# Blosc/c-blosc

Measured on AMD Instinct MI355X. Metric: compress+decompress GB/s (uncompressed) at 1/2/4/8 GPUs vs HBM roofline; ratio, higher is better.
Workload: dtype u8; 1 GPU; config #2: byte-shuffle + lz4 clevel=5 typesize=8, 128 x 64 MiB bench19 chunks per GPU (8 GiB), step = compress pass + decompress pass, device-resident; chunks_per_gpu=128, chunks_total=128, chunk_bytes=67108864

## Files before the change

### c-blosc_amd/csrc/blosc_api.hip

```cpp
#include <errno.h>
#include <pthread.h>
#include <stdio.h>
#include <stdlib.h>
#include <string.h>

#include "../../include/blosc.h"
#include "../../include/blosc_gpu.h"
#include "../../include/blosc_gpu_packed.h"
#include "../../include/blosc_gpu_params.h"
#include "../../include/blosc_gpu_getitem.h"
#include "../../include/blosc_gpu_checksum.h"
#include "blosc_format.h"
#include "engine.h"

using namespace bamd;

static pthread_mutex_t g_mutex = PTHREAD_MUTEX_INITIALIZER;
static int g_compressor = BLOSC_BLOSCLZ;
static int g_threads = 1;
static int g_force_blocksize = 0;
static int g_initlib = 0;
static int g_splitmode = BLOSC_FORWARD_COMPAT_SPLIT;

static const char* const kNames[6] = {BLOSC_BLOSCLZ_COMPNAME, BLOSC_LZ4_COMPNAME, BLOSC_LZ4HC_COMPNAME,
// ... 199 lines not shown
  const bool nolock = getenv("BLOSC_NOLOCK") != NULL;
  if (!nolock) pthread_mutex_lock(&g_mutex);
  int r = decompress_one(src, dest, destsize);
  if (!nolock) pthread_mutex_unlock(&g_mutex);
  return r;
}

int blosc_getitem(const void* src, int start, int nitems, void* dest) {
  return engine_getitem(src, start, nitems, dest, engine_is_device_pointer(src), engine_is_device_pointer(dest), (hipStream_t)0);
}

int blosc_gpu_set_device(int device) { return engine_set_device(device); }

static int compress_batch(int clevel, int doshuffle, size_t typesize, const char* compressor, size_t blocksize,
                          int nchunks, const void* const* src, const size_t* nbytes, void* const* dest,
                          const size_t* destsize, int* cbytes_out, void* stream, bool device_ptrs) {
  if (nchunks <= 0) return 0;
  const int code = compressor ? blosc_compname_to_compcode(compressor) : g_compressor;
  if (code < 0 || !codec_built(code)) { for (int i = 0; i < nchunks; i++) cbytes_out[i] = -5; return 0; }
  Job* jobs = (Job*)malloc(sizeof(Job) * (size_t)nchunks);
  if (!jobs) return -1;
  for (int i = 0; i < nchunks; i++) jobs[i] = Job{src[i], dest[i], nbytes[i], destsize[i]};
  CompressParams p{clevel, doshuffle, typesize, code, (int32_t)(blocksize ? blocksize : (size_t)g_force_blocksize), g_splitmode};
  int r = engine_compress_batch(&p, false, nchunks, jobs, cbytes_out, device_ptrs, (hipStream_t)stream);
  free(jobs);
  return r;
}
int blosc_gpu_compress_batch(int clevel, int doshuffle, size_t typesize, const char* compressor, size_t blocksize,
                             int nchunks, const void* const* src, const size_t* nbytes, void* const* dest,
                             const size_t* destsize, int* cbytes_out, void* stream) {
  return compress_batch(clevel, doshuffle, typesize, compressor, blocksize, nchunks, src, nbytes, dest, destsize, cbytes_out, stream, true);
}
int blosc_gpu_compress_batch_host(int clevel, int doshuffle, size_t typesize, const char* compressor, size_t blocksize,
                                  int nchunks, const void* const* src, const size_t* nbytes, void* const* dest,
                                  const size_t* destsize, int* cbytes_out) {
  return compress_batch(clevel, doshuffle, typesize, compressor, blocksize, nchunks, src, nbytes, dest, destsize, cbytes_out, nullptr, false);
}

static int decompress_batch(int nchunks, const void* const* src, const size_t* srcsize, void* const* dest,
                            const size_t* destsize, int* nbytes_out, void* stream, bool device_ptrs) {
  if (nchunks <= 0) return 0;
  Job* jobs = (Job*)malloc(sizeof(Job) * (size_t)nchunks);
  if (!jobs) return -1;
  for (int i = 0; i < nchunks; i++) jobs[i] = Job{src[i], dest[i], srcsize ? srcsize[i] : 0, destsize[i]};
  int r = engine_decompress_batch(nchunks, jobs, nbytes_out, device_ptrs, (hipStream_t)stream);
  free(jobs);
  return r;
}
int blosc_gpu_decompress_batch(int nchunks, const void* const* src, const size_t* srcsize, void* const* dest,
                               const size_t* destsize, int* nbytes_out, void* stream) {
  return decompress_batch(nchunks, src, srcsize, dest, destsize, nbytes_out, stream, true);
}
int blosc_gpu_decompress_batch_host(int nchunks, const void* const* src, const size_t* srcsize, void* const* dest,
                                    const size_t* destsize, int* nbytes_out) {
  return decompress_batch(nchunks, src, srcsize, dest, destsize, nbytes_out, nullptr, false);
}

static bool packed_align(size_t* align) {
  if (*align == 0) *align = 1;
  return *align <= 4096 && (*align & (*align - 1)) == 0;
}
size_t blosc_gpu_packed_bound(int nchunks, const size_t* nbytes, size_t align) {
  if (nchunks <= 0 || !nbytes || !packed_align(&align)) return 0;
  size_t total = 0;
  for (int i = 0; i < nchunks; i++) total += (nbytes[i] + BLOSC_MAX_OVERHEAD + align - 1) / align * align;
  return total;
}

int blosc_gpu_compress_packed(int clevel, int doshuffle, size_t typesize, const char* compressor, size_t blocksize,
                              int nchunks, const void* const* src, const size_t* nbytes, void* dest, size_t destsize, size_t align,
                              size_t* offsets_out, int* cbytes_out, void* stream) {
  if (nchunks < 0 || !offsets_out || !packed_align(&align)) return -1;
  if (nchunks == 0) { offsets_out[0] = 0; return 0; }
  if (!src || !nbytes || !cbytes_out || (!dest && destsize)) return -1;
  const int code = compressor ? blosc_compname_to_compcode(compressor) : g_compressor;
  if (code < 0 || !codec_built(code)) {
    for (int i = 0; i < nchunks; i++) { cbytes_out[i] = -5; offsets_out[i] = 0; }
    offsets_out[nchunks] = 0;
    return 0;
  }
  Job* jobs = (Job*)malloc(sizeof(Job) * (size_t)nchunks);
  if (!jobs) return -1;
  for (int i = 0; i < nchunks; i++) jobs[i] = Job{src[i], nullptr, nbytes[i], nbytes[i] + BLOSC_MAX_OVERHEAD};
  CompressParams p{clevel, doshuffle, typesize, code, (int32_t)(blocksize ? blocksize : (size_t)g_force_blocksize), g_splitmode};
  const PackedBuffer pk{dest, destsize, align, offsets_out};
  int r = engine_compress_batch(&p, false, nchunks, jobs, cbytes_out, true, (hipStream_t)stream, &pk);
  free(jobs);
  return r;
}

static CompressParams* chunk_params(int nchunks, const blosc_gpu_cparams* params) {
  CompressParams* p = (CompressParams*)malloc(sizeof(CompressParams) * (size_t)nchunks);
  for (int i = 0; p && i < nchunks; i++) {
    const blosc_gpu_cparams& c = params[i];
    p[i] = CompressParams{c.clevel, c.doshuffle, c.typesize, c.compcode == -1 ? g_compressor : c.compcode,
                          (int32_t)(c.blocksize ? c.blocksize : (size_t)g_force_blocksize), c.splitmode ? c.splitmode : g_splitmode};
    if (p[i].codec < 0 || p[i].codec > 5) p[i].codec = BLOSC_SNAPPY;
    if (c.splitmode < 0 || c.splitmode > BLOSC_FORWARD_COMPAT_SPLIT) p[i].doshuffle = -1;
  }
  return p;
}
int blosc_gpu_compress_batch_params(int nchunks, const blosc_gpu_cparams* params, const void* const* src, const size_t* nbytes,
                                    void* const* dest, const size_t* destsize, int* cbytes_out, void* stream) {
  if (nchunks <= 0) return 0;
  if (!params || !src || !nbytes || !dest || !destsize || !cbytes_out) return -1;
  Job* jobs = (Job*)malloc(sizeof(Job) * (size_t)nchunks);
  CompressParams* p = chunk_params(nchunks, params);
  int r = -1;
  if (jobs && p) {
    for (int i = 0; i < nchunks; i++) jobs[i] = Job{src[i], dest[i], nbytes[i], destsize[i]};
    r = engine_compress_batch(p, true, nchunks, jobs, cbytes_out, true, (hipStream_t)stream);
  }
  free(jobs); free(p);
  return r;
}
int blosc_gpu_compress_packed_params(int nchunks, const blosc_gpu_cparams* params, const void* const* src, const size_t* nbytes,
                                     void* dest, size_t destsize, size_t align, size_t* offsets_out, int* cbytes_out, void* stream) {
  if (nchunks < 0 || !offsets_out || !packed_align(&align)) return -1;
  if (nchunks == 0) { offsets_out[0] = 0; return 0; }
  if (!params || !src || !nbytes || !cbytes_out || (!dest && destsize)) return -1;
  Job* jobs = (Job*)malloc(sizeof(Job) * (size_t)nchunks);
  CompressParams* p = chunk_params(nchunks, params);
  int r = -1;
  if (jobs && p) {
    for (int i = 0; i < nchunks; i++) jobs[i] = Job{src[i], nullptr, nbytes[i], nbytes[i] + BLOSC_MAX_OVERHEAD};
    const PackedBuffer pk{dest, destsize, align, offsets_out};
    r = engine_compress_batch(p, true, nchunks, jobs, cbytes_out, true, (hipStream_t)stream, &pk);
  }
  free(jobs); free(p);
  return r;
}

int blosc_gpu_decompress_packed(int nchunks, const void* container, size_t containersize, const size_t* offsets,
                                void* dest, size_t destsize, size_t* dest_offsets_out, int* nbytes_out, void* stream) {
  if (nchunks < 0 || !dest_offsets_out) return -1;
  if (nchunks == 0) { dest_offsets_out[0] = 0; return 0; }
  if (!container || !offsets || !nbytes_out) return -1;
  for (int i = 0; i < nchunks; i++) if (offsets[i + 1] < offsets[i]) return -1;
  if (offsets[nchunks] > containersize) return -1;
  Job* jobs = (Job*)malloc(sizeof(Job) * (size_t)nchunks);
  if (!jobs) return -1;
  for (int i = 0; i < nchunks; i++) {
    const size_t span = offsets[i + 1] - offsets[i];
    jobs[i] = Job{(const uint8_t*)container + offsets[i], nullptr, span < (size_t)BLOSC_MIN_HEADER_LENGTH ? 1 : span, 0};
  }
  const PackedBuffer pk{dest, dest ? destsize : 0, 0, dest_offsets_out};
  int r = engine_decompress_batch(nchunks, jobs, nbytes_out, true, (hipStream_t)stream, &pk);
  free(jobs);
  return r;
}

int blosc_gpu_cbuffer_sizes_batch(int nchunks, const void* const* src, size_t* nbytes, size_t* cbytes, size_t* blocksize, void* stream) {
  if (nchunks < 0 || (nchunks > 0 && !src)) return -1;
  if (nchunks == 0) return 0;
  Header* h = (Header*)malloc(sizeof(Header) * (size_t)nchunks);
  if (!h) return -1;
  const int r = engine_chunk_headers(nchunks, src, h, (hipStream_t)stream);
  for (int i = 0; r == 0 && i < nchunks; i++) {
    const bool known = h[i].version == BLOSC_VERSION_FORMAT;
    if (nbytes) nbytes[i] = known ? (size_t)h[i].nbytes : 0;
    if (cbytes) cbytes[i] = known ? (size_t)h[i].cbytes : 0;
    if (blocksize) blocksize[i] = known ? (size_t)h[i].blocksize : 0;
  }
  free(h);
  return r;
}

int blosc_gpu_device_count(void) { return engine_device_count(); }
int blosc_gpu_partition(size_t nchunks, int world, int rank, size_t* lo, size_t* hi) {
  if (world <= 0 || rank < 0 || rank >= world || !lo || !hi) return -1;
  const size_t w = (size_t)world, r = (size_t)rank;
  size_t l = (r * nchunks + w - 1) / w, h = ((r + 1) * nchunks + w - 1) / w;
  if (h > nchunks) h = nchunks;
  *lo = l; *hi = h;
  return 0;
}
struct MultiArg {
  int dev, rc; bool compress; size_t lo, hi;
  int clevel, doshuffle; size_t typesize; const char* compressor; size_t blocksize;
  const void* const* src; const size_t* insize; void* const* dest; const size_t* destsize; int* out;
};
static void* multi_worker(void* p) {
  MultiArg& a = *(MultiArg*)p;
  a.rc = 0;
  if (a.hi == a.lo) return nullptr;
  if (engine_thread_device(a.dev) != 0) { a.rc = -1; return nullptr; }
  const int n = (int)(a.hi - a.lo);
  const bool devp = engine_is_device_pointer(a.src[a.lo]);
  if (a.compress) a.rc = compress_batch(a.clevel, a.doshuffle, a.typesize, a.compressor, a.blocksize, n, a.src + a.lo, a.insize + a.lo, a.dest + a.lo,
                                        a.destsize + a.lo, a.out + a.lo, nullptr, devp);
  else a.rc = decompress_batch(n, a.src + a.lo, a.insize ? a.insize + a.lo : nullptr, a.dest + a.lo, a.destsize + a.lo, a.out + a.lo, nullptr, devp);
  (void)engine_thread_device(-1);
  return nullptr;
}
static int run_multi(MultiArg proto, int ndev, const int* devices, int nchunks) {
  if (nchunks <= 0) return 0;
  const int have = engine_device_count();
  if (ndev <= 0 || ndev > 64) return -1;
  MultiArg args[64];
  pthread_t th[64];
  for (int r = 0; r < ndev; r++) {
    args[r] = proto;
    args[r].dev = devices ? devices[r] : r;
    if (args[r].dev < 0 || args[r].dev >= have) { fprintf(stderr, "blosc_amd: multi-GPU call names device %d, this node shows %d\n", args[r].dev, have); return -1; }
    (void)blosc_gpu_partition((size_t)nchunks, ndev, r, &args[r].lo, &args[r].hi);
  }
  int started = 0, rc = 0;
  for (; started < ndev; started++) if (pthread_create(&th[started], nullptr, multi_worker, &args[started]) != 0) { rc = -1; break; }
  for (int r = 0; r < started; r++) { pthread_join(th[r], nullptr); if (args[r].rc < 0) rc = args[r].rc; }
  return rc;
}
int blosc_gpu_compress_batch_multi(int ndev, const int* devices, int clevel, int doshuffle, size_t typesize, const char* compressor, size_t blocksize,
                                   int nchunks, const void* const* src, const size_t* nbytes, void* const* dest, const size_t* destsize, int* cbytes_out) {
  MultiArg a{}; a.compress = true; a.clevel = clevel; a.doshuffle = doshuffle; a.typesize = typesize; a.compressor = compressor; a.blocksize = blocksize;
  a.src = src; a.insize = nbytes; a.dest = dest; a.destsize = destsize; a.out = cbytes_out;
  return run_multi(a, ndev, devices, nchunks);
}
int blosc_gpu_decompress_batch_multi(int ndev, const int* devices, int nchunks, const void* const* src, const size_t* srcsize, void* const* dest,
                                     const size_t* destsize, int* nbytes_out) {
  MultiArg a{}; a.compress = false; a.src = src; a.insize = srcsize; a.dest = dest; a.destsize = destsize; a.out = nbytes_out;
  return run_multi(a, ndev, devices, nchunks);
}

int blosc_gpu_getitem(const void* src, int start, int nitems, void* dest, void* stream) {
  return engine_getitem(src, start, nitems, dest, true, true, (hipStream_t)stream);
}

static ItemRange* item_ranges(int nranges, const int* chunk, const int* start, const int* nitems, void* const* dest) {
  ItemRange* r = (ItemRange*)malloc(sizeof(ItemRange) * (size_t)(nranges > 0 ? nranges : 1));
  for (int i = 0; r && i < nranges; i++) r[i] = ItemRange{chunk[i], start[i], nitems[i], dest ? dest[i] : nullptr};
  return r;
}
int blosc_gpu_getitem_batch(int nchunks, const void* const* src, int nranges, const int* chunk, const int* start, const int* nitems,
                            void* const* dest, int* result_out, void* stream) {
  if (nchunks < 0 || nranges < 0) return -1;
  if (nranges == 0) return 0;
  if ((nchunks > 0 && !src) || !chunk || !start || !nitems || !dest || !result_out) return -1;
  Job* jobs = (Job*)malloc(sizeof(Job) * (size_t)(nchunks > 0 ? nchunks : 1));
  ItemRange* ranges = item_ranges(nranges, chunk, start, nitems, dest);
  int r = -1;
  if (jobs && ranges) {
    for (int i = 0; i < nchunks; i++) jobs[i] = Job{src[i], nullptr, 0, 0};
    r = engine_getitem_batch(nchunks, jobs, nranges, ranges, result_out, (hipStream_t)stream);
  }
  free(jobs); free(ranges);
  return r;
}
int blosc_gpu_getitem_packed(int nchunks, const void* container, size_t containersize, const size_t* offsets,
                             int nranges, const int* chunk, const int* start, const int* nitems,
                             void* dest, size_t destsize, size_t* dest_offsets_out, int* result_out, void* stream) {
  if (nchunks < 0 || nranges < 0 || !dest_offsets_out) return -1;
  if (nranges == 0) { dest_offsets_out[0] = 0; return 0; }
  if ((nchunks > 0 && (!container || !offsets)) || !chunk || !start || !nitems || !result_out) return -1;
  for (int i = 0; i < nchunks; i++) if (offsets[i + 1] < offsets[i]) return -1;
  if (nchunks > 0 && offsets[nchunks] > containersize) return -1;
  Job* jobs = (Job*)malloc(sizeof(Job) * (size_t)(nchunks > 0 ? nchunks : 1));
  ItemRange* ranges = item_ranges(nranges, chunk, start, nitems, nullptr);
  int r = -1;
  if (jobs && ranges) {
    for (int i = 0; i < nchunks; i++) {
      const size_t span = offsets[i + 1] - offsets[i];
      jobs[i] = Job{(const uint8_t*)container + offsets[i], nullptr, span < (size_t)BLOSC_MIN_HEADER_LENGTH ? 1 : span, 0};
    }
    const PackedBuffer pk{dest, dest ? destsize : 0, 0, dest_offsets_out};
    r = engine_getitem_batch(nchunks, jobs, nranges, ranges, result_out, (hipStream_t)stream, &pk);
  }
  free(jobs); free(ranges);
  return r;
}

static const size_t kChecksumMaxRun = (size_t)INT32_MAX + 16;
static int checksum_runs(int kind, int nruns, Job* jobs, unsigned int* digest_out, void* stream) {
  int r = -1;
  if (jobs) {
    bool ok = true;
    for (int i = 0; i < nruns && ok; i++) ok = jobs[i].srcsize <= kChecksumMaxRun && (jobs[i].srcsize == 0 || jobs[i].src);
    if (ok) r = engine_checksum_batch(kind, nruns, jobs, digest_out, (hipStream_t)stream);
  }
  free(jobs);
  return r;
}
int blosc_gpu_checksum_batch(int kind, int nruns, const void* const* src, const size_t* nbytes, unsigned int* digest_out, void* stream) {
  if (kind != BLOSC_GPU_CHECKSUM_ADLER32 && kind != BLOSC_GPU_CHECKSUM_CRC32) return -1;
  if (nruns <= 0) return 0;
  if (!src || !nbytes || !digest_out) return -1;
  Job* jobs = (Job*)malloc(sizeof(Job) * (size_t)nruns);
  for (int i = 0; jobs && i < nruns; i++) jobs[i] = Job{src[i], nullptr, nbytes[i], 0};
  return checksum_runs(kind, nruns, jobs, digest_out, stream);
}
int blosc_gpu_checksum_packed(int kind, int nruns, const void* container, size_t containersize, const size_t* offsets,
                              const size_t* length, unsigned int* digest_out, void* stream) {
  if (kind != BLOSC_GPU_CHECKSUM_ADLER32 && kind != BLOSC_GPU_CHECKSUM_CRC32) return -1;
  if (nruns <= 0) return 0;
  if (!offsets || !digest_out) return -1;
  for (int i = 0; i < nruns; i++)
    if (offsets[i + 1] < offsets[i] || (length && length[i] > offsets[i + 1] - offsets[i])) return -1;
  if (offsets[nruns] > containersize || (offsets[nruns] > offsets[0] && !container)) return -1;
  Job* jobs = (Job*)malloc(sizeof(Job) * (size_t)nruns);
  for (int i = 0; jobs && i < nruns; i++)
    jobs[i] = Job{(const uint8_t*)container + offsets[i], nullptr, length ? length[i] : offsets[i + 1] - offsets[i], 0};
  return checksum_runs(kind, nruns, jobs, digest_out, stream);
}

__attribute__((visibility("default"))) void blosc_internal_shuffle(const size_t typesize, const size_t blocksize,
                                                                   const uint8_t* src, const uint8_t* dest) {
  if (engine_filter(0, typesize, blocksize, src, (void*)dest) != 0) fprintf(stderr, "blosc_amd: shuffle failed (no GPU?)\n");
}
__attribute__((visibility("default"))) void blosc_internal_unshuffle(const size_t typesize, const size_t blocksize,
                                                                     const uint8_t* src, const uint8_t* dest) {
  if (engine_filter(1, typesize, blocksize, src, (void*)dest) != 0) fprintf(stderr, "blosc_amd: unshuffle failed (no GPU?)\n");
}
__attribute__((visibility("default"))) void blosc_internal_shuffle_generic(const size_t typesize, const size_t blocksize,
                                                                           const uint8_t* const src, uint8_t* const dest) {
  blosc_internal_shuffle(typesize, blocksize, src, dest);
}
__attribute__((visibility("default"))) void blosc_internal_unshuffle_generic(const size_t typesize, const size_t blocksize,
                                                                             const uint8_t* const src, uint8_t* const dest) {
  blosc_internal_unshuffle(typesize, blocksize, src, dest);
}
#define BAMD_SHUFFLE_ALIAS(isa)                                                                                                                  \
  __attribute__((visibility("default"))) void blosc_internal_shuffle_##isa(const size_t typesize, const size_t blocksize, const uint8_t* const src, \
                                                                           uint8_t* const dest) { blosc_internal_shuffle(typesize, blocksize, src, dest); } \
  __attribute__((visibility("default"))) void blosc_internal_unshuffle_##isa(const size_t typesize, const size_t blocksize, const uint8_t* const src, \
                                                                             uint8_t* const dest) { blosc_internal_unshuffle(typesize, blocksize, src, dest); }
BAMD_SHUFFLE_ALIAS(sse2)
BAMD_SHUFFLE_ALIAS(avx2)
#undef BAMD_SHUFFLE_ALIAS
__attribute__((visibility("default"))) int blosc_internal_bitshuffle(const size_t typesize, const size_t blocksize,
                                                                     const uint8_t* src, const uint8_t* dest,
                                                                     const uint8_t* tmp) {
  (void)tmp;
  if (engine_filter(2, typesize, blocksize, src, (void*)dest) != 0) return -1;
  const size_t n = blocksize / typesize;
  return (int)((n % 8) ? n : n * typesize);
}
__attribute__((visibility("default"))) int blosc_internal_bitunshuffle(const size_t typesize, const size_t blocksize,
                                                                       const uint8_t* src, const uint8_t* dest,
                                                                       const uint8_t* tmp) {
  (void)tmp;
  if (engine_filter(3, typesize, blocksize, src, (void*)dest) != 0) return -1;
  const size_t n = blocksize / typesize;
  return (int)((n % 8) ? n : n * typesize);
}

__attribute__((visibility("default"))) int blosc_amd_policy_blocksize(int clevel, int typesize, int nbytes, int forced,
                                                                      int codec, int splitmode) {
  return compute_blocksize(clevel, typesize, nbytes, forced, codec, splitmode);
}
__attribute__((visibility("default"))) int blosc_amd_policy_split(int codec, int typesize, int blocksize, int splitmode) {
  return split_block(codec, typesize, blocksize, splitmode);
}
__attribute__((visibility("default"))) void blosc_amd_getitem_pass_bytes(size_t bytes) { engine_getitem_pass_bytes(bytes); }

__attribute__((visibility("default"))) void blosc_amd_checksum_tile_bytes(size_t bytes) { engine_checksum_tile_bytes(bytes); }

void blosc_gpu_profile(int enable) { engine_prof_enable(enable); }
void blosc_gpu_profile_reset(void) { engine_prof_reset(); }
int blosc_gpu_profile_get(const char* kernel, double* total_ms, int* launches) { return engine_prof_get(kernel, total_ms, launches); }

}
```

### c-blosc_amd/csrc/enc_lz.h

```cpp
constexpr int ENC_WAVES = 1;
#ifndef BAMD_ENC_HASH_BITS
#define BAMD_ENC_HASH_BITS 11
#endif
constexpr int ENC_HASH_BITS = BAMD_ENC_HASH_BITS;
constexpr int ENC_TAB = 1 << ENC_HASH_BITS;
typedef uint32_t enc_entry_t;
#ifndef BAMD_ENC_SPLIT_TAB
#define BAMD_ENC_SPLIT_TAB 1
#endif
constexpr int ENC_TAB_BYTES = BAMD_ENC_SPLIT_TAB ? ENC_TAB * 3 : ENC_TAB * 4;
#ifndef BAMD_ENC_MINWAVES
#define BAMD_ENC_MINWAVES (BAMD_ENC_SPLIT_TAB ? 6 : 5)
#endif
#ifndef BAMD_ENC_SEQ_SKIPCAP
#define BAMD_ENC_SEQ_SKIPCAP 32u
#endif
#ifndef BAMD_ENC_LZ_MINWAVES
#define BAMD_ENC_LZ_MINWAVES 6
#endif
constexpr int ENC_LDS_WAVES = (160 * 1024) / ENC_TAB_BYTES;
constexpr int ENC_WAVES_PER_CU = ENC_LDS_WAVES < 4 * BAMD_ENC_MINWAVES ? ENC_LDS_WAVES : 4 * BAMD_ENC_MINWAVES;
constexpr int ENC_LZ_LDS_WAVES = (160 * 1024) / (ENC_TAB_BYTES + 512);
constexpr int ENC_LZ_WAVES_PER_CU = ENC_LZ_LDS_WAVES < 4 * BAMD_ENC_LZ_MINWAVES ? ENC_LZ_LDS_WAVES : 4 * BAMD_ENC_LZ_MINWAVES;

struct EncTable {
  __attribute__((address_space(3))) uint32_t* w;
  __attribute__((address_space(3))) uint16_t* pos;
  __attribute__((address_space(3))) uint8_t* tag;
  __device__ __forceinline__ void init(void* base) {
    w = (__attribute__((address_space(3))) uint32_t*)base;
    pos = (__attribute__((address_space(3))) uint16_t*)base;
    tag = (__attribute__((address_space(3))) uint8_t*)base + 2 * ENC_TAB;
  }
  __device__ __forceinline__ void clear(int lane) {
    for (int k = lane; k < ENC_TAB_BYTES / 4; k += 64) w[k] = 0u;
  }
  __device__ __forceinline__ void put(uint32_t h, uint32_t entry) {
    if (BAMD_ENC_SPLIT_TAB) { pos[h] = (uint16_t)entry; tag[h] = (uint8_t)(entry >> 24); }
    else w[h] = entry;
  }
  __device__ __forceinline__ uint32_t get(uint32_t h) const {
    if (BAMD_ENC_SPLIT_TAB) return (uint32_t)pos[h] | ((uint32_t)tag[h] << 24);
    return w[h];
  }
  __device__ __forceinline__ static bool tag_equal(uint32_t a, uint32_t b) {
    return BAMD_ENC_SPLIT_TAB ? ((a ^ b) >> 24) == 0u : ((a ^ b) >> 16) == 0u;
  }
};

__device__ __forceinline__ uint32_t enc_mix(uint32_t seq) { return seq * 2654435761u; }
__device__ __forceinline__ uint32_t enc_slot(uint32_t mix) { return mix >> (32 - ENC_HASH_BITS); }
__device__ __forceinline__ uint32_t enc_entry(uint32_t mix, uint32_t p) { return ((mix << ENC_HASH_BITS) & 0xffff0000u) | (p & 0xffffu); }

__device__ __forceinline__ uint64_t ld8u(const gu8* p) { return g_ld8(p); }

__device__ __forceinline__ uint32_t common16(const uint4& x, const uint4& y) {
  const uint64_t lo = ((uint64_t)(x.y ^ y.y) << 32) | (x.x ^ y.x);
  const uint64_t hi = ((uint64_t)(x.w ^ y.w) << 32) | (x.z ^ y.z);
  if (lo) return (uint32_t)__builtin_ctzll(lo) >> 3;
  return hi ? 8u + ((uint32_t)__builtin_ctzll(hi) >> 3) : 16u;
}

__device__ __forceinline__ uint32_t wave_common_fwd_rest(const gu8* src, uint32_t n, uint32_t a, uint32_t b,
                                                         uint32_t maxlen, uint32_t done, int lane) {
  if (done == 256u && done < maxlen && a + done + 1024u <= n) {
    const uint4 x0 = g_ld16(src + a + done + 16 * lane), y0 = g_ld16(src + b + done + 16 * lane);
    const uint32_t q1 = done + 16u * (uint32_t)lane;
    uint32_t e1 = common16(x0, y0);
    const uint32_t r1 = q1 < maxlen ? maxlen - q1 : 0u;
    if (e1 > r1) e1 = r1;
    const uint64_t s1 = __ballot(e1 < 16u);
    if (s1) { const int f = __builtin_ctzll(s1); return done + 16u * (uint32_t)f + (uint32_t)__builtin_amdgcn_readlane((int)e1, f); }
    done += 1024u;
  }
  while (done < maxlen && a + done + 2048u <= n) {
    const gu8* pa = src + a + done + 16 * lane;
    const gu8* pb = src + b + done + 16 * lane;
    const uint4 x0 = g_ld16(pa), x1 = g_ld16(pa + 1024);
    const uint4 y0 = g_ld16(pb), y1 = g_ld16(pb + 1024);
    const uint32_t q = done + 16u * (uint32_t)lane;
    uint32_t e0 = common16(x0, y0), e1 = common16(x1, y1);
    const uint32_t r0 = q < maxlen ? maxlen - q : 0u;
    const uint32_t r1 = q + 1024u < maxlen ? maxlen - q - 1024u : 0u;
    if (e0 > r0) e0 = r0;
    if (e1 > r1) e1 = r1;
    const uint64_t s0 = __ballot(e0 < 16u);
    if (s0) { const int f = __builtin_ctzll(s0); return done + 16u * (uint32_t)f + (uint32_t)__builtin_amdgcn_readlane((int)e0, f); }
    const uint64_t s1 = __ballot(e1 < 16u);
    if (s1) { const int f = __builtin_ctzll(s1); return done + 1024u + 16u * (uint32_t)f + (uint32_t)__builtin_amdgcn_readlane((int)e1, f); }
    done += 2048u;
  }
  while (done < maxlen) {
    const uint32_t q = done + 8u * (uint32_t)lane;
    uint32_t vb = 0;
    if (q < maxlen) vb = (maxlen - q < 8u) ? maxlen - q : 8u;
    uint32_t eq = 0;
    if (vb) {
      if (a + q + 8u <= n) {
        uint64_t x = ld8u(src + a + q) ^ ld8u(src + b + q);
        eq = x ? (uint32_t)(__builtin_ctzll(x) >> 3) : 8u;
        if (eq > vb) eq = vb;
      } else {
        while (eq < vb && src[a + q + eq] == src[b + q + eq]) eq++;
      }
    }
    const uint64_t stop = __ballot(eq < 8u);
    if (stop) {
      const int f = __builtin_ctzll(stop);
      return done + 8u * (uint32_t)f + (uint32_t)__builtin_amdgcn_readlane((int)eq, f);
    }
    done += 512u;
  }
  return maxlen;
}
__device__ __forceinline__ uint32_t wave_common_first256(uint32_t x, uint32_t maxlen, int lane) {
  const uint32_t q = 4u * (uint32_t)lane;
  uint32_t e0 = x ? (uint32_t)(__builtin_ctz(x) >> 3) : 4u;
  const uint32_t r0 = q < maxlen ? maxlen - q : 0u;
  if (e0 > r0) e0 = r0;
  const uint64_t s0 = __ballot(e0 < 4u);
  if (s0) { const int f = __builtin_ctzll(s0); return 4u * (uint32_t)f + (uint32_t)__builtin_amdgcn_readlane((int)e0, f); }
  return 0xffffffffu;
}
__device__ __forceinline__ uint32_t wave_common_fwd(const gu8* src, uint32_t n, uint32_t a, uint32_t b,
                                                    uint32_t maxlen, int lane) {
  uint32_t done = 0;
  if (maxlen && a + 256u <= n) {
    const uint32_t r = wave_common_first256(g_ld4(src + a + 4 * lane) ^ g_ld4(src + b + 4 * lane), maxlen, lane);
    if (r != 0xffffffffu) return r;
    done = 256u;
  }
  return wave_common_fwd_rest(src, n, a, b, maxlen, done, lane);
}

#ifdef BAMD_ENC_NOSTORE
#define ENC_ST1(ptr, val) do { (void)(ptr); (void)(val); } while (0)
#else
#define ENC_ST1(ptr, val) do { *(ptr) = (val); } while (0)
#endif
__device__ __forceinline__ uint32_t emit_ext255(gu8* p, uint32_t v, int lane) {
  const uint32_t n255 = v / 255u, rem = v - n255 * 255u;
  for (uint32_t k = (uint32_t)lane; k < n255; k += 64u) ENC_ST1(p + k, (uint8_t)255u);
  if (lane == 0) ENC_ST1(p + n255, (uint8_t)rem);
  return n255 + 1u;
}

enum { EF_LZ4 = 0, EF_BLOSCLZ = 1, EF_ZSTD = 2, EF_ZLIB = 3, EF_ZLIB2 = 4 };
#ifndef BAMD_ZSTD_MINLEN
#define BAMD_ZSTD_MINLEN 4
#endif

struct ZsSink {
  gu8* lit;
  uint32_t nlit, litcap;
  BAMD_GAS uint64_t* seq;
  uint32_t nseq, seqcap;
};
__device__ __forceinline__ uint32_t zs_emit_seq(ZsSink& z, const gu8* lit, uint32_t ll, uint32_t off, uint32_t mlen, int lit_lane0, uint32_t ownbyte, int lane);

struct DflSink {
  gu8* out; uint32_t cap;
  uint32_t pos;
  uint32_t acc, nb;
  volatile BAMD_LAS uint32_t* zb;
};
__device__ __forceinline__ uint32_t wave_incl_scan_u32(uint32_t v, int lane) {
#pragma unroll
  for (int d = 1; d < 64; d <<= 1) { const uint32_t t = (uint32_t)__shfl_up((int)v, d, 64); if (lane >= d) v += t; }
  return v;
}
__device__ __forceinline__ bool dfl_put_symbols(DflSink& z, uint32_t bits, uint32_t nbits, int lane) {
  const uint32_t incl = wave_incl_scan_u32(nbits, lane);
  const uint32_t total = (uint32_t)__builtin_amdgcn_readlane((int)incl, 63);
  z.zb[lane] = lane == 0 ? z.acc : 0u;
  if (lane == 0) z.zb[64] = 0u;
  BAMD_LDS_SYNC();
  if (nbits) {
    const uint32_t start = z.nb + incl - nbits, w = start >> 5, sh = start & 31u;
    __hip_atomic_fetch_or((BAMD_LAS uint32_t*)z.zb + w, bits << sh, __ATOMIC_RELAXED, __HIP_MEMORY_SCOPE_WAVEFRONT);
    if (sh + nbits > 32u) __hip_atomic_fetch_or((BAMD_LAS uint32_t*)z.zb + w + 1u, bits >> (32u - sh), __ATOMIC_RELAXED, __HIP_MEMORY_SCOPE_WAVEFRONT);
  }
  const uint32_t fill = z.nb + total, ndw = fill >> 5;
  if (z.pos + 4u * ndw + 16u > z.cap) return false;
  BAMD_LDS_SYNC();
  const uint32_t mine = z.zb[lane], rest = z.zb[ndw];
  if ((uint32_t)lane < ndw) g_st4(z.out + z.pos + 4u * (uint32_t)lane, mine);
  z.acc = uni(rest); z.nb = fill & 31u; z.pos += 4u * ndw;
  return true;
}
__device__ __forceinline__ uint32_t dfl_emit_seq(DflSink& z, const gu8* lit, uint32_t ll, uint32_t dist, uint32_t mlen, int lit_lane0, uint32_t ownbyte, int lane) {
  const bool in_regs = lit_lane0 >= 0 && ll <= 64u && (uint32_t)lit_lane0 + ll <= 64u;
  const uint32_t np = mlen ? dfl::npieces(mlen) : 0u;
  uint32_t ldone = 0, pdone = 0;
  do {
    const uint32_t lcnt = ll - ldone < 64u ? ll - ldone : 64u;
    uint32_t pcnt = 0;
    if (ldone + lcnt == ll) { pcnt = np - pdone < 64u - lcnt ? np - pdone : 64u - lcnt; }
    const uint32_t vreg = in_regs ? (uint32_t)__builtin_amdgcn_ds_bpermute((int)(((uint32_t)lit_lane0 + (uint32_t)lane) & 63u) << 2, (int)ownbyte) & 0xffu : 0u;
    dfl::Sym s = {0u, 0u};
    if ((uint32_t)lane < lcnt) s = dfl::literal(in_regs ? vreg : (uint32_t)lit[ldone + (uint32_t)lane]);
    else if ((uint32_t)lane < lcnt + pcnt) s = dfl::match(dfl::piece_len(mlen, pdone + (uint32_t)lane - lcnt, np), dist);
    if (!dfl_put_symbols(z, s.bits, s.nbits, lane)) return 0xffffffffu;
    ldone += lcnt; pdone += pcnt;
  } while (ldone < ll || pdone < np);
  return 0u;
}

__device__ __forceinline__ void emit_literals(gu8* dst, const gu8* lit, uint32_t ll, int lit_lane0, uint32_t ownbyte, int lane) {
  if (lit_lane0 >= 0 && ll <= 64u && (uint32_t)lit_lane0 + ll <= 64u) {
    const uint32_t v = (uint32_t)__builtin_amdgcn_ds_bpermute((int)(((uint32_t)lit_lane0 + (uint32_t)lane) & 63u) << 2, (int)ownbyte);
    if ((uint32_t)lane < ll) ENC_ST1(dst + lane, (uint8_t)v);
  } else {
    wave_copy_disjoint(dst, lit, ll, lane);
  }
}

__device__ __forceinline__ uint32_t lz4_emit_seq(gu8* dst, uint32_t op, uint32_t cap, const gu8* lit,
                                                 uint32_t ll, uint32_t off, uint32_t mlen, int lit_lane0, uint32_t ownbyte, int lane) {
  if (op + 1u + ll + (2u + 1u + 5u) + ll / 255u > cap) return 0xffffffffu;
  const uint32_t mcode = mlen - 4u;
  if (ll < 15u && mcode < 15u + 255u && (ll == 0u || (lit_lane0 >= 0 && (uint32_t)lit_lane0 + ll <= 64u))) {
    if (op + 1u + ll + 2u + (1u + 5u) + (mcode + 240u) / 255u > cap) return 0xffffffffu;
    const uint32_t v = (uint32_t)__builtin_amdgcn_ds_bpermute((int)(((uint32_t)lit_lane0 + (uint32_t)lane - 1u) & 63u) << 2, (int)ownbyte);
    uint32_t b = v;
    b = lane == 0 ? ((ll << 4) | (mcode < 15u ? mcode : 15u)) : b;
    b = (uint32_t)lane == ll + 1u ? off : b;
    b = (uint32_t)lane == ll + 2u ? off >> 8 : b;
    b = (uint32_t)lane == ll + 3u ? mcode - 15u : b;
    const uint32_t total = ll + 3u + (mcode >= 15u ? 1u : 0u);
    if ((uint32_t)lane < total) ENC_ST1(dst + op + lane, (uint8_t)b);
    return op + total;
  }
  const uint32_t tok = ((ll < 15u ? ll : 15u) << 4) | (mcode < 15u ? mcode : 15u);
  if (lane == 0) ENC_ST1(dst + op, (uint8_t)tok);
  op += 1u;
  if (ll >= 15u) op += emit_ext255(dst + op, ll - 15u, lane);
  emit_literals(dst + op, lit, ll, lit_lane0, ownbyte, lane);
  op += ll;
  if (lane < 2) ENC_ST1(dst + op + lane, (uint8_t)(off >> (8 * lane)));
  op += 2u;
  if (op + (1u + 5u) + (mcode + 240u) / 255u > cap) return 0xffffffffu;
  if (mcode >= 15u) op += emit_ext255(dst + op, mcode - 15u, lane);
  return op;
}
__device__ __forceinline__ uint32_t lz4_emit_tail(gu8* dst, uint32_t op, uint32_t cap, const gu8* lit,
                                                  uint32_t run, int lane) {
  if (op + run + 1u + (run + 255u - 15u) / 255u > cap) return 0xffffffffu;
  if (lane == 0) dst[op] = (uint8_t)((run < 15u ? run : 15u) << 4);
  op += 1u;
  if (run >= 15u) op += emit_ext255(dst + op, run - 15u, lane);
  wave_copy_disjoint(dst + op, lit, run, lane);
  return op + run;
}

__device__ __forceinline__ uint32_t blz_emit_literals(gu8* dst, uint32_t op, uint32_t cap, const gu8* lit,
                                                      uint32_t ll, int lane) {
  if (ll == 0u) return op;
  const uint32_t nch = (ll + 31u) >> 5;
  if (op + ll + nch > cap) return 0xffffffffu;
  for (uint32_t c = (uint32_t)lane; c < nch; c += 64u) {
    const uint32_t cnt = (ll - 32u * c < 32u) ? ll - 32u * c : 32u;
    dst[op + 33u * c] = (uint8_t)(cnt - 1u);
  }
  for (uint32_t k = (uint32_t)lane; k < ll; k += 64u) dst[op + k + (k >> 5) + 1u] = lit[k];
  return op + ll + nch;
}
__device__ __forceinline__ uint32_t blz_emit_match(gu8* dst, uint32_t op, uint32_t cap, uint32_t dist,
                                                   uint32_t mlen, int lane) {
  const uint32_t L = mlen - 2u;
  uint32_t bd = dist - 1u;
  const bool far = bd >= 8191u;
  if (far) bd -= 8191u;
  const uint32_t hi = far ? 31u : (bd >> 8);
  const uint32_t next = (L >= 7u) ? (L - 7u) / 255u + 1u : 0u;
  const uint32_t total = 1u + next + (far ? 3u : 1u);
  if (op + total + 2u > cap) return 0xffffffffu;
  if (lane == 0) dst[op] = (uint8_t)(((L < 7u ? L : 7u) << 5) | hi);
  op += 1u;
  if (L >= 7u) op += emit_ext255(dst + op, L - 7u, lane);
  if (far) {
    if (lane == 0) { dst[op] = 255u; dst[op + 1] = (uint8_t)(bd >> 8); dst[op + 2] = (uint8_t)bd; }
    op += 3u;
  } else {
    if (lane == 0) dst[op] = (uint8_t)bd;
    op += 1u;
  }
  return op;
}

#ifndef BAMD_ENC_RANK_CAP
#define BAMD_ENC_RANK_CAP 20
#endif
constexpr uint32_t RANK_CAP = BAMD_ENC_RANK_CAP;

struct Bytes20 { uint64_t a, b; uint32_t c; };

__device__ __forceinline__ Bytes20 load20(const gu8* src, uint32_t pos, uint32_t n) {
  Bytes20 r;
  if (pos + 20u <= n) { r.a = g_ld8(src + pos); r.b = g_ld8(src + pos + 8u); r.c = RANK_CAP > 16u ? g_ld4(src + pos + 16u) : 0u; }
  else {
    r.a = 0; r.b = 0; r.c = 0;
    for (uint32_t k = 0; k < 20u && pos + k < n; k++) {
      const uint64_t v = src[pos + k];
      if (k < 8u) r.a |= v << (8u * k); else if (k < 16u) r.b |= v << (8u * (k - 8u)); else r.c |= (uint32_t)v << (8u * (k - 16u));
    }
  }
  return r;
}
__device__ __forceinline__ uint32_t common20(const Bytes20& x, const Bytes20& y) {
  uint64_t d = x.a ^ y.a;
  if (d) return (uint32_t)__builtin_ctzll(d) >> 3;
  d = x.b ^ y.b;
  if (d) return 8u + ((uint32_t)__builtin_ctzll(d) >> 3);
  const uint32_t e = x.c ^ y.c;
  return e ? 16u + ((uint32_t)__builtin_ctz(e) >> 3) : 20u;
}
__device__ __forceinline__ uint32_t runlen20(const Bytes20& x, uint32_t v) {
  const uint64_t rep = 0x0101010101010101ull * (uint64_t)v;
  Bytes20 y; y.a = rep; y.b = rep; y.c = (uint32_t)rep;
  return common20(x, y);
}
template <int N> __device__ __forceinline__ uint32_t dpp_row_shr0(uint32_t v) {
  return (uint32_t)__builtin_amdgcn_update_dpp(0, (int)v, 0x110 + N, 0xf, 0xf, true);
}
__device__ __forceinline__ uint32_t wave_max_u32(uint32_t v) {
  uint32_t t;
// ... 452 lines not shown
```

### c-blosc_amd/csrc/enc_lz4p.h

```cpp
#ifndef BAMD_ENC_PAR
#define BAMD_ENC_PAR 1
#endif
constexpr int ENC_SCR_BYTES = 512;
static_assert(ENC_LZ_LDS_WAVES == (160 * 1024) / (ENC_TAB_BYTES + ENC_SCR_BYTES), "enc_lz.h sizes the persistent grid with this scratch in mind");
#ifndef BAMD_ENC_BACK2
#define BAMD_ENC_BACK2 1
#endif
#ifndef BAMD_ENC_SKIPCAP
#define BAMD_ENC_SKIPCAP 32u
#endif
#ifndef BAMD_ENC_NEIGHBOUR
#define BAMD_ENC_NEIGHBOUR 4u
#endif
#ifndef BAMD_ENC_KEEPJ
#define BAMD_ENC_KEEPJ 0
#endif
#ifndef BAMD_ENC_EXT2
#define BAMD_ENC_EXT2 1
#endif
#ifndef BAMD_ENC_LAUNDER
#define BAMD_ENC_LAUNDER 1
#endif
#ifndef BAMD_ENC_PREFULL
#define BAMD_ENC_PREFULL 1
#endif

template <int N> __device__ __forceinline__ uint32_t dpp_row_shl0(uint32_t v) {
  return (uint32_t)__builtin_amdgcn_update_dpp(0, (int)v, 0x100 + N, 0xf, 0xf, true);
}
__device__ __forceinline__ uint32_t umax32(uint32_t a, uint32_t b) { return a > b ? a : b; }
__device__ __forceinline__ uint32_t umin32(uint32_t a, uint32_t b) { return a < b ? a : b; }

__device__ __forceinline__ uint32_t wave_common_fwd_lite(const gu8* src, uint32_t n, uint32_t a, uint32_t b, uint32_t maxlen, int lane) {
  uint32_t done = 0;
  if (maxlen && a + 256u <= n) {
    const uint32_t x = g_ld4(src + a + 4 * lane) ^ g_ld4(src + b + 4 * lane);
    const uint32_t q = 4u * (uint32_t)lane;
    uint32_t e0 = x ? (uint32_t)(__builtin_ctz(x) >> 3) : 4u;
    const uint32_t r0 = q < maxlen ? maxlen - q : 0u;
    if (e0 > r0) e0 = r0;
    const uint64_t s0 = __ballot(e0 < 4u);
    if (s0) { const int f = __builtin_ctzll(s0); return 4u * (uint32_t)f + (uint32_t)__builtin_amdgcn_readlane((int)e0, f); }
    done = 256u;
  }
  while (done < maxlen && a + done + 1024u <= n) {
    const uint4 x0 = g_ld16(src + a + done + 16 * lane), y0 = g_ld16(src + b + done + 16 * lane);
    const uint32_t q1 = done + 16u * (uint32_t)lane;
    uint32_t e1 = common16(x0, y0);
    const uint32_t r1 = q1 < maxlen ? maxlen - q1 : 0u;
    if (e1 > r1) e1 = r1;
    const uint64_t s1 = __ballot(e1 < 16u);
    if (s1) { const int f = __builtin_ctzll(s1); return done + 16u * (uint32_t)f + (uint32_t)__builtin_amdgcn_readlane((int)e1, f); }
    done += 1024u;
  }
  while (done < maxlen) {
    const uint32_t q = done + 8u * (uint32_t)lane;
    uint32_t vb = 0;
    if (q < maxlen) vb = (maxlen - q < 8u) ? maxlen - q : 8u;
    uint32_t eq = 0;
    if (vb) {
      if (a + q + 8u <= n) {
        const uint64_t x = ld8u(src + a + q) ^ ld8u(src + b + q);
        eq = x ? (uint32_t)(__builtin_ctzll(x) >> 3) : 8u;
        if (eq > vb) eq = vb;
      } else {
        while (eq < vb && src[a + q + eq] == src[b + q + eq]) eq++;
      }
    }
    const uint64_t stop = __ballot(eq < 8u);
    if (stop) { const int f = __builtin_ctzll(stop); return done + 8u * (uint32_t)f + (uint32_t)__builtin_amdgcn_readlane((int)eq, f); }
    done += 512u;
  }
  return maxlen;
}

template <int SS>
__device__ uint32_t lz4_encode_wave_par(const gu8* __restrict__ src, uint32_t n, gu8* __restrict__ dst, uint32_t cap,
                                        int clevel, enc_entry_t* tab_generic, int lane_in EPROF_ARG) {
  static_assert(SS == 0 || SS == 1, "one or two positions per lane");
  const int lane = lane_in;
  constexpr uint32_t SPAN = 64u << SS;
  EncTable tab;
  tab.init((void*)tab_generic);
  volatile BAMD_LAS uint32_t* scr = (volatile BAMD_LAS uint32_t*)((BAMD_LAS uint8_t*)(void*)tab_generic + ENC_TAB_BYTES);
  if (n < 13u) return 0u;
  const uint32_t last_start = n - 12u;
  const uint32_t mlimit = n - 5u;
  const int accel = 10 - clevel;
  const uint32_t minlen = clevel >= 9 ? 4u : (clevel >= 6 ? 5u : 7u);
  tab.clear(lane);
  EncWindow win;
  win.init(src, n, lane);
  uint32_t ip = 0, anchor = 0, op = 0, nfail = 0;
  bool ins_pending = false;
  while (ip <= last_start) {
    int lane = lane_in;
#if !defined(BAMD_WAVE_EMU) && BAMD_ENC_LAUNDER
    asm volatile("; lane of this step" : "+v"(lane));
#endif
    const uint32_t lq = (uint32_t)lane << SS;
    const uint32_t p = ip + lq;
    const bool live = p <= last_start;
    const bool live1 = SS && p + 1u <= last_start;
    win.seek(ip, lane);
    const uint32_t lo = ip >= 4u ? ip - 4u : 0u;
    const uint32_t rb = lo & ~3u;
    const uint32_t D = (rb - win.wbase) >> 2;
    const int gsel = (int)((D + (uint32_t)lane) << 2);
    const uint32_t ra = (uint32_t)__builtin_amdgcn_ds_bpermute(gsel, (int)win.w0);
    const uint32_t rc = (uint32_t)__builtin_amdgcn_ds_bpermute(gsel, (int)win.w1);
    const uint32_t r = (D + (uint32_t)lane < 64u) ? ra : rc;
    const uint32_t bo0 = ip - rb;
    const uint32_t bo = bo0 + lq;
    const int ksel = (int)((bo >> 2) << 2);
    const uint32_t x0 = (uint32_t)__builtin_amdgcn_ds_bpermute(ksel, (int)r);
    const uint32_t x1 = (uint32_t)__builtin_amdgcn_ds_bpermute(ksel + 4, (int)r);
    const uint32_t x2 = (uint32_t)__builtin_amdgcn_ds_bpermute(ksel + 8, (int)r);
    const uint32_t x3 = (uint32_t)__builtin_amdgcn_ds_bpermute(ksel + 12, (int)r);
    const uint32_t x4 = (uint32_t)__builtin_amdgcn_ds_bpermute(ksel + 16, (int)r);
    const uint32_t x5 = (uint32_t)__builtin_amdgcn_ds_bpermute(ksel + 20, (int)r);
    const uint32_t sh = bo & 3u;
    const uint32_t o0 = __builtin_amdgcn_alignbyte(x1, x0, sh), o1 = __builtin_amdgcn_alignbyte(x2, x1, sh);
    const uint32_t o2 = __builtin_amdgcn_alignbyte(x3, x2, sh), o3 = __builtin_amdgcn_alignbyte(x4, x3, sh);
    const uint32_t o4 = __builtin_amdgcn_alignbyte(x5, x4, sh);
    const uint32_t ownpre = __builtin_amdgcn_alignbyte(x0, (uint32_t)__builtin_amdgcn_ds_bpermute(ksel - 4, (int)r), sh);
    Bytes20 own;
    own.a = ((uint64_t)o1 << 32) | o0; own.b = ((uint64_t)o3 << 32) | o2; own.c = RANK_CAP > 16u ? o4 : 0u;
    const uint64_t r01 = ((uint64_t)(uint32_t)__builtin_amdgcn_readlane((int)r, 1) << 32) | (uint32_t)__builtin_amdgcn_readlane((int)r, 0);
    const uint32_t before2 = bo0 >= 2u ? (uint32_t)(r01 >> (8u * (bo0 - 2u))) & 0xffffu : 0u;
    uint32_t prev;
    if (SS) prev = ownpre >> 24;
    else prev = (uint32_t)__builtin_amdgcn_update_dpp(0, (int)(o0 & 0xffu), 0x138, 0xf, 0xf, false);
    if (lane == 0) prev = ip ? (bo0 >= 2u ? before2 >> 8 : (uint32_t)(r01 >> (8u * (bo0 - 1u))) & 0xffu) : 0x100u;
    if (ins_pending) {
      const uint32_t m2 = enc_mix(before2 | (o0 << 16));
      if (lane == 0) tab.put(enc_slot(m2), enc_entry(m2, ip - 2u));
      ins_pending = false;
    }
    uint32_t cand = 0, limit = 0;
    bool tab_ok = false;
    const uint32_t mix = enc_mix(o0);
#define PAR_PUT() do { const uint32_t mix_ = enc_mix((uint32_t)own.a); tab.put(enc_slot(mix_), enc_entry(mix_, p)); } while (0)
#define PAR_PUT1() do { const uint32_t mix1_ = enc_mix((uint32_t)(own.a >> 8)); tab.put(enc_slot(mix1_), enc_entry(mix1_, p + 1u)); } while (0)
    if (live) {
      limit = mlimit - p; if (limit > RANK_CAP) limit = RANK_CAP;
      const uint32_t h = enc_slot(mix), mine = enc_entry(mix, p);
      const uint32_t e = tab.get(h);
      const uint32_t d = (p - e) & 0xffffu;
      if (d != 0u && d <= p && EncTable::tag_equal(e, mine)) { cand = p - d; tab_ok = true; }
    } else {
      prev = 0x100u;
    }
    PROF_LAP(8); PROF_ADD(0, 1);
    uint32_t len = 0, nb = 0;
    if (tab_ok) {
      const uint32_t cpre = cand >= 4u ? ld4u(src + cand - 4u) : 0u;
      const Bytes20 cb = load20(src, cand, n);
      if (cand >= 4u) { const uint32_t x = cpre ^ ownpre; nb = x ? (uint32_t)__builtin_clz(x) >> 3 : 4u; }
      len = common20(own, cb);
      if (len > limit) len = limit;
      if (len < 4u || len + (SS && nb ? 1u : 0u) < minlen) len = 0;
    }
    if (live && prev < 0x100u) {
      uint32_t rl = runlen20(own, prev);
      if (rl > limit) rl = limit;
      const uint32_t xr = (ownpre ^ (ownpre << 8)) | 0xffu;
      const uint32_t nbr = p >= 5u ? (uint32_t)__builtin_clz(xr) >> 3 : 0u;
      if (rl >= 4u && rl + (SS && nbr ? 1u : 0u) >= minlen && rl > len) { len = rl; cand = p - 1u; nb = nbr; }
    }
    win.settle(lane);
    PROF_LAP(9);
    const uint32_t step_end = ip + SPAN;
    const uint32_t cn = (p - cand) | (nb << 28);
    uint32_t S = len ? (((len + (SS && nb ? 1u : 0u) + SPAN - lq) << 11) | ((63u - (uint32_t)lane) << 5) | len) : 0u;
    S = umax32(S, dpp_row_shl0<1>(S)); S = umax32(S, dpp_row_shl0<2>(S)); S = umax32(S, dpp_row_shl0<4>(S)); S = umax32(S, dpp_row_shl0<8>(S));
    {
      const uint32_t t3 = (uint32_t)__builtin_amdgcn_readlane((int)S, 48);
      const uint32_t t2 = umax32((uint32_t)__builtin_amdgcn_readlane((int)S, 32), t3);
      const uint32_t t1 = umax32((uint32_t)__builtin_amdgcn_readlane((int)S, 16), t2);
      const uint32_t add = lane < 16 ? t1 : (lane < 32 ? t2 : (lane < 48 ? t3 : 0u));
      S = umax32(S, add);
    }
    uint32_t J0;
    {
      const uint32_t wS = 63u - ((S >> 5) & 63u), LS = S & 31u;
      const uint32_t nx = ((wS << SS) + LS + (SS ? 1u : 0u)) >> SS;
      J0 = (S == 0u || LS >= RANK_CAP || nx > 63u) ? 63u : nx;
    }
#if BAMD_ENC_KEEPJ
    const uint32_t J1 = (uint32_t)__builtin_amdgcn_ds_bpermute((int)(J0 << 2), (int)J0);
    const uint32_t J2 = (uint32_t)__builtin_amdgcn_ds_bpermute((int)(J1 << 2), (int)J1);
    const uint32_t J3 = (uint32_t)__builtin_amdgcn_ds_bpermute((int)(J2 << 2), (int)J2);
#endif
    uint32_t lane_lo = 0;
    bool any = false, tail_open = false;
    for (;;) {
#if !defined(BAMD_WAVE_EMU) && BAMD_ENC_LAUNDER
      asm volatile("; lane of this chain" : "+v"(lane));
#endif
#if !BAMD_ENC_KEEPJ
      const uint32_t J1 = (uint32_t)__builtin_amdgcn_ds_bpermute((int)(J0 << 2), (int)J0);
      const uint32_t J2 = (uint32_t)__builtin_amdgcn_ds_bpermute((int)(J1 << 2), (int)J1);
      const uint32_t J3 = (uint32_t)__builtin_amdgcn_ds_bpermute((int)(J2 << 2), (int)J2);
#endif
      uint32_t c = umin32((lane_lo + (SS ? 1u : 0u)) >> SS, 63u);
      { const uint32_t t = (uint32_t)__builtin_amdgcn_ds_bpermute((int)(c << 2), (int)J0); c = (lane & 1) ? t : c; }
      { const uint32_t t = (uint32_t)__builtin_amdgcn_ds_bpermute((int)(c << 2), (int)J1); c = (lane & 2) ? t : c; }
      { const uint32_t t = (uint32_t)__builtin_amdgcn_ds_bpermute((int)(c << 2), (int)J2); c = (lane & 4) ? t : c; }
      { const uint32_t t = (uint32_t)__builtin_amdgcn_ds_bpermute((int)(c << 2), (int)J3); c = (lane & 8) ? t : c; }
      const uint32_t Sr = (uint32_t)__builtin_amdgcn_ds_bpermute((int)(c << 2), (int)S);
      const bool valid = lane < 16 && c < 63u && Sr != 0u;
      const uint32_t nseq = (uint32_t)__builtin_popcountll(__ballot(valid));
      if (nseq == 0u) { tail_open = any; break; }
      any = true;
      const uint32_t last = nseq - 1u;
      const uint32_t w = 63u - ((Sr >> 5) & 63u), L = Sr & 31u;
      const uint32_t wq = w << SS;
      const uint32_t cnr = (uint32_t)__builtin_amdgcn_ds_bpermute((int)(w << 2), (int)cn);
      const uint32_t dist_r = cnr & 0xffffu, nb_r = cnr >> 28;
      const uint32_t cand_r = ip + wq - dist_r;
      uint32_t cq = c;
      if (SS) { const uint32_t e_prev = dpp_row_shr0<1>(wq + L); cq = lane == 0 ? lane_lo : e_prev; }
      const uint32_t room = wq - cq;
      const uint32_t w_last = (uint32_t)__builtin_amdgcn_readlane((int)wq, (int)last), L_last = (uint32_t)__builtin_amdgcn_readlane((int)L, (int)last);
      const uint32_t pm_last = ip + w_last;
      uint32_t mext = 0;
      if (L_last >= RANK_CAP && pm_last + RANK_CAP < mlimit) {
        const uint32_t c_last = (uint32_t)__builtin_amdgcn_readlane((int)cand_r, (int)last);
        mext = BAMD_ENC_EXT2 ? wave_common_fwd(src, n, pm_last + RANK_CAP, c_last + RANK_CAP, mlimit - (pm_last + RANK_CAP), lane)
                              : wave_common_fwd_lite(src, n, pm_last + RANK_CAP, c_last + RANK_CAP, mlimit - (pm_last + RANK_CAP), lane);
      }
      uint32_t back = valid ? umin32(nb_r, umin32(room, cand_r)) : 0u;
      if (BAMD_ENC_BACK2) {
        const bool more = valid && back == 4u && room > 4u && cand_r >= 12u;
        if (__ballot(more)) {
          const uint32_t pm = ip + wq;
          const uint64_t a = g_ld8(src + (more ? pm - 12u : 0u)), b = g_ld8(src + (more ? cand_r - 12u : 0u));
          const uint64_t x = a ^ b;
          const uint32_t eq = x ? (uint32_t)__builtin_clzll(x) >> 3 : 8u;
          if (more) back += umin32(eq, room - 4u);
        }
      }
      uint32_t pre = lane_lo == 0u ? ip - anchor : 0u;
      uint32_t pre_ext = 0;
      if (BAMD_ENC_PREFULL && pre) {
        const uint32_t b0 = (uint32_t)__builtin_amdgcn_readlane((int)back, 0), room0 = (uint32_t)__builtin_amdgcn_readlane((int)room, 0);
        const uint32_t cand0 = (uint32_t)__builtin_amdgcn_readlane((int)cand_r, 0);
        if (b0 == room0 && cand0 > b0) {
          uint32_t maxb = umin32(pre, cand0 - b0);
          if (maxb > 64u) maxb = 64u;
          const uint32_t pm0 = ip + (uint32_t)__builtin_amdgcn_readlane((int)wq, 0) - b0, cm0 = cand0 - b0;
          const bool bl = (uint32_t)lane < maxb;
          const uint32_t bx = src[bl ? pm0 - 1u - (uint32_t)lane : pm0], by = src[bl ? cm0 - 1u - (uint32_t)lane : cm0];
          const uint64_t bm = __ballot(!bl || bx != by);
          pre_ext = bm ? (uint32_t)__builtin_ctzll(bm) : 64u;
          pre -= pre_ext;
        }
      }
      PROF_LAP(10); PROF_ADD(2, L_last >= RANK_CAP); PROF_ADD(6, nseq);
      const uint32_t mlen = L + back + ((uint32_t)lane == last ? mext : 0u) + (lane == 0 ? pre_ext : 0u);
      const uint32_t mcode = mlen - 4u;
      const uint32_t inl = room - back;
      const uint32_t ll = inl + (lane == 0 ? pre : 0u);
      const bool r0pre = pre != 0u && lane == 0;
      const uint32_t hdr = r0pre ? 0u : (ll >= 15u ? 2u : 1u);
      const uint32_t nme = mcode >= 15u ? 1u : 0u;
      const uint32_t size = valid ? hdr + inl + 2u + nme : 0u;
      uint32_t incl = size;
      incl += dpp_row_shr0<1>(incl); incl += dpp_row_shr0<2>(incl); incl += dpp_row_shr0<4>(incl); incl += dpp_row_shr0<8>(incl);
      const uint32_t excl = incl - size;
      const uint32_t mcode_last = (uint32_t)__builtin_amdgcn_readlane((int)mcode, (int)last);
      const uint32_t extra_last = mcode_last >= 15u + 255u ? (mcode_last - 15u) / 255u : 0u;
      const uint32_t total = (uint32_t)__builtin_amdgcn_readlane((int)incl, (int)last) + extra_last;
      uint32_t ll0 = 0, prebytes = 0;
      if (pre) { ll0 = (uint32_t)__builtin_amdgcn_readlane((int)ll, 0); prebytes = 1u + (ll0 >= 15u ? 1u + (ll0 - 15u) / 255u : 0u) + pre; }
      if (op + prebytes + total + 8u > cap) return 0u;
      if (pre) {
        const uint32_t mc0 = (uint32_t)__builtin_amdgcn_readlane((int)mcode, 0);
        if (lane == 0) ENC_ST1(dst + op, (uint8_t)(((ll0 < 15u ? ll0 : 15u) << 4) | (mc0 < 15u ? mc0 : 15u)));
        op += 1u;
        if (ll0 >= 15u) op += emit_ext255(dst + op, ll0 - 15u, lane);
        wave_copy_disjoint(dst + op, src + anchor, pre, lane);
        op += pre;
        PROF_ADD(3, 1);
      }
      scr[lane] = 0u;
      if (SS) scr[lane + 64] = 0u;
      BAMD_LDS_SYNC();
      if (valid) scr[cq] = 0x80000000u | (excl + hdr) | (inl << 10) | (w << 17) | (L << 23);
      BAMD_LDS_SYNC();
      const uint32_t myw = scr[lq];
      const uint32_t myw1 = SS ? scr[lq + 1u] : 0u;
      const uint64_t fm = __ballot((myw >> 31) != 0u);
      uint32_t s;
      bool has;
      if (SS) {
        const uint64_t fm1 = __ballot((myw1 >> 31) != 0u);
        const uint64_t be = fm & ((2ull << lane) - 1ull), bo_ = fm1 & ((1ull << lane) - 1ull);
        const uint32_t se = 2u * (63u - (uint32_t)__builtin_clzll(be | 1ull)), so = 2u * (63u - (uint32_t)__builtin_clzll(bo_ | 1ull)) + 1u;
        s = (bo_ != 0ull && (be == 0ull || so > se)) ? so : se;
        has = (be | bo_) != 0ull;
      } else {
        const uint64_t below = fm & ((2ull << lane) - 1ull);
        s = 63u - (uint32_t)__builtin_clzll(below | 1ull);
        has = below != 0ull;
      }
      const uint32_t inf = scr[s];
      BAMD_LDS_SYNC();
      {
        const uint32_t tpos = op + excl;
        if (valid && hdr) ENC_ST1(dst + tpos, (uint8_t)(((ll < 15u ? ll : 15u) << 4) | (mcode < 15u ? mcode : 15u)));
        if (valid && hdr == 2u) ENC_ST1(dst + tpos + 1u, (uint8_t)(ll - 15u));
        const uint32_t opos = tpos + hdr + inl;
#ifndef BAMD_ENC_NOSTORE
        if (valid) g_st2(dst + opos, dist_r);
#endif
        if (valid && nme) ENC_ST1(dst + opos + 2u, (uint8_t)(mcode - 15u < 255u ? mcode - 15u : 255u));
        if (extra_last) {
          const uint32_t opos_last = (uint32_t)__builtin_amdgcn_readlane((int)opos, (int)last);
          emit_ext255(dst + opos_last + 2u, mcode_last - 15u, lane);
        }
      }
      {
        const uint32_t k = lq - s;
        const uint32_t i_out = inf & 1023u, i_inl = (inf >> 10) & 127u, i_w = ((inf >> 17) & 63u) << SS, i_L = (inf >> 23) & 31u;
        if (has && k < i_inl) ENC_ST1(dst + op + i_out + k, (uint8_t)own.a);
        const bool open_end = i_L < RANK_CAP;
        const uint32_t e = i_w + i_L;
        if (live && has && (lq <= i_w || (open_end && (lq + 2u == e || lq >= e)))) PAR_PUT();
      }
      if (SS) {
        const bool own1 = (myw1 >> 31) != 0u;
        const uint32_t inf1 = own1 ? myw1 : inf;
        const bool has1 = has || own1;
        const uint32_t q1 = lq + 1u, k1 = own1 ? 0u : q1 - s;
        const uint32_t j_out = inf1 & 1023u, j_inl = (inf1 >> 10) & 127u, j_w = ((inf1 >> 17) & 63u) << SS, j_L = (inf1 >> 23) & 31u;
        if (has1 && k1 < j_inl) ENC_ST1(dst + op + j_out + k1, (uint8_t)(own.a >> 8));
        const bool open1 = j_L < RANK_CAP;
        const uint32_t e1 = j_w + j_L;
        if (live1 && has1 && (q1 <= j_w || (open1 && (q1 + 2u == e1 || q1 >= e1)))) PAR_PUT1();
      }
      op += total;
      const uint32_t e_last = w_last + L_last + mext;
      anchor = ip + e_last;
      PROF_LAP(11);
      if (L_last < RANK_CAP || e_last >= SPAN) break;
      lane_lo = e_last;
      if (live && lq + 2u == lane_lo) PAR_PUT();
      if (live1 && lq + 3u == lane_lo) PAR_PUT1();
    }
    if (!any) {
      PROF_ADD(1, 1);
      if (live) PAR_PUT();
      if (live1) PAR_PUT1();
      nfail += 1u << SS;
      uint32_t adv = (nfail * (uint32_t)accel) / 16u;
      if (adv > BAMD_ENC_SKIPCAP - (1u << SS)) adv = BAMD_ENC_SKIPCAP - (1u << SS);
      if (BAMD_ENC_NEIGHBOUR && ((nfail >> SS) & (BAMD_ENC_NEIGHBOUR - 1u)) == 0u) adv = 0u;
      ip += SPAN + 64u * adv;
      continue;
    }
    nfail = 0;
    if (anchor >= step_end) {
      ip = anchor;
      ins_pending = true;
    } else {
      if (tail_open && live && lq >= lane_lo) PAR_PUT();
      if (tail_open && live1 && lq + 1u >= lane_lo) PAR_PUT1();
      ip = step_end;
    }
  }
#undef PAR_PUT
#undef PAR_PUT1
  op = lz4_emit_tail(dst, op, cap, src + anchor, n - anchor, lane);
  if (op == 0xffffffffu) return 0u;
  PROF_LAP(12);
  return op < n ? op : 0u;
}

#ifndef BAMD_ENC_STRIDE2_MAXCLEVEL
#define BAMD_ENC_STRIDE2_MAXCLEVEL 5
#endif
__device__ __forceinline__ uint32_t lz4_encode_wave_auto(const gu8* __restrict__ src, uint32_t n, gu8* __restrict__ dst, uint32_t cap,
                                                         int clevel, enc_entry_t* tab_generic, int lane EPROF_ARG) {
  if (clevel <= BAMD_ENC_STRIDE2_MAXCLEVEL) return lz4_encode_wave_par<1>(src, n, dst, cap, clevel, tab_generic, lane EPROF_PASS);
  return lz4_encode_wave_par<0>(src, n, dst, cap, clevel, tab_generic, lane EPROF_PASS);
}
```

### c-blosc_amd/csrc/engine.h

```cpp
#pragma once
#include <hip/hip_runtime.h>
#include <stddef.h>
#include <stdint.h>

namespace bamd {

struct CompressParams {
  int clevel;
  int doshuffle;
  size_t typesize;
  int codec;
  int32_t forced_blocksize;
  int splitmode;
};

struct Job {
  const void* src;
  void* dst;
  size_t srcsize;
  size_t dstsize;
};

struct PackedBuffer {
  void* base;
  size_t size;
  size_t align;
  size_t* offsets;
};

int engine_compress_batch(const CompressParams* params, bool per_chunk, int n, const Job* jobs, int* results, bool device_ptrs,
                          hipStream_t stream, const PackedBuffer* packed = nullptr);
int engine_decompress_batch(int n, const Job* jobs, int* results, bool device_ptrs, hipStream_t stream,
                            const PackedBuffer* packed = nullptr);
struct Header;
int engine_chunk_headers(int n, const void* const* src, Header* out, hipStream_t stream);
int engine_getitem(const void* src, int start, int nitems, void* dest, bool src_on_device, bool dst_on_device,
                   hipStream_t stream);
struct ItemRange { int chunk, start, nitems; void* dst; };
int engine_getitem_batch(int nchunks, const Job* chunks, int nranges, const ItemRange* ranges, int* results, hipStream_t stream,
                         const PackedBuffer* packed = nullptr);
void engine_getitem_pass_bytes(size_t bytes);

int engine_checksum_batch(int kind, int n, const Job* runs, uint32_t* digests, hipStream_t stream);
void engine_checksum_tile_bytes(size_t bytes);

int engine_filter(int kind, size_t typesize, size_t blocksize, const void* src, void* dst);

int engine_set_device(int dev);
int engine_thread_device(int dev);
int engine_device_count();
void engine_release();
bool engine_is_device_pointer(const void* p);

void engine_prof_enable(int on);
void engine_prof_reset();
int engine_prof_get(const char* kernel, double* total_ms, int* launches);

}
```

### c-blosc_amd/csrc/engine.hip

```cpp
#include "engine.h"

#include <pthread.h>
#include <stdio.h>
#include <stdlib.h>
#include <string.h>

#include <map>
#include <atomic>
#include <mutex>
#include <string>
#include <vector>
#include <algorithm>

#include <chrono>
#include "blosc_format.h"
#include "dev_types.h"
#include "queue_order.h"

#include "k_filters.hip"
#include "k_decode.hip"
#include "k_encode.hip"
#include "k_zstd.hip"
#include "k_zstd2.hip"
#include "k_zlib.hip"
#include "k_checksum.hip"

namespace bamd {

static std::atomic<bool> g_warned{false};
#define HIP_TRY(expr)                                                                             \
  do {                                                                                            \
    hipError_t _e = (expr);                                                                       \
    if (_e != hipSuccess) {                                                                       \
      fprintf(stderr, "blosc_amd: HIP error '%s' at %s:%d (%s)\n", hipGetErrorString(_e), __FILE__, __LINE__, #expr); \
      return -1;                                                                                  \
    }                                                                                             \
  } while (0)

static inline size_t align_up(size_t v, size_t a) { return (v + a - 1) / a * a; }
struct Carver {
  size_t off = 0; size_t take(size_t bytes, size_t align = 256) { off = align_up(off, align); size_t r = off; off += bytes; return r; }
};

constexpr long SWITCH_SET = -0x7fffffffL;
static long switch_every_call(const char* name, long dflt) {
  const char* e = getenv(name);
  return dflt == SWITCH_SET ? (e != nullptr) : (e ? atol(e) : dflt);
}
#define SWITCH_ONCE(name, dflt) ([] { static const long v = switch_every_call(name, dflt); return v; }())
#ifdef BAMD_ENV_EVERY_CALL
#define SWITCH_PLACEMENT switch_every_call
#else
#define SWITCH_PLACEMENT SWITCH_ONCE
#endif
#ifndef BAMD_LZ4HC_DEFAULT
#define BAMD_LZ4HC_DEFAULT 1
#endif
#ifndef BAMD_ZSTD_TABLES_DEFAULT
#define BAMD_ZSTD_TABLES_DEFAULT 1
#endif
static bool is_on(long v) { return (int)v != 0; }
static bool debug_cost_enabled()  { return is_on(SWITCH_ONCE("BLOSC_AMD_DEBUG_COST", SWITCH_SET)); }
static bool hosttime_on()         { return is_on(SWITCH_ONCE("BLOSC_AMD_HOSTTIME", 0)); }
static bool table_cache_enabled() { return is_on(SWITCH_ONCE("BLOSC_AMD_TABLE_CACHE", 1)); }
static bool fuse_enabled()        { return is_on(SWITCH_ONCE("BLOSC_AMD_FUSE", 1)); }
static bool span_enabled()        { return is_on(SWITCH_ONCE("BLOSC_AMD_SPANS", 1)); }
static bool periodic_enabled()    { return is_on(SWITCH_ONCE("BLOSC_AMD_PERIODIC", 1)); }
static int zstd2_mode()           { return (int)SWITCH_ONCE("BLOSC_AMD_ZSTD2", 2); }
static int contexts_wanted()      { return (int)SWITCH_ONCE("BLOSC_AMD_CONTEXTS", 8); }
static size_t arena_skew_bytes()  { const long k = SWITCH_PLACEMENT("BLOSC_AMD_ARENA_SKEW_KIB", 0); return (size_t)(k < 0 ? 0 : (k > 65536 ? 65536 : k)) << 10; }
static bool debug_enabled()        { return is_on(switch_every_call("BLOSC_AMD_DEBUG", SWITCH_SET)); }
static bool single_queue_forced()  { return is_on(switch_every_call("BLOSC_AMD_SINGLE_QUEUE", 0)); }
static bool lz4hc_search_enabled() { return is_on(switch_every_call("BLOSC_AMD_LZ4HC", BAMD_LZ4HC_DEFAULT)); }
static bool zstd_tables_enabled()  { return is_on(switch_every_call("BLOSC_AMD_ZSTD_TABLES", BAMD_ZSTD_TABLES_DEFAULT)); }
static bool zstd_search_enabled(int clevel) { return is_on(switch_every_call("BLOSC_AMD_ZSTD_SEARCH", clevel >= 6)); }
static bool zlib_search_enabled()  { return is_on(switch_every_call("BLOSC_AMD_ZLIB_SEARCH", 1)); }
static bool zstd_huffman_enabled() { return is_on(switch_every_call("BLOSC_AMD_ZSTD_HUFFMAN", 0)); }
static bool zlib_dynamic_enabled() { return is_on(switch_every_call("BLOSC_AMD_ZLIB_DYNAMIC", 1)); }

struct DeviceArena {
  uint8_t* base = nullptr;
  uint8_t* raw = nullptr;
  size_t cap = 0;
  int ensure(size_t bytes) {
    if (bytes <= cap) return 0;
    if (raw) { (void)hipFree(raw); raw = base = nullptr; cap = 0; }
    size_t want = align_up(bytes + bytes / 8, 1 << 20);
    const size_t skew = arena_skew_bytes();
    HIP_TRY(hipMalloc((void**)&raw, want + skew));
    base = raw + skew;
    cap = want;
    if (debug_enabled()) fprintf(stderr, "[blosc_amd] device arena %p, %zu MiB\n", (void*)base, want >> 20);
    return 0;
  }
  void release() { if (raw) (void)hipFree(raw); raw = base = nullptr; cap = 0; }
};
struct PinnedArena {
  uint8_t* base = nullptr;
  size_t cap = 0;
  int ensure(size_t bytes) {
    if (bytes <= cap) return 0;
    if (base) { (void)hipHostFree(base); base = nullptr; cap = 0; }
    size_t want = align_up(bytes + bytes / 4, 1 << 16);
    HIP_TRY(hipHostMalloc((void**)&base, want, hipHostMallocDefault));
    cap = want;
    return 0;
  }
  void release() { if (base) (void)hipHostFree(base); base = nullptr; cap = 0; }
};

struct ProfEntry { double ms = 0; int launches = 0; };

constexpr size_t kCostWords = 264;
static int check_done(const uint32_t* fb, size_t expect, size_t expect_zstd, const char* what, size_t expect_zlib = 0) {
  if (fb[256] == expect && fb[257] == expect_zstd && fb[259] == expect_zlib) return 0;
  fprintf(stderr, "blosc_amd: %s: the device took %u of %zu queued tasks (Zstd: %u of %zu, Zlib: %u of %zu) - results discarded\n",
          what, fb[256], expect, fb[257], expect_zstd, fb[259], expect_zlib);
  return -1;
}

struct EngineState {
  std::mutex mu;
  bool device_ok = false;
  int device = -1;
  std::atomic<int> device_hint{-1};
  DeviceArena dev;
  DeviceArena io;
  PinnedArena pin;
  std::map<std::string, ProfEntry> prof_acc;
  struct Pending { std::string name; hipEvent_t a, b; };
  std::vector<Pending> prof_pending;
  std::vector<hipEvent_t> ev_pool;
  uint32_t enc_cost[256] = {0}, dec_cost[256] = {0};
  bool enc_cost_valid = false, dec_cost_valid = false;
  bool single_queue = false;
  int cus = 0;
  struct TableKey { std::vector<BlockDesc> blocks; std::vector<uint32_t> modes; std::vector<int> order; int nq = 0; };
  struct EncGroup { int mode; size_t q_at, sh_at; int32_t ntasks; };
  struct TableCache {
    TableKey key; bool valid = false;
    DeviceArena tabs; size_t o_queues = 0, o_zqueues = 0; std::vector<EncGroup> groups;
    bool hit = false;
    std::vector<int32_t> queues, zqueues; size_t p_blocks = 0, p_queues = 0, p_zqueues = 0;
    bool same(const TableKey& k) const {
      return valid && key.nq == k.nq && key.blocks.size() == k.blocks.size() && key.modes == k.modes && key.order == k.order &&
             (k.blocks.empty() || memcmp(key.blocks.data(), k.blocks.data(), k.blocks.size() * sizeof(BlockDesc)) == 0);
    }
    template <class Build>
    int begin(const char* what, const TableKey& k, size_t queue_words, size_t zqueue_words, Carver& pin, Build&& build) {
      hit = table_cache_enabled() && same(k);
      if (debug_cost_enabled()) fprintf(stderr, "[blosc_amd] %s: block table and queues %s\n", what, hit ? "still on the device" : "built and uploaded");
      if (hit) return 0;
      valid = false;
      queues.clear(); zqueues.clear();
      build(*this);
      const size_t nblk = k.blocks.size();
      Carver tcv;
      tcv.take(sizeof(BlockDesc) * (nblk ? nblk : 1));
      o_queues = tcv.take(sizeof(int32_t) * (queue_words ? queue_words : queues.size()));
      if (zqueue_words) o_zqueues = tcv.take(sizeof(int32_t) * zqueue_words);
      if (tabs.ensure(tcv.off)) return -1;
      p_blocks = pin.take(sizeof(BlockDesc) * (nblk ? nblk : 1));
      p_queues = pin.take(sizeof(int32_t) * queues.size());
      p_zqueues = pin.take(sizeof(int32_t) * (zqueues.size() + 1));
      return 0;
    }
    int upload(const TableKey& k, uint8_t* P, hipStream_t stream) {
      if (hit) return 0;
      const struct { size_t dev, pin; const void* from; size_t bytes; } up[3] = {
        {0, p_blocks, k.blocks.data(), sizeof(BlockDesc) * k.blocks.size()},
        {o_queues, p_queues, queues.data(), sizeof(int32_t) * queues.size()},
        {o_zqueues, p_zqueues, zqueues.data(), sizeof(int32_t) * zqueues.size()}};
      for (const auto& u : up) {
        if (!u.bytes) continue;
        memcpy(P + u.pin, u.from, u.bytes);
        HIP_TRY(hipMemcpyAsync(tabs.base + u.dev, P + u.pin, u.bytes, hipMemcpyHostToDevice, stream));
      }
      return 0;
    }
    void commit(TableKey& k) { if (!hit) { std::swap(key, k); valid = true; } }
    BlockDesc* d_blocks() const { return (BlockDesc*)tabs.base; }
    const int32_t* d_qoff() const { return (const int32_t*)(tabs.base + o_queues); }
    const int32_t* d_zqoff() const { return (const int32_t*)(tabs.base + o_zqueues); }
    void drop() { valid = false; tabs.release(); }
  } enc_tabs, dec_tabs;
  hipStream_t own = nullptr;
};

constexpr int kMaxCtx = 8;
static EngineState g_ctx[kMaxCtx];
static std::atomic<int> g_device{-1};
static thread_local int tl_device = -1;
static bool g_forked = false;
static int wanted_device() {
  if (tl_device >= 0) return tl_device;
  int d = g_device.load();
  if (d >= 0 || g_forked) return d;
  int cur = -1;
  if (hipGetDevice(&cur) != hipSuccess || cur < 0) { (void)hipGetLastError(); return -1; }
  int none = -1;
  (void)g_device.compare_exchange_strong(none, cur);
  return g_device.load();
}
static std::atomic<bool> g_prof{false};
static std::atomic<unsigned> g_ctx_turn{0};
static int ctx_count() {
#ifdef BAMD_WAVE_EMU
  return 1;
#else
  return std::min(std::max(contexts_wanted(), 1), kMaxCtx);
#endif
}
static std::mutex g_pick_mu;
struct CtxGuard {
  EngineState* st = nullptr;
  CtxGuard() {
    const int n = ctx_count();
    const int want = wanted_device();
    int wait_on = -1;
    {
      std::lock_guard<std::mutex> pick(g_pick_mu);
      for (int pass = 0; pass < 3 && !st; pass++)
        for (int i = 0; i < n && !st; i++) {
          if (!g_ctx[i].mu.try_lock()) continue;
          const bool ok = pass == 2 || (pass == 0 ? (g_ctx[i].device_ok && g_ctx[i].device == want) : !g_ctx[i].device_ok);
          if (ok) st = &g_ctx[i]; else g_ctx[i].mu.unlock();
        }
      if (!st) {
        const unsigned turn = g_ctx_turn.fetch_add(1u);
        for (int k = 0; k < n && wait_on < 0; k++) { const int i = (int)((turn + (unsigned)k) % (unsigned)n); if (g_ctx[i].device_hint.load(std::memory_order_relaxed) == want) wait_on = i; }
        if (wait_on < 0) wait_on = (int)(turn % (unsigned)n);
      }
    }
    if (!st) { st = &g_ctx[wait_on]; st->mu.lock(); }
  }
  ~CtxGuard() { st->mu.unlock(); }
  CtxGuard(const CtxGuard&) = delete;
  CtxGuard& operator=(const CtxGuard&) = delete;
};

__global__ void k_probe_xcc(uint32_t* hist) {
  if (threadIdx.x == 0) atomicAdd(&hist[__builtin_amdgcn_s_getreg((3 << 11) | 20) & 15u], 1u);
}
static void probe_topology(EngineState& st) {
  st.single_queue = single_queue_forced();
  if (st.single_queue) return;
  uint32_t* d = nullptr; uint32_t h[16] = {0};
  bool ok = hipMalloc((void**)&d, sizeof h) == hipSuccess && hipMemset(d, 0, sizeof h) == hipSuccess;
  if (ok) {
    hipLaunchKernelGGL(k_probe_xcc, dim3(64), dim3(64), 0, 0, d);
    ok = hipMemcpy(h, d, sizeof h, hipMemcpyDeviceToHost) == hipSuccess;
  }
  if (d) (void)hipFree(d);
  for (int x = 0; ok && x < 16; x++) ok = h[x] == (x < 8 ? 8u : 0u);
  if (!ok) {
    st.single_queue = true;
    if (debug_enabled()) fprintf(stderr, "blosc_amd: workgroups are not dealt round-robin to 8 XCDs here; using one task queue and unfused filters\n");
  }
}

static void atfork_prepare() { g_pick_mu.lock(); for (int i = 0; i < kMaxCtx; i++) g_ctx[i].mu.lock(); }
static void atfork_parent() { for (int i = kMaxCtx - 1; i >= 0; i--) g_ctx[i].mu.unlock(); g_pick_mu.unlock(); }
static void atfork_child() { for (int i = kMaxCtx - 1; i >= 0; i--) g_ctx[i].mu.unlock(); g_pick_mu.unlock(); g_forked = true; }

static int ensure_device(EngineState& st) {
  if (g_forked) {
    fprintf(stderr, "blosc_amd: this process was forked after the library had initialised its HIP device; a device context does not survive fork() - call exec() or use the library only in the parent\n");
    return -1;
  }
  static std::once_flag atfork_once;
  std::call_once(atfork_once, [] { (void)pthread_atfork(atfork_prepare, atfork_parent, atfork_child); });
  const int want_dev = wanted_device();
  if (st.device_ok && want_dev == st.device) { HIP_TRY(hipSetDevice(st.device)); return 0; }
  if (st.device_ok) {
    (void)hipSetDevice(st.device);
    st.dev.release(); st.io.release(); st.enc_tabs.drop(); st.dec_tabs.drop();
    if (st.own) { (void)hipStreamDestroy(st.own); st.own = nullptr; }
    for (auto& p : st.prof_pending) { (void)hipEventDestroy(p.a); (void)hipEventDestroy(p.b); }
    st.prof_pending.clear();
    for (hipEvent_t e : st.ev_pool) (void)hipEventDestroy(e);
    st.ev_pool.clear();
    st.device_ok = false;
  }
  st.device = want_dev;
  int cnt = 0;
  hipError_t e = hipGetDeviceCount(&cnt);
  if (e != hipSuccess || cnt <= 0) {
    if (!g_warned.exchange(true))
      fprintf(stderr, "blosc_amd: no usable HIP device (%s); this library has no CPU path\n",
              e == hipSuccess ? "device count 0" : hipGetErrorString(e));
    return -1;
  }
  if (st.device >= 0) HIP_TRY(hipSetDevice(st.device));
  else { HIP_TRY(hipGetDevice(&st.device)); int none = -1; (void)g_device.compare_exchange_strong(none, st.device); }
  probe_topology(st);
  hipDeviceProp_t pr;
  const bool have_props = hipGetDeviceProperties(&pr, st.device) == hipSuccess;
  st.cus = (have_props && pr.multiProcessorCount > 0) ? pr.multiProcessorCount : 256;
  if (!st.single_queue && !(have_props && (strncmp(pr.gcnArchName, "gfx950", 6) == 0 || strncmp(pr.gcnArchName, "gfx942", 6) == 0))) {
    st.single_queue = true;
    if (debug_enabled()) fprintf(stderr, "blosc_amd: %s is not on the allow-list of the relaxed in-kernel hand-off; using one task queue and unfused filters\n", have_props ? pr.gcnArchName : "(unknown device)");
  }
  st.enc_cost_valid = st.dec_cost_valid = false;
  st.device_ok = true;
  st.device_hint.store(st.device, std::memory_order_relaxed);
  return 0;
}

static hipEvent_t prof_event(EngineState& st) {
  if (!st.ev_pool.empty()) { hipEvent_t e = st.ev_pool.back(); st.ev_pool.pop_back(); return e; }
  hipEvent_t e; (void)hipEventCreate(&e); return e;
}
struct HostTime { double t[2][6] = {}; long calls[2] = {}; };
static HostTime g_ht;
static double now_ms() { return std::chrono::duration<double, std::milli>(std::chrono::steady_clock::now().time_since_epoch()).count(); }
static std::mutex g_ht_mu;
struct HostPhases {
  const int dir; double last = 0.0;
  explicit HostPhases(int dir_) : dir(dir_) { if (hosttime_on()) { last = now_ms(); std::lock_guard<std::mutex> l(g_ht_mu); g_ht.calls[dir]++; } }
  void mark(int i) {
    if (!hosttime_on()) return;
    const double t = now_ms();
    std::lock_guard<std::mutex> l(g_ht_mu);
    g_ht.t[dir][i] += t - last; last = t;
  }
};
struct ProfScope {
  EngineState& st; hipStream_t s; const char* name; hipEvent_t a{}, b{}; bool on;
  ProfScope(EngineState& st_, hipStream_t s_, const char* n) : st(st_), s(s_), name(n), on(g_prof.load(std::memory_order_relaxed)) {
    if (on) { a = prof_event(st); b = prof_event(st); (void)hipEventRecord(a, s); }
  }
  ~ProfScope() { if (on) { (void)hipEventRecord(b, s); st.prof_pending.push_back({name, a, b}); } }
};
static void prof_collect(EngineState& st) {
  for (auto& p : st.prof_pending) {
    float ms = 0;
    if (hipEventElapsedTime(&ms, p.a, p.b) == hipSuccess) { auto& e = st.prof_acc[p.name]; e.ms += ms; e.launches++; }
    st.ev_pool.push_back(p.a); st.ev_pool.push_back(p.b);
  }
  st.prof_pending.clear();
}

__global__ void k_gather_headers(const uint8_t* const* __restrict__ srcs, uint8_t* __restrict__ out, int n) {
  int i = blockIdx.x * blockDim.x + threadIdx.x;
  if (i >= n * 16) return;
  out[i] = srcs[i >> 4][i & 15];
}

static unsigned persistent_grid(const EngineState& st, size_t nitems, int waves_per_cu) {
  const int cus = st.cus > 0 ? st.cus : 256;
  size_t g = (size_t)cus * (size_t)waves_per_cu;
  if (nitems < g) g = nitems;
  return (unsigned)(g < 8 ? 8 : g);
}

static dim3 grid1(size_t n, int per) { return dim3((unsigned)((n + per - 1) / per)); }

static bool fused_typesize(int T) { return T >= 2 && T <= 32; }
static bool fused_fast_typesize(int T) { return T == 8 || T == 4 || T == 2 || T == 16; }
static bool bitunshuffle_fused_host(int T) { return T == 1 || T == 2 || T == 4 || T == 8; }

static void order_signature(const std::vector<BlockDesc>& blocks, const uint32_t* cost, bool valid, std::vector<int>& sig) {
  bool seen[257] = {false};
  for (const BlockDesc& b : blocks) seen[b.nstreams < 0 ? 0 : (b.nstreams > 256 ? 256 : b.nstreams)] = true;
  sig.clear();
  std::vector<int> order; int nheavy = 0;
  for (int T = 2; T <= 256; T++) {
    if (!seen[T]) continue;
    plane_order(cost, valid && sched_enabled(), T, order, &nheavy);
    std::sort(order.begin(), order.begin() + (nheavy < T ? nheavy : T));
    sig.push_back(T); sig.push_back(nheavy); sig.insert(sig.end(), order.begin(), order.begin() + (nheavy < T ? nheavy : 0));
  }
}

static int call_stream(EngineState& st, bool host_buffers, hipStream_t* stream) {
  if (!host_buffers || *stream != (hipStream_t)0 || ctx_count() == 1) return 0;
  if (!st.own) HIP_TRY(hipStreamCreateWithFlags(&st.own, hipStreamNonBlocking));
  *stream = st.own;
  return 0;
}

static int filter_tile_count(int32_t elems, int per_tile) { const int t = (elems + per_tile - 1) / per_tile; return t < 1 ? 1 : t; }

constexpr size_t kTicketGap = 32;
constexpr size_t kEncTicketWords = 16;
constexpr size_t kDecTicketWords = 8;
static size_t ticket_offset(size_t nchunks) { return sizeof(int32_t) * nchunks + kTicketGap; }

struct HostStaging {
  const bool host;
  size_t in_bytes = 0, out_bytes = 0, in_at = 0, out_at = 0;
  uint8_t *in_base = nullptr, *out_base = nullptr;
  void add(size_t in, size_t out) { if (host) { in_bytes = align_up(in_bytes, 256) + in; out_bytes = align_up(out_bytes, 256) + out; } }
  int reserve(DeviceArena& io) {
    if (!host) return 0;
    const size_t out_off = align_up(in_bytes + 256, 256);
    if (io.ensure(out_off + out_bytes + 512)) return -1;
    in_base = io.base; out_base = io.base + out_off; return 0;
  }
  int stage(ChunkDesc& c, const void* src, size_t in, size_t out, hipStream_t stream) {
    if (!host) return 0;
    in_at = align_up(in_at, 256); out_at = align_up(out_at, 256);
    HIP_TRY(hipMemcpyAsync(in_base + in_at, src, in, hipMemcpyHostToDevice, stream));
    c.src = in_base + in_at; c.dst = out_base + out_at;
    in_at += in; out_at += out; return 0;
  }
  int collect(int n, const Job* jobs, const std::vector<ChunkDesc>& chunks, const std::vector<uint8_t>& live, const int* results, hipStream_t stream) {
    if (!host) return 0;
    for (int i = 0; i < n; i++)
      if (live[(size_t)i] && results[i] > 0) HIP_TRY(hipMemcpyAsync(jobs[i].dst, chunks[(size_t)i].dst, (size_t)results[i], hipMemcpyDeviceToHost, stream));
    HIP_TRY(hipStreamSynchronize(stream));
    return 0;
  }
};

#ifdef BAMD_PROFILE_DECODE
struct StreamProfile {
  uint32_t* d = nullptr; const char* path; size_t bytes; hipStream_t stream;
  StreamProfile(const char* switch_name, size_t nstr, hipStream_t s) : path(getenv(switch_name)), bytes(nstr * 64), stream(s) {
    if (path && hipMalloc((void**)&d, bytes) == hipSuccess) (void)hipMemsetAsync(d, 0, bytes, stream);
  }
  ~StreamProfile() {
    if (!d) return;
    std::vector<uint32_t> h(bytes / 4);
    (void)hipStreamSynchronize(stream); (void)hipMemcpy(h.data(), d, bytes, hipMemcpyDeviceToHost); (void)hipFree(d);
    FILE* f = fopen(path, "wb");
    if (f) { fwrite(h.data(), 4, h.size(), f); fclose(f); }
  }
};
#define BAMD_STREAM_PROFILE(var, switch_name, nstr) StreamProfile var(switch_name, nstr, stream)
#define BAMD_PROF_ARG(var) , var.d
#else
#define BAMD_STREAM_PROFILE(var, switch_name, nstr)
#define BAMD_PROF_ARG(var)
#endif

struct EncVariant {
  int mode = ENC_LZ; const char* name = "k_encode_streams";
  int waves_per_cu = 0;
  bool zstd = false, zdyn = false;
  int detect = 0;
};
static EncVariant encoder_variant(int codec, int clevel) {
  EncVariant v;
  const bool zstd = codec == kZstd, zlibc = codec == kZlib;
  const bool hc = codec == kLZ4HC && lz4hc_search_enabled();
  const bool ztab = zstd && zstd_tables_enabled();
  const bool zsearch = (zstd && zstd_search_enabled(clevel)) || (zlibc && zlib_search_enabled());
  const bool zhuf = zstd && (ztab || zsearch) && zstd_huffman_enabled();
  const int enc_wpc_lz = (zstd || zlibc) ? ENC_WAVES_PER_CU : ENC_LZ_WAVES_PER_CU;
  v.waves_per_cu = zsearch ? (160 * 1024) / (HC_TAB_BYTES + ZS_LDS_BYTES) : (hc ? HC_WAVES_PER_CU : enc_wpc_lz);
  v.zstd = zstd;
  v.zdyn = zlibc && zlib_dynamic_enabled();
  v.detect = (!zstd && !zlibc && periodic_enabled()) ? 1 : 0;
  v.name = zstd ? "k_zstd_encode" : (zlibc ? "k_zlib_encode" : (hc ? "k_lz4hc_encode" : "k_encode_streams"));
  if (zstd && zsearch) v.mode = zhuf ? ENC_ZSTD_HCH : ENC_ZSTD_HC;
  else if (zstd && ztab) v.mode = zhuf ? ENC_ZSTD_TH : ENC_ZSTD_T;
  else if (zstd) v.mode = ENC_ZSTD;
  else if (zlibc && v.zdyn) v.mode = zsearch ? ENC_ZLIB_DYN_HC : ENC_ZLIB_DYN;
  else if (zlibc && zsearch) v.mode = ENC_ZLIB_HC;
  else if (zlibc) v.mode = ENC_ZLIB;
  else if (hc) v.mode = ENC_HC;
  else v.mode = ENC_LZ;
  return v;
}
constexpr int kEncModes = 11;

struct EncodeBatch {
  std::vector<ChunkDesc> chunks; std::vector<uint8_t> live;
  std::vector<uint8_t> variant;
  EncVariant variants[kEncModes]; bool present[kEncModes] = {false}; int ngroups = 0;
  EngineState::TableKey key;
  size_t nstr = 0, filt_bytes = 0, stage_bytes = 0;
  int tiles_shuf = 0, tiles_bit = 0; bool any_shuf = false, any_bit = false;
  explicit EncodeBatch(int n) : chunks((size_t)n), live((size_t)n, 0), variant((size_t)n, (uint8_t)kEncModes) {}
};

static bool add_encode_chunk(const CompressParams& p, const Job& job, int i, int n, bool may_fuse, EncodeBatch& B, int* result) {
  ChunkDesc& c = B.chunks[(size_t)i];
  std::vector<BlockDesc>& blocks = B.key.blocks;
  memset(&c, 0, sizeof c);
  c.mode = CH_SKIP;
  size_t nbytes = job.srcsize, destsize = job.dstsize, typesize = p.typesize;
  const int codec = p.codec;
  *result = 0;
  if (nbytes > (size_t)kMaxBufferSize || destsize < (size_t)kMaxOverhead) return false;
  if (destsize - kMaxOverhead > nbytes) destsize = nbytes + kMaxOverhead;
  if (p.clevel < 0 || p.clevel > 9 || (p.doshuffle != 0 && p.doshuffle != 1 && p.doshuffle != 2) || typesize == 0) { *result = -10; return false; }
  if (typesize > (size_t)kMaxTypeSize) typesize = 1;
  if (codec != kBloscLZ && codec != kLZ4 && codec != kLZ4HC && codec != kZlib && codec != kZstd) { *result = -5; return false; }
  const int32_t T = (int32_t)typesize, nb = (int32_t)nbytes;
  const int32_t bs = compute_blocksize(p.clevel, T, nb, p.forced_blocksize, codec, p.splitmode);
  const int32_t leftover = nb % bs, nblocks = nb / bs + (leftover > 0 ? 1 : 0);
  const bool memcpyed = (p.clevel == 0) || (nb < kMinBufferSize);
  const int split = split_block(codec, T, bs, p.splitmode);
  int flags = ((!split) << 4) | (codec_to_format(codec) << 5);
  if (memcpyed) flags |= kFlagMemcpyed;
  if (p.doshuffle == 1) flags |= kFlagShuffle;
  if (p.doshuffle == 2) flags |= kFlagBitShuffle;
  if (memcpyed && (size_t)nb + kMaxOverhead > destsize) return false;

  c.src = (const uint8_t*)job.src; c.dst = (uint8_t*)job.dst;
  c.nbytes = nb; c.cbytes = (int32_t)destsize; c.blocksize = bs; c.typesize = T;
  c.nblocks = nblocks; c.leftover = leftover; c.nsplits = split ? T : 1;
  c.fmt = codec_to_format(codec); c.clevel = (codec == kLZ4HC) ? 9 : p.clevel; c.hdr_flags = flags;
  c.mode = 0;
  c.first_block = (int32_t)blocks.size(); c.first_stream = (int32_t)B.nstr;
  if (memcpyed) c.mode |= CH_MEMCPYED;
  else if (p.doshuffle == 1 && T > 1) { c.mode |= CH_SHUFFLE; if (fused_typesize(T) && fuse_enabled() && may_fuse) c.mode |= CH_FUSED_SHUF; }
  else if (p.doshuffle == 2) { c.mode |= CH_BITSHUFFLE; if (bitunshuffle_fused_host(T) && fuse_enabled() && may_fuse) c.mode |= CH_FUSED_SHUF; }
  const bool filtered = (c.mode & (CH_SHUFFLE | CH_BITSHUFFLE)) != 0;
  if (filtered && !(c.mode & CH_FUSED_SHUF)) {
    if (c.mode & CH_SHUFFLE) { B.any_shuf = true; B.tiles_shuf = std::max(B.tiles_shuf, filter_tile_count(bs / T, shuffle_tile_elems(T))); }
    else { B.any_bit = true; B.tiles_bit = std::max(B.tiles_bit, filter_tile_count(bs / T, bitshuffle_tile_elems(T))); }
  }
  if (blocks.capacity() < blocks.size() + (size_t)nblocks) blocks.reserve(std::max(blocks.size() + (size_t)nblocks, (size_t)(n - i) * (size_t)nblocks + blocks.size()));
  for (int32_t j = 0; j < nblocks; j++) {
    BlockDesc b;
    b.chunk = i; b.blk = j; b.first_stream = (int32_t)B.nstr;
    const bool last = (j == nblocks - 1) && leftover > 0;
    b.nstreams = memcpyed ? 0 : ((split && !last) ? T : 1);
    b.bsize = last ? leftover : bs; b.flags = 0;
    B.nstr += (size_t)b.nstreams;
    blocks.push_back(b);
  }
  if (!memcpyed) {
    if (filtered) B.filt_bytes = align_up(B.filt_bytes, 256) + (size_t)nb;
    B.stage_bytes = align_up(B.stage_bytes, 256) + (size_t)nb;
  }
  return true;
}

int engine_compress_batch(const CompressParams* params, bool per_chunk, int n, const Job* jobs, int* results, bool device_ptrs,
                          hipStream_t stream, const PackedBuffer* packed) {
  if (n <= 0) return 0;
  if (packed && !device_ptrs) return -1;
  CtxGuard ctx; EngineState& st = *ctx.st;
  if (ensure_device(st) || call_stream(st, !device_ptrs, &stream)) return -1;
  HostPhases ht(0);
  EncodeBatch B(n);
  HostStaging io{!device_ptrs};
  std::vector<ChunkDesc>& chunks = B.chunks;
  int8_t variant_of[6][10]; memset(variant_of, -1, sizeof variant_of);
  for (int i = 0; i < n; i++) {
    const CompressParams& p = params[per_chunk ? i : 0];
    B.live[(size_t)i] = add_encode_chunk(p, jobs[i], i, n, !st.single_queue, B, &results[i]);
    if (!B.live[(size_t)i]) continue;
    io.add((size_t)chunks[(size_t)i].nbytes, (size_t)chunks[(size_t)i].cbytes);
    if (chunks[(size_t)i].mode & CH_MEMCPYED) continue;
    int8_t& m = variant_of[p.codec][p.clevel];
    if (m < 0) { const EncVariant v = encoder_variant(p.codec, p.clevel); m = (int8_t)v.mode; B.variants[v.mode] = v; }
    B.variant[(size_t)i] = (uint8_t)m;
    if (!B.present[m]) { B.present[m] = true; B.ngroups++; }
  }
  const size_t nblk = B.key.blocks.size(), nstr = B.nstr;
  const bool feedback = B.ngroups <= 1;
  const bool cost_valid = feedback && st.enc_cost_valid;
  const size_t ngrp = (size_t)(B.ngroups > 0 ? B.ngroups : 1);
  ht.mark(0);
  EngineState::TableCache& tc = st.enc_tabs;
  B.key.nq = st.single_queue ? 1 : 8;
  B.key.modes.resize((size_t)n);
  for (int i = 0; i < n; i++) B.key.modes[(size_t)i] = (chunks[(size_t)i].mode & CH_FUSED_SHUF) | (B.variant[(size_t)i] < kEncModes ? (uint32_t)(B.variant[(size_t)i] + 1) << 8 : 0u);
  order_signature(B.key.blocks, st.enc_cost, cost_valid, B.key.order);
  Carver pc;
  if (tc.begin("compress", B.key, 0, 0, pc, [&](EngineState::TableCache& t) {
        t.groups.clear();
        std::vector<int32_t> q;
        for (int m = 0; m < kEncModes; m++) {
          if (!B.present[m]) continue;
          size_t sh_at = 0;
          build_encode_queues(B.key.blocks, chunks, st.enc_cost, cost_valid, q, B.key.nq, &sh_at, B.ngroups > 1 ? B.variant.data() : nullptr, m);
          t.groups.push_back({m, t.queues.size(), t.queues.size() + sh_at, q[8]});
          t.queues.insert(t.queues.end(), q.begin(), q.end());
        }
      })) return -1;
  Carver cv;
  const size_t o_chunks = cv.take(sizeof(ChunkDesc) * (size_t)n);
  const size_t o_streams = cv.take(sizeof(StreamDesc) * (nstr ? nstr : 1));
  const size_t o_blkoff = cv.take(sizeof(int32_t) * (nblk ? nblk : 1));
  const size_t o_results = cv.take(ticket_offset((size_t)n) + sizeof(uint32_t) * kEncTicketWords * ngrp);
  const size_t o_ready = cv.take(sizeof(uint32_t) * (nblk ? nblk : 1));
  const size_t o_cost = cv.take(sizeof(uint32_t) * kCostWords * ngrp);
  const size_t clear_bytes = cv.off - o_results;
  const size_t o_filt = cv.take(B.filt_bytes + 256);
  const size_t o_stage = cv.take(B.stage_bytes + 256);
  size_t o_ctabs[kEncModes] = {0}, o_seqbufs[kEncModes] = {0};
  bool any_zstd = false;
  for (const EngineState::EncGroup& g : tc.groups) {
    const EncVariant& v = B.variants[g.mode];
    const size_t zwaves = (v.zstd || v.zdyn) ? (size_t)(st.cus > 0 ? st.cus : 256) * (size_t)v.waves_per_cu : 0;
    if (v.zstd) { o_ctabs[g.mode] = cv.take(sizeof(zenc::CTabs) + 64); any_zstd = true; }
    if (zwaves) o_seqbufs[g.mode] = cv.take(zwaves * (v.zdyn ? (size_t)ZD_SCRATCH_U64 : (size_t)ZS_SEQCAP) * sizeof(uint64_t) + 64);
  }
  const size_t o_offsets = packed ? cv.take(sizeof(uint64_t) * ((size_t)n + 1)) : 0;
  if (st.dev.ensure(cv.off)) return -1;
  uint8_t* D = st.dev.base;
  if (any_zstd) {
    static zenc::CTabs host_tabs; static bool built = false;
    if (!built) { zenc::build_predefined(host_tabs); built = true; }
    for (const EngineState::EncGroup& g : tc.groups)
      if (B.variants[g.mode].zstd) HIP_TRY(hipMemcpyAsync(D + o_ctabs[g.mode], &host_tabs, sizeof host_tabs, hipMemcpyHostToDevice, stream));
  }
  if (io.reserve(st.io)) return -1;
  {
    size_t fo = 0, so = 0;
    for (int i = 0; i < n; i++) {
      if (!B.live[(size_t)i]) continue;
      ChunkDesc& c = chunks[(size_t)i];
      if (io.stage(c, jobs[i].src, (size_t)c.nbytes, (size_t)c.cbytes, stream)) return -1;
      if (c.mode & CH_MEMCPYED) continue;
      const bool filtered = (c.mode & (CH_SHUFFLE | CH_BITSHUFFLE)) != 0;
      if (filtered) { fo = align_up(fo, 256); c.filt = D + o_filt + fo; fo += (size_t)c.nbytes; }
      so = align_up(so, 256); c.stage = D + o_stage + so; so += (size_t)c.nbytes;
    }
  }
  ht.mark(1);
  const size_t p_chunks = pc.take(sizeof(ChunkDesc) * (size_t)n);
  const size_t p_results = pc.take(sizeof(int32_t) * (size_t)n);
  const size_t p_cost = pc.take(sizeof(uint32_t) * kCostWords * ngrp);
  const size_t p_offsets = packed ? pc.take(sizeof(uint64_t) * ((size_t)n + 1)) : 0;
  if (st.pin.ensure(pc.off)) return -1;
  uint8_t* P = st.pin.base;
  memcpy(P + p_chunks, chunks.data(), sizeof(ChunkDesc) * (size_t)n);
  if (tc.upload(B.key, P, stream)) return -1;
  HIP_TRY(hipMemsetAsync(D + o_results, 0, clear_bytes, stream));
  HIP_TRY(hipMemcpyAsync(D + o_chunks, P + p_chunks, sizeof(ChunkDesc) * (size_t)n, hipMemcpyHostToDevice, stream));

  ChunkDesc* d_chunks = (ChunkDesc*)(D + o_chunks); BlockDesc* d_blocks = tc.d_blocks(); StreamDesc* d_streams = (StreamDesc*)(D + o_streams);
  int32_t* d_blkoff = (int32_t*)(D + o_blkoff); int32_t* d_results = (int32_t*)(D + o_results);
  uint32_t* d_tickets = (uint32_t*)(D + o_results + ticket_offset((size_t)n));
  ht.mark(2);
  if (nstr) hipLaunchKernelGGL(k_encode_plan, grid1(nblk, 256), dim3(256), 0, stream, d_chunks, d_blocks, d_streams, (int)nblk);
  if (B.any_shuf && nblk) {
    ProfScope ps(st, stream, "k_shuffle");
    hipLaunchKernelGGL(k_shuffle, dim3((unsigned)nblk, (unsigned)B.tiles_shuf), dim3(FT_THREADS), 0, stream, d_chunks, d_blocks);
  }
  if (B.any_bit && nblk) {
    ProfScope ps(st, stream, "k_bitshuffle");
    hipLaunchKernelGGL(k_bitfilter_fast<0>, dim3((unsigned)nblk, (unsigned)B.tiles_bit), dim3(FT_THREADS), 0, stream, d_chunks, d_blocks);
    hipLaunchKernelGGL(k_bitshuffle, dim3((unsigned)nblk, (unsigned)B.tiles_bit), dim3(FT_THREADS), 0, stream, d_chunks, d_blocks, 1);
  }
  for (size_t k = 0; nstr && k < tc.groups.size(); k++) {
    const EngineState::EncGroup& g = tc.groups[k];
    const EncVariant& v = B.variants[g.mode];
    if (g.ntasks <= 0) continue;
    ProfScope ps(st, stream, v.name);
    const int32_t* d_qoff = tc.d_qoff() + g.q_at; const int32_t* d_qlist = d_qoff + 9; const int32_t* d_shoff = tc.d_qoff() + g.sh_at;
    uint32_t* d_ticket = d_tickets + kEncTicketWords * k;
    uint32_t* d_cost = (uint32_t*)(D + o_cost) + kCostWords * k;
    uint32_t* d_ready = (uint32_t*)(D + o_ready);
    uint64_t* d_seqbufs = (v.zstd || v.zdyn) ? (uint64_t*)(D + o_seqbufs[g.mode]) : nullptr;
    const zenc::CTabs* d_ctabs = v.zstd ? (const zenc::CTabs*)(D + o_ctabs[g.mode]) : nullptr;
    const int detect = v.detect;
    const dim3 grid(persistent_grid(st, (size_t)g.ntasks, v.waves_per_cu)), block(64 * ENC_WAVES);
    BAMD_STREAM_PROFILE(prof, "BLOSC_AMD_ENC_PROFILE", nstr);
#define BAMD_ENC_LAUNCH(MODE) case MODE: hipLaunchKernelGGL(k_encode_streams_t<MODE>, grid, block, 0, stream, d_streams, d_ticket, d_qlist, d_qoff, d_shoff, d_chunks, d_blocks, d_ready, d_cost, st.single_queue ? 1 : 0, d_seqbufs, d_ctabs, detect BAMD_PROF_ARG(prof)); break
    switch (g.mode) {
      BAMD_ENC_LAUNCH(ENC_ZSTD_HCH); BAMD_ENC_LAUNCH(ENC_ZSTD_HC); BAMD_ENC_LAUNCH(ENC_ZSTD_TH); BAMD_ENC_LAUNCH(ENC_ZSTD_T); BAMD_ENC_LAUNCH(ENC_ZSTD);
      BAMD_ENC_LAUNCH(ENC_ZLIB_DYN_HC); BAMD_ENC_LAUNCH(ENC_ZLIB_DYN); BAMD_ENC_LAUNCH(ENC_ZLIB_HC); BAMD_ENC_LAUNCH(ENC_ZLIB);
      BAMD_ENC_LAUNCH(ENC_HC); BAMD_ENC_LAUNCH(ENC_LZ);
    }
#undef BAMD_ENC_LAUNCH
  }
  if (!packed) {
    ProfScope ps(st, stream, "k_chunk_scan");
    hipLaunchKernelGGL(k_chunk_scan, dim3((unsigned)n), dim3(SCAN_THREADS), 0, stream, d_chunks, d_blocks, d_streams, d_blkoff, d_results);
  } else {
    uint64_t* d_offsets = (uint64_t*)(D + o_offsets);
    {
      ProfScope ps(st, stream, "k_chunk_scan");
      hipLaunchKernelGGL(k_chunk_scan_packed, dim3((unsigned)n), dim3(SCAN_THREADS), 0, stream, d_chunks, d_blocks, d_streams, d_blkoff, d_results);
    }
    ProfScope ps(st, stream, "k_packed_layout");
    hipLaunchKernelGGL(k_packed_layout, dim3(1), dim3(SCAN_THREADS), 0, stream, d_chunks, d_results, n, (uint8_t*)packed->base, (uint64_t)packed->size,
                       (uint64_t)packed->align, d_offsets);
    hipLaunchKernelGGL(k_packed_headers, dim3((unsigned)n), dim3(SCAN_THREADS), 0, stream, d_chunks, d_blkoff, d_results, d_offsets, (uint64_t)packed->size);
  }
  if (nblk) {
    ProfScope ps(st, stream, "k_chunk_compact");
    hipLaunchKernelGGL(k_chunk_compact, dim3((unsigned)nblk), dim3(COMPACT_THREADS), 0, stream, d_chunks, d_blocks, d_streams, d_blkoff);
  }
  HIP_TRY(hipGetLastError());
  HIP_TRY(hipMemcpyAsync(P + p_results, d_results, sizeof(int32_t) * (size_t)n, hipMemcpyDeviceToHost, stream));
  HIP_TRY(hipMemcpyAsync(P + p_cost, D + o_cost, sizeof(uint32_t) * kCostWords * ngrp, hipMemcpyDeviceToHost, stream));
  if (packed) HIP_TRY(hipMemcpyAsync(P + p_offsets, D + o_offsets, sizeof(uint64_t) * ((size_t)n + 1), hipMemcpyDeviceToHost, stream));
  ht.mark(3);
  HIP_TRY(hipStreamSynchronize(stream));
  ht.mark(4);
  prof_collect(st);
  for (size_t k = 0; nstr && k < tc.groups.size(); k++)
    if (check_done((const uint32_t*)(P + p_cost) + kCostWords * k, (size_t)tc.groups[k].ntasks, 0, "compress")) return -1;
  if (packed) for (int i = 0; i <= n; i++) packed->offsets[i] = (size_t)((const uint64_t*)(P + p_offsets))[i];
  tc.commit(B.key);
  if (feedback && nstr >= 4096) { memcpy(st.enc_cost, P + p_cost, sizeof st.enc_cost); st.enc_cost_valid = true; }
  const int32_t* r = (const int32_t*)(P + p_results);
  for (int i = 0; i < n; i++) if (B.live[(size_t)i]) results[i] = r[i];
  return io.collect(n, jobs, chunks, B.live, results, stream);
}

static int classify_for_decompress(const Header& h, size_t srcsize, size_t destsize, int* res, int* fmt) {
  if (h.nbytes == 0) { *res = 0; return 0; }
  if (h.blocksize <= 0 || (size_t)h.blocksize > destsize || h.blocksize > kMaxBlockSize || h.typesize <= 0) { *res = -1; return 0; }
  if (h.version != kVersionFormat) { *res = -1; return 0; }
  if (h.flags & kFlagReserved) { *res = -1; return 0; }
  const bool neg = h.nbytes < 0;
  if (!neg && (size_t)h.nbytes > destsize) { *res = -1; return 0; }
  if (srcsize && (h.cbytes < 0 || (size_t)h.cbytes > srcsize)) { *res = -1; return 0; }
  if (h.flags & kFlagMemcpyed) {
    if ((int32_t)((uint32_t)h.nbytes + (uint32_t)kMaxOverhead) != h.cbytes) { *res = -1; return 0; }
    *fmt = 0;
    if (neg) { *res = 0; return 0; }
    return 1;
  }
  const int f = (h.flags & 0xe0) >> 5;
  if (f != FMT_BLOSCLZ && f != FMT_LZ4 && f != FMT_ZLIB && f != FMT_ZSTD) { *res = -5; return 0; }
  if (h.versionlz != 1) { *res = -9; return 0; }
  *fmt = f;
  int32_t nblocks = h.nbytes / h.blocksize + ((h.nbytes % h.blocksize) > 0 ? 1 : 0);
  if (nblocks > (h.cbytes - 16) / 4) { *res = -1; return 0; }
  if (neg) { *res = 0; return 0; }
  return 1;
}

static int fetch_headers(EngineState& st, int n, const Job* jobs, bool device_ptrs, hipStream_t stream,
                         std::vector<Header>& hdrs) {
  hdrs.resize((size_t)n);
  if (!device_ptrs) {
    for (int i = 0; i < n; i++) hdrs[(size_t)i] = parse_header((const uint8_t*)jobs[i].src);
    return 0;
  }
  if (st.dev.ensure(16)) return -1;
  Carver cv;
  const size_t o_ptrs = cv.take(sizeof(void*) * (size_t)n);
  const size_t o_hdr = cv.take(16 * (size_t)n);
  if (st.pin.ensure(cv.off)) return -1;
  const void** pp = (const void**)(st.pin.base + o_ptrs);
  bool any_short = false;
  for (int i = 0; i < n; i++) { const bool sh = jobs[i].srcsize && jobs[i].srcsize < (size_t)kMaxOverhead; any_short |= sh; pp[i] = sh ? (const void*)st.dev.base : jobs[i].src; }
  if (any_short) HIP_TRY(hipMemsetAsync(st.dev.base, 0, 16, stream));
  hipLaunchKernelGGL(k_gather_headers, grid1((size_t)n * 16, 256), dim3(256), 0, stream,
                     (const uint8_t* const*)(st.pin.base + o_ptrs), st.pin.base + o_hdr, n);
  HIP_TRY(hipGetLastError());
  HIP_TRY(hipStreamSynchronize(stream));
  for (int i = 0; i < n; i++) hdrs[(size_t)i] = parse_header(st.pin.base + o_hdr + 16 * (size_t)i);
  for (int i = 0; i < n; i++) if (jobs[i].srcsize && jobs[i].srcsize < (size_t)kMaxOverhead) { hdrs[(size_t)i] = Header{}; hdrs[(size_t)i].nbytes = -1; hdrs[(size_t)i].version = -1; }
  return 0;
}

static void add_decode_chunk(const Header& h, int fmt, int chunk_index, int32_t j0, int32_t j1,
                             ChunkDesc& c, std::vector<BlockDesc>& blocks, size_t& nstreams) {
  memset(&c, 0, sizeof c);
  const int32_t T = h.typesize, bs = h.blocksize;
  c.nbytes = h.nbytes; c.cbytes = h.cbytes; c.blocksize = bs; c.typesize = T;
  c.nblocks = h.nbytes / bs + ((h.nbytes % bs) ? 1 : 0);
  c.leftover = h.nbytes % bs;
  c.fmt = fmt;
  const bool dont_split = (h.flags & kFlagDontSplit) != 0;
  const bool split = !dont_split && T <= kMaxSplits && bs / T >= kMinBufferSize;
  c.nsplits = split ? T : 1;
  c.mode = 0;
  if (h.flags & kFlagMemcpyed) c.mode |= CH_MEMCPYED;
  else if ((h.flags & kFlagShuffle) && T > 1) c.mode |= CH_SHUFFLE;
  else if (h.flags & kFlagBitShuffle) c.mode |= CH_BITSHUFFLE;
  c.first_block = (int32_t)blocks.size();
  c.first_stream = (int32_t)nstreams;
  if (c.mode & CH_MEMCPYED) return;
  for (int32_t j = j0; j < j1; j++) {
    BlockDesc b;
    b.chunk = chunk_index; b.blk = j; b.first_stream = (int32_t)nstreams;
    const bool last = (j == c.nblocks - 1) && c.leftover > 0;
    b.nstreams = (split && !last) ? T : 1;
    b.bsize = last ? c.leftover : bs; b.flags = fmt == FMT_ZSTD ? BLK_Z : (fmt == FMT_ZLIB ? (BLK_Z | BLK_ZLIB) : 0);
    nstreams += (size_t)b.nstreams;
    blocks.push_back(b);
  }
}

struct DecodeLaunch {
  ChunkDesc* d_chunks; BlockDesc* d_blocks; StreamDesc* d_streams; int32_t* d_status; uint32_t* d_ticket; uint32_t* d_blkdone;
  size_t clear_bytes;
  uint32_t* d_spans; uint8_t* d_pat;
  uint32_t* d_cost;
  uint32_t* d_zticket; bool any_zstd;
  bool any_zlib;
  const int32_t* d_zqlist; const int32_t* d_zqoff; size_t nstr_zlib;
  ZMeta* d_zmeta; ptrdiff_t zseq_delta;
  ZgLds* d_zgscr;
  ZcTab* d_zctab;
  const int32_t* d_qlist; const int32_t* d_qoff;
  size_t nblk, nstr; int nchunks;
  bool any_shuf, any_bit, any_copy; int tiles_shuf, tiles_bit;
  size_t nstr_queued;
};

struct DecodeShape {
  int nchunks; size_t nblk, nstr;
  size_t filt_bytes;
  size_t zlit_bytes;
  bool any_zstd, two_phase;
  size_t out_bytes = 0;
  size_t extra_bytes = 0;
};
struct DecodeAreas { uint8_t *filt, *zlit, *out, *extra; };
static int decode_workspace(EngineState& st, const DecodeShape& s, DecodeLaunch& L, DecodeAreas& A) {
  const size_t n = (size_t)s.nchunks, nblk1 = s.nblk ? s.nblk : 1, nstr1 = s.nstr ? s.nstr : 1;
  const int zstd2 = (s.any_zstd && s.two_phase) ? zstd2_mode() : 0;
  const bool use_zctab = zstd2 == 2 && BAMD_ZSTD_SEQ_KERNEL && !BAMD_ZSTD_LDS_FSE;
  Carver cv;
  const size_t o_chunks = cv.take(sizeof(ChunkDesc) * n);
  const size_t o_streams = cv.take(sizeof(StreamDesc) * nstr1);
  const size_t o_blkdone = ticket_offset(n) + sizeof(uint32_t) * kDecTicketWords;
  const size_t o_status = cv.take(o_blkdone + sizeof(uint32_t) * nblk1);
  const size_t o_cost = cv.take(sizeof(uint32_t) * kCostWords);
  L.clear_bytes = cv.off - o_status;
  const size_t o_spans = cv.take(8 * nstr1);
  const size_t o_pat = cv.take(span_enabled() ? (size_t)2048 * nstr1 : 256);
  const size_t o_filt = cv.take(s.filt_bytes + 256);
  const size_t o_zlit = cv.take(s.zlit_bytes + 256);
  const size_t o_zseq = cv.take(s.zlit_bytes + 512);
  const size_t o_zmeta = cv.take(s.any_zstd && s.two_phase ? sizeof(ZMeta) * nstr1 : 64);
  const size_t o_zticket = cv.take(64);
  const size_t o_zgscr = cv.take(zstd2 == 2 ? sizeof(ZgLds) * nstr1 : 64);
  const size_t o_zctab = cv.take(use_zctab ? sizeof(ZcTab) * nstr1 : 64);
  const size_t o_out = cv.take(s.out_bytes ? s.out_bytes + 256 : 0);
  const size_t o_extra = cv.take(s.extra_bytes);
  if (st.dev.ensure(cv.off)) return -1;
  uint8_t* D = st.dev.base;
  A = DecodeAreas{D + o_filt, D + o_zlit, D + o_out, D + o_extra};
  L.d_chunks = (ChunkDesc*)(D + o_chunks); L.d_streams = (StreamDesc*)(D + o_streams);
  L.d_status = (int32_t*)(D + o_status);
  L.d_ticket = (uint32_t*)(D + o_status + ticket_offset(n));
  L.d_blkdone = (uint32_t*)(D + o_status + o_blkdone);
  L.d_cost = (uint32_t*)(D + o_cost);
  L.d_spans = span_enabled() ? (uint32_t*)(D + o_spans) : nullptr; L.d_pat = D + o_pat;
  L.d_zticket = (uint32_t*)(D + o_zticket);
  L.d_zmeta = (s.any_zstd && s.two_phase) ? (ZMeta*)(D + o_zmeta) : nullptr; L.zseq_delta = (ptrdiff_t)o_zseq - (ptrdiff_t)o_zlit + 8;
  L.d_zgscr = zstd2 == 2 ? (ZgLds*)(D + o_zgscr) : nullptr;
  L.d_zctab = use_zctab ? (ZcTab*)(D + o_zctab) : nullptr;
  L.nblk = s.nblk; L.nstr = s.nstr; L.nchunks = s.nchunks;
  return 0;
}
static int clear_decode_counters(const DecodeLaunch& L, hipStream_t stream) {
  HIP_TRY(hipMemsetAsync(L.d_status, 0, L.clear_bytes, stream));
  if (L.any_zstd || L.any_zlib) HIP_TRY(hipMemsetAsync(L.d_zticket, 0, 64, stream));
  return 0;
}

static int read_back_decode(const DecodeLaunch& L, void* status, void* cost, hipStream_t stream) {
  HIP_TRY(hipMemcpyAsync(status, L.d_status, sizeof(int32_t) * (size_t)L.nchunks, hipMemcpyDeviceToHost, stream));
  HIP_TRY(hipMemcpyAsync(cost, L.d_cost, sizeof(uint32_t) * kCostWords, hipMemcpyDeviceToHost, stream));
  return 0;
}
static int decode_feedback(EngineState& st, const DecodeLaunch& L, const void* cost, const char* what) {
  if (check_done((const uint32_t*)cost, L.nstr_queued, L.any_zstd ? L.nstr : 0, what, L.nstr_zlib)) return -1;
  if (L.nstr >= 4096) { memcpy(st.dec_cost, cost, sizeof st.dec_cost); st.dec_cost_valid = true; }
  return 0;
}

static int launch_decode(EngineState& st, const DecodeLaunch& L, hipStream_t stream) {
  if (L.nblk) {
    {
      ProfScope ps(st, stream, "k_decode_plan");
      hipLaunchKernelGGL(k_decode_plan, grid1(L.nblk, 256), dim3(256), 0, stream, L.d_chunks, L.d_blocks, L.d_streams, L.d_status, (int)L.nblk);
    }
    if (L.nstr_queued) {
      ProfScope ps(st, stream, "k_decode_streams");
      const dim3 dgrid(persistent_grid(st, L.nstr_queued ? L.nstr_queued : 1, DEC_WAVES_PER_CU));
      BAMD_STREAM_PROFILE(prof, "BLOSC_AMD_DEC_PROFILE", L.nstr);
      hipLaunchKernelGGL(k_decode_streams, dgrid, dim3(64 * DEC_WAVES), 0, stream, L.d_streams, L.d_status, L.d_ticket, L.d_qlist, L.d_qoff, L.d_chunks, L.d_blocks, L.d_blkdone, L.d_spans, L.d_pat, L.d_cost, st.single_queue ? 1 : 0 BAMD_PROF_ARG(prof));
    }
    const int zstd2 = zstd2_mode();
    const uint32_t* d_taken = nullptr;
    if (L.any_zstd && L.d_zmeta && zstd2) {
      {
        ProfScope ps(st, stream, "k_zstd_entropy");
        if (zstd2 == 2 && L.d_zgscr) hipLaunchKernelGGL(k_zstd_entropy_t<true>, grid1(L.nstr, ZG_FRAMES), dim3(64), 0, stream, L.d_streams, (int)L.nstr, L.d_chunks, L.d_blocks, L.d_zmeta, L.zseq_delta, L.d_zgscr, L.d_zctab);
        else hipLaunchKernelGGL(k_zstd_entropy_t<false>, grid1(L.nstr, ZG_FRAMES), dim3(64), 0, stream, L.d_streams, (int)L.nstr, L.d_chunks, L.d_blocks, L.d_zmeta, L.zseq_delta, (ZgLds*)nullptr, (ZcTab*)nullptr);
      }
      if (zstd2 == 2 && L.d_zgscr && BAMD_ZSTD_SEQ_KERNEL && !BAMD_ZSTD_LDS_FSE) {
        ProfScope ps(st, stream, "k_zstd_seq");
        hipLaunchKernelGGL(k_zstd_seq, grid1(L.nstr, ZSEQ_FRAMES), dim3(64), 0, stream, L.d_streams, (int)L.nstr, L.d_chunks, L.d_blocks, L.d_zmeta, L.zseq_delta, L.d_zgscr, L.d_zctab);
      }
      {
        ProfScope ps(st, stream, "k_zstd_exec");
        hipLaunchKernelGGL(k_zstd_exec, dim3(persistent_grid(st, L.nstr, ZEXEC_WAVES_PER_CU)), dim3(64), 0, stream, L.d_streams, (int)L.nstr, L.d_status, L.d_zticket + 1,
                           L.d_chunks, L.d_blocks, L.d_zmeta, L.zseq_delta);
      }
      d_taken = (const uint32_t*)L.d_zmeta;
    }
    if (L.any_zstd) {
      ProfScope ps(st, stream, "k_zstd_streams");
      BAMD_STREAM_PROFILE(zprof, "BLOSC_AMD_ZSTD_PROFILE", L.nstr);
      hipLaunchKernelGGL(k_zstd_streams, dim3(persistent_grid(st, L.nstr, ZSTD_WAVES_PER_CU)), dim3(64), 0, stream, L.d_streams, (int)L.nstr, L.d_status,
                         L.d_zticket, L.d_chunks, L.d_blocks, L.d_cost + 257, d_taken BAMD_PROF_ARG(zprof));
    }
    if (L.any_zlib) {
      ProfScope ps(st, stream, "k_zlib_streams");
      hipLaunchKernelGGL(k_zlib_streams, dim3(persistent_grid(st, L.nstr_zlib ? L.nstr_zlib : 1, ZLIB_WAVES_PER_CU)), dim3(64), 0, stream, L.d_streams, L.d_status,
                         L.d_zticket + 8, L.d_zqlist, L.d_zqoff, L.d_cost + 259, L.d_chunks, L.d_blocks, L.d_blkdone, st.single_queue ? 1 : 0);
    }
    if (L.any_shuf) {
      ProfScope ps(st, stream, "k_unshuffle");
      hipLaunchKernelGGL(k_unshuffle, dim3((unsigned)L.nblk, (unsigned)L.tiles_shuf), dim3(FT_THREADS), 0, stream, L.d_chunks, L.d_blocks);
    }
    if (L.any_bit) {
      ProfScope ps(st, stream, "k_bitunshuffle");
      hipLaunchKernelGGL(k_bitfilter_fast<1>, dim3((unsigned)L.nblk, (unsigned)L.tiles_bit), dim3(FT_THREADS), 0, stream, L.d_chunks, L.d_blocks);
      hipLaunchKernelGGL(k_bitunshuffle, dim3((unsigned)L.nblk, (unsigned)L.tiles_bit), dim3(FT_THREADS), 0, stream, L.d_chunks, L.d_blocks, 1);
    }
  }
  if (L.any_copy) {
    ProfScope ps(st, stream, "k_copy_chunks");
    hipLaunchKernelGGL(k_copy_chunks, dim3(64, (unsigned)L.nchunks), dim3(COMPACT_THREADS), 0, stream, L.d_chunks, kMaxOverhead);
  }
  HIP_TRY(hipGetLastError());
  return 0;
}

static void filter_tiles(ChunkDesc& c, DecodeLaunch& L, bool may_fuse) {
  const int32_t T = c.typesize, N = c.blocksize / T;
  const bool zfmt = c.fmt == FMT_ZSTD || c.fmt == FMT_ZLIB;
  if ((c.mode & CH_SHUFFLE) && fuse_enabled() && may_fuse && (zfmt ? (fused_fast_typesize(T) && (c.fmt == FMT_ZLIB || c.nsplits == 1)) : fused_typesize(T))) { c.mode |= CH_FUSED_UNSHUF; return; }
  if (c.mode & CH_SHUFFLE) {
    L.any_shuf = true;
    L.tiles_shuf = std::max(L.tiles_shuf, filter_tile_count(N, shuffle_tile_elems(T)));
  } else if ((c.mode & CH_BITSHUFFLE) && bitunshuffle_fused_host(T) && fuse_enabled() && may_fuse && !zfmt) {
    c.mode |= CH_FUSED_BITUNSH;
  } else if (c.mode & CH_BITSHUFFLE) {
    L.any_bit = true;
    L.tiles_bit = std::max(L.tiles_bit, filter_tile_count(N, bitshuffle_tile_elems(T)));
  }
}

static bool place_packed_chunks(int n, const std::vector<Header>& hdrs, const PackedBuffer& pk, std::vector<Job>& jobs, int* results) {
  constexpr size_t kAnySize = (size_t)INT32_MAX;
  size_t off = 0;
  for (int i = 0; i < n; i++) {
    const Header& h = hdrs[(size_t)i];
    int res = -1, fmt = 0;
    const bool valid = classify_for_decompress(h, jobs[(size_t)i].srcsize, kAnySize, &res, &fmt) == 1;
    const size_t width = valid ? (size_t)h.nbytes : 0;
    pk.offsets[i] = off;
    jobs[(size_t)i].dst = pk.base ? (uint8_t*)pk.base + off : nullptr;
    jobs[(size_t)i].dstsize = valid ? (off + width <= pk.size ? width : 0) : kAnySize;
    if (!pk.base) results[i] = valid ? h.nbytes : res;
    off += width;
  }
  pk.offsets[n] = off;
  return pk.base != nullptr;
}

int engine_chunk_headers(int n, const void* const* src, Header* out, hipStream_t stream) {
  if (n <= 0) return 0;
  CtxGuard ctx; EngineState& st = *ctx.st;
  if (ensure_device(st)) return -1;
  std::vector<Job> jobs((size_t)n);
  for (int i = 0; i < n; i++) jobs[(size_t)i] = Job{src[i], nullptr, 0, 0};
  std::vector<Header> hdrs;
  if (fetch_headers(st, n, jobs.data(), true, stream, hdrs)) return -1;
  std::copy(hdrs.begin(), hdrs.end(), out);
  return 0;
}

int engine_decompress_batch(int n, const Job* jobs, int* results, bool device_ptrs, hipStream_t stream, const PackedBuffer* packed) {
  if (n <= 0) return 0;
  if (packed && !device_ptrs) return -1;
  CtxGuard ctx; EngineState& st = *ctx.st;
  if (ensure_device(st) || call_stream(st, !device_ptrs, &stream)) return -1;
  HostPhases ht(1);
  std::vector<Header> hdrs;
  if (fetch_headers(st, n, jobs, device_ptrs, stream, hdrs)) return -1;
  ht.mark(0);
  std::vector<Job> placed;
  if (packed) {
    placed.assign(jobs, jobs + n);
    if (!place_packed_chunks(n, hdrs, *packed, placed, results)) return 0;
    jobs = placed.data();
  }
  std::vector<ChunkDesc> chunks((size_t)n);
  std::vector<uint8_t> live((size_t)n, 0);
  EngineState::TableKey key;
  std::vector<BlockDesc>& blocks = key.blocks;
  HostStaging io{!device_ptrs};
  size_t nstr = 0, nstr_z = 0, nstr_zlib = 0, filt_bytes = 0, zlit_bytes = 0;
  DecodeLaunch L{};
  for (int i = 0; i < n; i++) {
    ChunkDesc& c = chunks[(size_t)i];
    const Header& h = hdrs[(size_t)i];
    memset(&c, 0, sizeof c);
    c.mode = CH_SKIP;
    int res = -1, fmt = 0;
    if (!classify_for_decompress(h, jobs[i].srcsize, jobs[i].dstsize, &res, &fmt)) { results[i] = res; continue; }
    add_decode_chunk(h, fmt, i, 0, h.nbytes / h.blocksize + ((h.nbytes % h.blocksize) ? 1 : 0), c, blocks, nstr);
    c.src = (const uint8_t*)jobs[i].src; c.dst = (uint8_t*)jobs[i].dst;
    live[(size_t)i] = 1;
    results[i] = c.nbytes;
    if (c.mode & CH_MEMCPYED) L.any_copy = true;
    filter_tiles(c, L, !st.single_queue);
    if (c.mode & (CH_SHUFFLE | CH_BITSHUFFLE)) filt_bytes = align_up(filt_bytes, 256) + (size_t)c.nblocks * filt_block_stride(c);
    if (c.fmt == FMT_ZSTD && !(c.mode & CH_MEMCPYED)) { L.any_zstd = true; zlit_bytes = align_up(zlit_bytes, 256) + (size_t)c.nbytes; }
    if (c.fmt == FMT_ZLIB && !(c.mode & CH_MEMCPYED)) L.any_zlib = true;
    if (c.fmt == FMT_ZSTD || c.fmt == FMT_ZLIB) nstr_z += nstr - (size_t)c.first_stream;
    if (c.fmt == FMT_ZLIB) nstr_zlib += nstr - (size_t)c.first_stream;
    io.add((size_t)c.cbytes, (size_t)c.nbytes);
  }
  const size_t nblk = blocks.size();
  DecodeAreas A;
  if (decode_workspace(st, DecodeShape{n, nblk, nstr, filt_bytes, zlit_bytes, L.any_zstd,  true}, L, A)) return -1;
  if (io.reserve(st.io)) return -1;
  {
    size_t fo = 0, zo = 0;
    for (int i = 0; i < n; i++) {
      if (!live[(size_t)i]) continue;
      ChunkDesc& c = chunks[(size_t)i];
      if (io.stage(c, jobs[i].src, (size_t)c.cbytes, (size_t)c.nbytes, stream)) return -1;
      if (c.mode & (CH_SHUFFLE | CH_BITSHUFFLE)) { fo = align_up(fo, 256); c.filt = A.filt + fo; fo += (size_t)c.nblocks * filt_block_stride(c); }
      if (c.fmt == FMT_ZSTD && !(c.mode & CH_MEMCPYED)) { zo = align_up(zo, 256); c.stage = A.zlit + zo; zo += (size_t)c.nbytes; }
    }
  }
  EngineState::TableCache& tc = st.dec_tabs;
  key.nq = st.single_queue ? 1 : 8;
  order_signature(blocks, st.dec_cost, st.dec_cost_valid, key.order);
  Carver pc;
  const size_t queue_words = 9 + (nstr ? nstr : 1);
  if (tc.begin("decompress", key, queue_words, queue_words, pc, [&](EngineState::TableCache& t) {
        build_xcd_queues(blocks, nstr, st.dec_cost, st.dec_cost_valid, t.queues, key.nq);
        if (L.any_zlib) build_xcd_queues(blocks, nstr, nullptr, false, t.zqueues, key.nq, BLK_ZLIB);
      })) return -1;
  const size_t p_chunks = pc.take(sizeof(ChunkDesc) * (size_t)n);
  const size_t p_status = pc.take(sizeof(int32_t) * (size_t)n);
  const size_t p_cost = pc.take(sizeof(uint32_t) * kCostWords);
  if (st.pin.ensure(pc.off)) return -1;
  uint8_t* P = st.pin.base;
  memcpy(P + p_chunks, chunks.data(), sizeof(ChunkDesc) * (size_t)n);
  HIP_TRY(hipMemcpyAsync(L.d_chunks, P + p_chunks, sizeof(ChunkDesc) * (size_t)n, hipMemcpyHostToDevice, stream));
  if (tc.upload(key, P, stream) || clear_decode_counters(L, stream)) return -1;
  L.d_blocks = tc.d_blocks();
  L.d_qoff = tc.d_qoff(); L.d_qlist = L.d_qoff + 9;
  L.d_zqoff = tc.d_zqoff(); L.d_zqlist = L.d_zqoff + 9; L.nstr_zlib = nstr_zlib;
  L.nstr_queued = nstr - nstr_z;
  ht.mark(2);
  if (launch_decode(st, L, stream) || read_back_decode(L, P + p_status, P + p_cost, stream)) return -1;
  ht.mark(3);
  HIP_TRY(hipStreamSynchronize(stream));
  ht.mark(4);
  prof_collect(st);
  if (nblk && decode_feedback(st, L, P + p_cost, "decompress")) return -1;
  tc.commit(key);
  if (debug_cost_enabled()) {
    fprintf(stderr, "[blosc_amd] decode plane costs:");
    for (int k = 0; k < 16; k++) fprintf(stderr, " %u", st.dec_cost[k]);
    fprintf(stderr, "\n");
  }
  const int32_t* stt = (const int32_t*)(P + p_status);
  for (int i = 0; i < n; i++) if (live[(size_t)i] && stt[i] < 0) results[i] = -1;
  return io.collect(n, jobs, chunks, live, results, stream);
}

static int classify_for_getitem(const Header& h, int* res, int* fmt) {
  if (h.version != kVersionFormat) { *res = -9; return 0; }
  if (h.blocksize <= 0 || h.blocksize > h.nbytes || h.blocksize > kMaxBlockSize || h.typesize <= 0) { *res = -1; return 0; }
  *fmt = 0;
  if (h.flags & kFlagMemcpyed) {
    if (h.nbytes + kMaxOverhead != h.cbytes) { *res = -1; return 0; }
    return 1;
  }
  const int f = (h.flags & 0xe0) >> 5;
  if (f != FMT_BLOSCLZ && f != FMT_LZ4 && f != FMT_ZLIB && f != FMT_ZSTD) { *res = -5; return 0; }
  if (h.versionlz != 1) { *res = -9; return 0; }
  *fmt = f;
  const int32_t nblocks = h.nbytes / h.blocksize + ((h.nbytes % h.blocksize) ? 1 : 0);
  if (nblocks >= (h.cbytes - 16) / 4) { *res = -1; return 0; }
  return 1;
}

constexpr size_t kGetitemPassBytes = (size_t)256 << 20;
static std::atomic<size_t> g_getitem_pass_bytes{kGetitemPassBytes};
void engine_getitem_pass_bytes(size_t bytes) { g_getitem_pass_bytes.store(bytes ? bytes : kGetitemPassBytes); }

namespace {
struct BlockRun { int32_t j0, j1; size_t off; int32_t entry0; };
struct RangeChunk {
  int fmt = 0, verdict = -1, pass = 0;
  bool usable = false, memcpyed = false;
  std::vector<BlockRun> runs;
};
struct PlacedRange { int slot = -1; int64_t lo = 0; uint32_t want = 0; int32_t j0 = 0, j1 = 0; uint8_t* dst = nullptr; };
}

static size_t merge_runs(std::vector<BlockRun>& runs, size_t bs) {
  std::sort(runs.begin(), runs.end(), [](const BlockRun& a, const BlockRun& b) { return a.j0 < b.j0; });
  size_t m = 0, bytes = 0;
  for (size_t i = 1; i < runs.size(); i++) {
    if (runs[i].j0 <= runs[m].j1) runs[m].j1 = std::max(runs[m].j1, runs[i].j1);
    else runs[++m] = runs[i];
  }
  if (!runs.empty()) runs.resize(m + 1);
  for (const BlockRun& r : runs) bytes += align_up((size_t)(r.j1 - r.j0) * bs, 256);
  return bytes;
}

static int getitem_pass(EngineState& st, int pass, std::vector<RangeChunk>& uc, const std::vector<Header>& hdrs, const std::vector<Job>& jobs,
                        int nranges, const std::vector<PlacedRange>& pr, int* results, hipStream_t stream) {
  std::vector<ChunkDesc> entries; std::vector<BlockDesc> blocks;
  size_t nstr = 0, nstr_z = 0, nstr_zlib = 0, span = 0;
  bool any_filt = false;
  DecodeLaunch L{};
  for (size_t k = 0; k < uc.size(); k++) {
    RangeChunk& u = uc[k];
    if (u.pass != pass) continue;
    const Header& h = hdrs[k];
    for (BlockRun& r : u.runs) {
      r.off = span; r.entry0 = (int32_t)entries.size();
      span += align_up((size_t)(r.j1 - r.j0) * (size_t)h.blocksize, 256);
      for (int32_t j = r.j0; j < r.j1; j++) {
        ChunkDesc c;
        const size_t s0 = nstr;
        add_decode_chunk(h, u.fmt, (int)entries.size(), j, j + 1, c, blocks, nstr);
        filter_tiles(c, L, !st.single_queue);
        if (c.mode & (CH_SHUFFLE | CH_BITSHUFFLE)) any_filt = true;
        if (c.fmt == FMT_ZSTD) L.any_zstd = true;
        if (c.fmt == FMT_ZLIB) { L.any_zlib = true; nstr_zlib += nstr - s0; }
        if (c.fmt == FMT_ZSTD || c.fmt == FMT_ZLIB) nstr_z += nstr - s0;
        entries.push_back(c);
      }
    }
  }
  const size_t n = entries.size(), nblk = blocks.size();
  std::vector<GatherRange> gr((size_t)nranges);
  std::vector<uint32_t> tile_first((size_t)nranges + 1, 0);
  for (int r = 0; r < nranges; r++) {
    GatherRange& g = gr[(size_t)r];
    memset(&g, 0, sizeof g);
    const PlacedRange& p = pr[(size_t)r];
    uint32_t tiles = 0;
    if (p.slot >= 0 && uc[(size_t)p.slot].pass == pass) { g.nbytes = p.want; g.dst = p.dst; tiles = (p.want + GI_TILE - 1) / GI_TILE; }
    tile_first[(size_t)r + 1] = tile_first[(size_t)r] + tiles;
  }
  const uint32_t ntiles = tile_first[(size_t)nranges];
  if (!nblk && !ntiles) return 0;
  const int nq = st.single_queue ? 1 : 8;
  std::vector<int32_t> queues, zqueues;
  build_xcd_queues(blocks, nstr, st.dec_cost, st.dec_cost_valid, queues, nq);
  if (L.any_zlib) build_xcd_queues(blocks, nstr, nullptr, false, zqueues, nq, BLK_ZLIB);
  Carver tv;
  const size_t t_chunks = tv.take(sizeof(ChunkDesc) * (n ? n : 1));
  const size_t t_blocks = tv.take(sizeof(BlockDesc) * (nblk ? nblk : 1));
  const size_t t_queues = tv.take(sizeof(int32_t) * queues.size());
  const size_t t_zqueues = tv.take(sizeof(int32_t) * (zqueues.size() + 1));
  const size_t t_ranges = tv.take(sizeof(GatherRange) * (size_t)nranges);
  const size_t t_tiles = tv.take(sizeof(uint32_t) * ((size_t)nranges + 1));
  const size_t table_bytes = tv.off;
  const size_t p_status = tv.take(sizeof(int32_t) * (n ? n : 1));
  const size_t p_cost = tv.take(sizeof(uint32_t) * kCostWords);
  DecodeAreas A;
  if (decode_workspace(st, DecodeShape{(int)n, nblk, nstr, any_filt ? span : 0, L.any_zstd ? span : 0, L.any_zstd,  false,  span, table_bytes}, L, A)) return -1;
  if (st.pin.ensure(tv.off)) return -1;
  uint8_t* P = st.pin.base;
  for (size_t k = 0; k < uc.size(); k++) {
    if (uc[k].pass != pass) continue;
    const size_t bs = (size_t)hdrs[k].blocksize;
    for (const BlockRun& r : uc[k].runs)
      for (int32_t j = r.j0; j < r.j1; j++) {
        ChunkDesc& c = entries[(size_t)(r.entry0 + (j - r.j0))];
        c.src = (const uint8_t*)jobs[k].src;
        c.dst = A.out + r.off - (size_t)r.j0 * bs;
        c.stage = c.fmt == FMT_ZSTD ? A.zlit + r.off - (size_t)r.j0 * bs : nullptr;
        c.filt = (c.mode & (CH_SHUFFLE | CH_BITSHUFFLE)) ? A.filt + r.off - (size_t)r.j0 * filt_block_stride(c) : nullptr;
      }
  }
  for (int r = 0; r < nranges; r++) {
    GatherRange& g = gr[(size_t)r];
    if (!g.nbytes) continue;
    const PlacedRange& p = pr[(size_t)r];
    const RangeChunk& u = uc[(size_t)p.slot];
    if (u.memcpyed) { g.src = (const uint8_t*)jobs[(size_t)p.slot].src + kMaxOverhead + p.lo; continue; }
    auto it = std::upper_bound(u.runs.begin(), u.runs.end(), p.j0, [](int32_t j, const BlockRun& b) { return j < b.j0; });
    const BlockRun& run = *(it - 1);
    g.src = A.out + run.off + (size_t)(p.lo - (int64_t)run.j0 * hdrs[(size_t)p.slot].blocksize);
    g.status0 = run.entry0 + (p.j0 - run.j0); g.nstatus = p.j1 - p.j0;
  }
  memcpy(P + t_chunks, entries.data(), sizeof(ChunkDesc) * n);
  memcpy(P + t_blocks, blocks.data(), sizeof(BlockDesc) * nblk);
  memcpy(P + t_queues, queues.data(), sizeof(int32_t) * queues.size());
  memcpy(P + t_zqueues, zqueues.data(), sizeof(int32_t) * zqueues.size());
  memcpy(P + t_ranges, gr.data(), sizeof(GatherRange) * (size_t)nranges);
  memcpy(P + t_tiles, tile_first.data(), sizeof(uint32_t) * ((size_t)nranges + 1));
  HIP_TRY(hipMemcpyAsync(A.extra, P, table_bytes, hipMemcpyHostToDevice, stream));
  L.d_chunks = (ChunkDesc*)(A.extra + t_chunks); L.d_blocks = (BlockDesc*)(A.extra + t_blocks);
  L.d_qoff = (const int32_t*)(A.extra + t_queues); L.d_qlist = L.d_qoff + 9;
  L.d_zqoff = (const int32_t*)(A.extra + t_zqueues); L.d_zqlist = L.d_zqoff + 9; L.nstr_zlib = nstr_zlib;
  L.nstr_queued = nstr - nstr_z;
  if (nblk) {
    if (clear_decode_counters(L, stream) || launch_decode(st, L, stream) || read_back_decode(L, P + p_status, P + p_cost, stream)) return -1;
  }
  if (ntiles) {
    ProfScope ps(st, stream, "k_getitem_gather");
    hipLaunchKernelGGL(k_getitem_gather, dim3(persistent_grid(st, ntiles, GI_WAVES_PER_CU)), dim3(GI_THREADS), 0, stream,
                       (const GatherRange*)(A.extra + t_ranges), (const uint32_t*)(A.extra + t_tiles), nranges, (const int32_t*)L.d_status);
    HIP_TRY(hipGetLastError());
  }
// ... 273 lines not shown
```

### c-blosc_amd/csrc/k_encode.hip

```cpp
#include <hip/hip_runtime.h>
#include <stdint.h>
#include "dev_types.h"
#include "wave_prims.h"
#include "zstd_enc.h"
#include "deflate_enc.h"

namespace bamd {

#ifdef BAMD_PROFILE_DECODE
#define EPROF_ARG , DecProf& prof_
#define EPROF_PASS , prof_
#else
#define EPROF_ARG
#define EPROF_PASS
#endif

#include "enc_lz.h"
#include "enc_lz4p.h"
#include "enc_zstd.h"
#include "enc_zlib.h"
#include "enc_shuffle.h"

enum { ENC_LZ = 0, ENC_ZSTD = 1, ENC_ZLIB = 2, ENC_HC = 3, ENC_ZSTD_T = 4, ENC_ZSTD_HC = 5, ENC_ZLIB_HC = 6, ENC_ZSTD_TH = 7, ENC_ZSTD_HCH = 8,
       ENC_ZLIB_DYN = 9, ENC_ZLIB_DYN_HC = 10 };
constexpr bool enc_mode_hc(int mode) { return mode == ENC_HC || mode == ENC_ZSTD_HC || mode == ENC_ZLIB_HC || mode == ENC_ZSTD_HCH || mode == ENC_ZLIB_DYN_HC; }
constexpr bool enc_mode_zlib(int mode) { return mode == ENC_ZLIB || mode == ENC_ZLIB_HC || mode == ENC_ZLIB_DYN || mode == ENC_ZLIB_DYN_HC; }
constexpr bool enc_mode_zstd(int mode) { return mode == ENC_ZSTD || mode == ENC_ZSTD_T || mode == ENC_ZSTD_HC || mode == ENC_ZSTD_TH || mode == ENC_ZSTD_HCH; }
#ifndef BAMD_ENC_HELP
#define BAMD_ENC_HELP 256
#endif
template <int MODE>
__device__ __attribute__((noinline)) void encode_one_stream(StreamDesc* sd_, enc_entry_t* tab_, const ChunkDesc* chunks_, uint32_t* blk_ready_, int lane,
                                                            const BlockDesc* blocks_, uint32_t sid_, uint32_t* plane_cost_, uint64_t* seqbuf_
#ifdef BAMD_PROFILE_DECODE
                                                            , uint32_t* profslot_
#endif
                                                            ) {
  StreamDesc* sd; enc_entry_t* tab; const ChunkDesc* chunks; uint32_t* blk_ready; const BlockDesc* blocks; uint32_t sid; uint32_t* plane_cost; uint64_t* seqbuf;
#ifdef BAMD_PROFILE_DECODE
  uint32_t* profslot;
#endif
  PROF_DECL
#ifdef BAMD_PROFILE_DECODE
  prof_.c[4] = 0; prof_.c[5] = 0;
#endif
  sd = uni_gp(sd_); tab = uni_gp(tab_); chunks = uni_gp(chunks_); blk_ready = uni_gp(blk_ready_); blocks = uni_gp(blocks_);
  plane_cost = uni_gp(plane_cost_); seqbuf = uni_gp(seqbuf_); sid = uni(sid_);
#ifdef BAMD_PROFILE_DECODE
  profslot = uni_gp(profslot_);
#endif
  const uint32_t n = uni((uint32_t)sd->in_size), cap = uni((uint32_t)sd->out_size);
  const uint32_t aux = uni((uint32_t)sd->aux);
  const int clevel = (int)(aux & 15u);
  if (uni(chunks[uni((uint32_t)sd->chunk)].mode) & CH_FUSED_SHUF) {
    const uint32_t gb = aux >> 4;
    while (__hip_atomic_load(&blk_ready[gb], __ATOMIC_RELAXED, __HIP_MEMORY_SCOPE_AGENT) == 0u) __builtin_amdgcn_s_sleep(16);
    __builtin_amdgcn_fence(__ATOMIC_ACQUIRE, "agent");
  }
  PROF_LAP(13);
  const uint64_t cost_t0 = __builtin_amdgcn_s_memtime();
  uint32_t r;
  const int32_t hint = (int32_t)uni((uint32_t)sd->result);
  if (MODE == ENC_ZSTD) r = seqbuf ? zstd_encode_wave(uni_ptr(as_global(sd->in)), n, uni_ptr(as_global(sd->out)), cap, clevel, tab, (BAMD_GAS uint64_t*)seqbuf, lane EPROF_PASS) : 0u;
  else if (MODE == ENC_ZSTD_HCH) r = seqbuf ? zstd_encode_wave<true, true, true>(uni_ptr(as_global(sd->in)), n, uni_ptr(as_global(sd->out)), cap, clevel, tab, (BAMD_GAS uint64_t*)seqbuf, lane EPROF_PASS) : 0u;
  else if (MODE == ENC_ZSTD_TH) r = seqbuf ? zstd_encode_wave<true, false, true>(uni_ptr(as_global(sd->in)), n, uni_ptr(as_global(sd->out)), cap, clevel, tab, (BAMD_GAS uint64_t*)seqbuf, lane EPROF_PASS) : 0u;
  else if (MODE == ENC_ZSTD_HC) r = seqbuf ? zstd_encode_wave<true, true>(uni_ptr(as_global(sd->in)), n, uni_ptr(as_global(sd->out)), cap, clevel, tab, (BAMD_GAS uint64_t*)seqbuf, lane EPROF_PASS) : 0u;
  else if (MODE == ENC_ZLIB_DYN) r = seqbuf ? zlib_dyn_encode_wave<false>(uni_ptr(as_global(sd->in)), n, uni_ptr(as_global(sd->out)), cap, clevel, tab, (BAMD_GAS uint64_t*)seqbuf, lane EPROF_PASS) : 0u;
  else if (MODE == ENC_ZLIB_DYN_HC) r = seqbuf ? zlib_dyn_encode_wave<true>(uni_ptr(as_global(sd->in)), n, uni_ptr(as_global(sd->out)), cap, clevel, tab, (BAMD_GAS uint64_t*)seqbuf, lane EPROF_PASS) : 0u;
  else if (MODE == ENC_ZLIB_HC) r = zlib_encode_wave<true>(uni_ptr(as_global(sd->in)), n, uni_ptr(as_global(sd->out)), cap, clevel, tab, lane EPROF_PASS);
  else if (MODE == ENC_ZSTD_T) r = seqbuf ? zstd_encode_wave<true>(uni_ptr(as_global(sd->in)), n, uni_ptr(as_global(sd->out)), cap, clevel, tab, (BAMD_GAS uint64_t*)seqbuf, lane EPROF_PASS) : 0u;
  else if (MODE == ENC_ZLIB) r = zlib_encode_wave(uni_ptr(as_global(sd->in)), n, uni_ptr(as_global(sd->out)), cap, clevel, tab, lane EPROF_PASS);
  else if (hint < 0) r = emit_periodic_stream(uni_ptr(as_global(sd->in)), n, uni_ptr(as_global(sd->out)), cap, (uint32_t)-hint, uni((uint32_t)sd->fmt) == (uint32_t)FMT_LZ4, lane);
  else if (MODE == ENC_HC) r = lz4hc_encode_wave(uni_ptr(as_global(sd->in)), n, uni_ptr(as_global(sd->out)), cap, tab, lane);
  else if (sd->fmt == FMT_LZ4) r = BAMD_ENC_PAR ? lz4_encode_wave_auto(uni_ptr(as_global(sd->in)), n, uni_ptr(as_global(sd->out)), cap, clevel, tab, lane EPROF_PASS)
                                                : lz_encode_wave<EF_LZ4>(uni_ptr(as_global(sd->in)), n, uni_ptr(as_global(sd->out)), cap, clevel, tab, lane EPROF_PASS);
  else r = lz_encode_wave<EF_BLOSCLZ>(uni_ptr(as_global(sd->in)), n, uni_ptr(as_global(sd->out)), cap, clevel, tab, lane EPROF_PASS);
  if (lane == 0) sd->result = (int32_t)r;
  if (plane_cost && lane == 0) {
    const uint32_t j = sid - (uint32_t)blocks[aux >> 4].first_stream;
    atomicAdd(plane_cost + (j & 255u), (uint32_t)((__builtin_amdgcn_s_memtime() - cost_t0) >> 10));
  }
#ifdef BAMD_PROFILE_DECODE
  prof_.c[15] = (uint32_t)(prof_.t0 >> 6);
  if (lane == 0 && profslot) for (int i_ = 0; i_ < 16; i_++) profslot[i_] = prof_.c[i_];
#endif
}

template <int MODE>
__global__ __launch_bounds__(64 * ENC_WAVES, enc_mode_hc(MODE) ? 2 : ((MODE == ENC_ZSTD_T || MODE == ENC_ZSTD_TH) ? 5 : (MODE == ENC_LZ ? BAMD_ENC_LZ_MINWAVES : BAMD_ENC_MINWAVES))) void k_encode_streams_t(
    StreamDesc* __restrict__ streams, uint32_t* __restrict__ tickets , const int32_t* __restrict__ qlist,
    const int32_t* __restrict__ qoff , const int32_t* __restrict__ shoff , const ChunkDesc* __restrict__ chunks, const BlockDesc* __restrict__ blocks,
    uint32_t* __restrict__ blk_ready, uint32_t* __restrict__ plane_cost, int single_queue,
    uint64_t* __restrict__ seqbufs, const zenc::CTabs* __restrict__ ctabs, int detect_periodic
#ifdef BAMD_PROFILE_DECODE
    , uint32_t* __restrict__ profbuf
#endif
    ) {
  constexpr bool ZSTD = enc_mode_zstd(MODE);
  constexpr int TABBYTES = enc_mode_hc(MODE) ? HC_TAB_BYTES : ENC_TAB_BYTES;
  __shared__ __attribute__((aligned(16))) enc_entry_t tabs[ENC_WAVES][(TABBYTES + (ZSTD ? ZS_LDS_BYTES : (enc_mode_zlib(MODE) ? DFL_LDS_BYTES : (MODE == ENC_LZ ? ENC_SCR_BYTES : 0)))) / 4];
  static_assert(ENC_WAVES == 1, "one stream per wave, one wave per workgroup");
  const int lane = threadIdx.x & 63;
  uint64_t* seqbuf = nullptr;
  if (ZSTD) {
    const uint32_t* g = (const uint32_t*)ctabs;
    for (uint32_t k = (uint32_t)lane; k < sizeof(zenc::CTabs) / 4u; k += 64u) tabs[0][TABBYTES / 4 + k] = g[k];
    seqbuf = seqbufs + (size_t)blockIdx.x * ZS_SEQCAP;
  }
  if (MODE == ENC_ZLIB_DYN || MODE == ENC_ZLIB_DYN_HC) seqbuf = seqbufs + (size_t)blockIdx.x * ZD_SCRATCH_U64;
  const uint32_t xcc = single_queue ? 0u : (__builtin_amdgcn_s_getreg((3 << 11) | 20) & 7u);
  const uint32_t qbase = (uint32_t)qoff[xcc], qlen = (uint32_t)qoff[xcc + 1] - qbase;
  const uint32_t shbase = (uint32_t)shoff[xcc], shlen = (uint32_t)shoff[xcc + 1] - shbase;
  const int32_t* shlist = shoff + 9;
  auto shuffle_one = [&]() -> bool {
    const uint32_t s = take_ticket(tickets + 8 + xcc, lane);
    if (s >= shlen) return false;
    shuffle_block_task(chunks, blocks, uni((uint32_t)shlist[shbase + s]), blk_ready, streams, detect_periodic, lane, (volatile uint32_t*)tabs[0]);
    return true;
  };
  uint32_t t = take_ticket(tickets + xcc, lane);
  uint32_t ndone = 0;
  while (t < qlen) {
    const int32_t task = (int32_t)uni((uint32_t)qlist[qbase + t]);
    if (task < 0) {
      shuffle_one();
    } else {
      const StreamDesc* sd = streams + task;
      if (uni(chunks[uni((uint32_t)sd->chunk)].mode) & CH_FUSED_SHUF) {
        const uint32_t gb = uni((uint32_t)sd->aux) >> 4;
        const ChunkDesc* cd = chunks + uni((uint32_t)sd->chunk);
        bool more = !(uni(cd->mode) & CH_BITSHUFFLE) && shuffle_generic_T(uni((uint32_t)cd->typesize));
        while (__hip_atomic_load(&blk_ready[gb], __ATOMIC_RELAXED, __HIP_MEMORY_SCOPE_AGENT) == 0u) {
          if (BAMD_ENC_HELP && more && __hip_atomic_load(tickets + 8 + xcc, __ATOMIC_RELAXED, __HIP_MEMORY_SCOPE_AGENT) < (single_queue ? gb : gb / 8u) + (uint32_t)BAMD_ENC_HELP) more = shuffle_one();
          else __builtin_amdgcn_s_sleep(16);
        }
      }
#ifdef BAMD_PROFILE_DECODE
      encode_one_stream<MODE>(streams + task, tabs[0], chunks, blk_ready, lane, blocks, (uint32_t)task, plane_cost, seqbuf, profbuf ? profbuf + (size_t)task * 16 : nullptr);
#else
      encode_one_stream<MODE>(streams + task, tabs[0], chunks, blk_ready, lane, blocks, (uint32_t)task, plane_cost, seqbuf);
#endif
    }
    ndone++;
    t = take_ticket(tickets + xcc, lane);
  }
  if (lane == 0 && ndone) atomicAdd(plane_cost + 256, ndone);
}

__global__ __launch_bounds__(256) void k_encode_plan(const ChunkDesc* __restrict__ chunks, const BlockDesc* __restrict__ blocks,
                                                     StreamDesc* __restrict__ streams, int nblocks_total) {
  const int g = (int)(blockIdx.x * blockDim.x + threadIdx.x);
  if (g >= nblocks_total) return;
  const BlockDesc b = blocks[g];
  if (b.nstreams <= 0) return;
  const ChunkDesc& c = chunks[b.chunk];
  const uint8_t* inbase = (c.mode & (CH_SHUFFLE | CH_BITSHUFFLE)) ? c.filt : c.src;
  const int32_t neblock = b.bsize / b.nstreams;
  const size_t at = (size_t)b.blk * (size_t)c.blocksize;
  for (int32_t k = 0; k < b.nstreams; k++) {
    StreamDesc sd;
    sd.in = inbase + at + (size_t)k * (size_t)neblock;
    sd.out = c.stage + at + (size_t)k * (size_t)neblock;
    sd.in_size = neblock; sd.out_size = neblock; sd.chunk = b.chunk; sd.fmt = c.fmt; sd.aux = c.clevel | (int32_t)((uint32_t)g << 4); sd.result = 0;
    streams[(size_t)b.first_stream + k] = sd;
  }
}

constexpr int SCAN_THREADS = 256;

__device__ __forceinline__ void st_i32(gu8* p, int32_t v) { g_st_i32le(p, v); }

template <bool PACKED>
__device__ __forceinline__ void chunk_scan(ChunkDesc* __restrict__ chunks,
                                           const BlockDesc* __restrict__ blocks,
                                           const StreamDesc* __restrict__ streams,
                                           int32_t* __restrict__ blk_off,
                                           int32_t* __restrict__ results) {
  __shared__ int32_t part[SCAN_THREADS];
  __shared__ int32_t carry_s;
  const int cid = blockIdx.x, tid = threadIdx.x;
  ChunkDesc& c = chunks[cid];
  if (c.mode & CH_SKIP) return;
  gu8* d = as_global(c.dst);
  if (c.mode & CH_MEMCPYED) {
    if (tid == 0) {
      if (!PACKED) {
        d[0] = 2; d[1] = 1; d[2] = (uint8_t)c.hdr_flags; d[3] = (uint8_t)c.typesize;
        st_i32(d + 4, c.nbytes); st_i32(d + 8, c.blocksize); st_i32(d + 12, c.nbytes + 16);
      }
      results[cid] = c.nbytes + 16;
    }
    return;
  }
  if (tid == 0) carry_s = 16 + 4 * c.nblocks;
  __syncthreads();
  for (int base = 0; base < c.nblocks; base += SCAN_THREADS) {
    const int j = base + tid;
    int32_t mine = 0;
    if (j < c.nblocks) {
      const BlockDesc b = blocks[c.first_block + j];
      for (int s = 0; s < b.nstreams; s++) {
        const StreamDesc& sd = streams[b.first_stream + s];
        mine += 4 + (sd.result > 0 ? sd.result : sd.in_size);
      }
    }
    part[tid] = mine;
    __syncthreads();
    for (int o = 1; o < SCAN_THREADS; o <<= 1) {
      int32_t v = (tid >= o) ? part[tid - o] : 0;
      __syncthreads();
      part[tid] += v;
      __syncthreads();
    }
    const int32_t carry = carry_s;
    if (j < c.nblocks) {
      int64_t start = (int64_t)carry + part[tid] - mine;
      blk_off[c.first_block + j] = start > 0x7fffffff ? 0x7fffffff : (int32_t)start;
    }
    __syncthreads();
    if (tid == SCAN_THREADS - 1) {
      int64_t nc = (int64_t)carry + part[tid];
      carry_s = nc > 0x7fffffff ? 0x7fffffff : (int32_t)nc;
    }
    __syncthreads();
  }
  const int32_t total = carry_s;
  const int32_t maxbytes = c.cbytes;
  int32_t res;
  uint32_t flags = (uint32_t)c.hdr_flags;
  if (total <= maxbytes) {
    res = total;
    if (!PACKED) for (int j = tid; j < c.nblocks; j += SCAN_THREADS) st_i32(d + 16 + 4 * (size_t)j, blk_off[c.first_block + j]);
  } else if ((int64_t)c.nbytes + 16 <= (int64_t)maxbytes) {
    res = c.nbytes + 16;
    flags |= 0x2u;
    if (tid == 0) c.mode |= CH_MEMCPYED;
  } else {
    res = 0;
    if (tid == 0) c.mode |= CH_SKIP;
  }
  if (tid == 0) {
    if (!PACKED) {
      d[0] = 2;
      d[1] = 1;
      d[2] = (uint8_t)flags; d[3] = (uint8_t)c.typesize;
      st_i32(d + 4, c.nbytes); st_i32(d + 8, c.blocksize); st_i32(d + 12, res);
    }
    results[cid] = res;
  }
}
__global__ __launch_bounds__(SCAN_THREADS) void k_chunk_scan(ChunkDesc* __restrict__ chunks, const BlockDesc* __restrict__ blocks,
                                                            const StreamDesc* __restrict__ streams, int32_t* __restrict__ blk_off,
                                                            int32_t* __restrict__ results) {
  chunk_scan<false>(chunks, blocks, streams, blk_off, results);
}
__global__ __launch_bounds__(SCAN_THREADS) void k_chunk_scan_packed(ChunkDesc* __restrict__ chunks, const BlockDesc* __restrict__ blocks,
                                                                   const StreamDesc* __restrict__ streams, int32_t* __restrict__ blk_off,
                                                                   int32_t* __restrict__ results) {
  chunk_scan<true>(chunks, blocks, streams, blk_off, results);
}

__global__ __launch_bounds__(SCAN_THREADS) void k_packed_layout(ChunkDesc* __restrict__ chunks, int32_t* __restrict__ results, int nchunks,
                                                               uint8_t* dest, uint64_t destsize, uint64_t align ,
                                                               uint64_t* __restrict__ offsets) {
  __shared__ uint64_t part[SCAN_THREADS];
  __shared__ uint64_t carry_s;
  const int tid = threadIdx.x;
  if (tid == 0) carry_s = 0;
  __syncthreads();
  for (int base = 0; base < nchunks; base += SCAN_THREADS) {
    const int i = base + tid;
    uint64_t size = 0, mine = 0;
    if (i < nchunks) {
      const int32_t r = results[i];
      size = r > 0 ? (uint64_t)r : 0;
      mine = (size + align - 1) & ~(align - 1);
    }
    part[tid] = mine;
    __syncthreads();
    for (int o = 1; o < SCAN_THREADS; o <<= 1) {
      uint64_t v = (tid >= o) ? part[tid - o] : 0;
      __syncthreads();
      part[tid] += v;
      __syncthreads();
    }
    const uint64_t carry = carry_s;
    if (i < nchunks) {
      const uint64_t off = carry + part[tid] - mine;
      offsets[i] = off;
      ChunkDesc& c = chunks[i];
      if (!(c.mode & CH_SKIP)) {
        if (off + size <= destsize) c.dst = dest + off;
        else { c.mode |= CH_SKIP; results[i] = 0; }
      }
    }
    __syncthreads();
    if (tid == SCAN_THREADS - 1) carry_s = carry + part[tid];
    __syncthreads();
  }
  if (tid == 0) offsets[nchunks] = carry_s;
}

__global__ __launch_bounds__(SCAN_THREADS) void k_packed_headers(const ChunkDesc* __restrict__ chunks, const int32_t* __restrict__ blk_off,
                                                                const int32_t* __restrict__ results, const uint64_t* __restrict__ offsets,
                                                                uint64_t destsize) {
  const int cid = blockIdx.x, tid = threadIdx.x;
  const ChunkDesc& c = chunks[cid];
  if (c.mode & CH_SKIP) return;
  gu8* d = as_global(c.dst);
  const int32_t res = results[cid];
  const bool memcpyed = (c.mode & CH_MEMCPYED) != 0;
  if (!memcpyed) for (int j = tid; j < c.nblocks; j += SCAN_THREADS) st_i32(d + 16 + 4 * (size_t)j, blk_off[c.first_block + j]);
  if (tid == 0) {
    d[0] = 2; d[1] = 1; d[2] = (uint8_t)((uint32_t)c.hdr_flags | (memcpyed ? 0x2u : 0u)); d[3] = (uint8_t)c.typesize;
    st_i32(d + 4, c.nbytes); st_i32(d + 8, c.blocksize); st_i32(d + 12, res);
  }
  const uint64_t next = offsets[cid + 1] < destsize ? offsets[cid + 1] : destsize;
  for (uint64_t k = offsets[cid] + (uint64_t)res + (uint64_t)tid; k < next; k += SCAN_THREADS) d[k - offsets[cid]] = 0;
}

constexpr int COMPACT_THREADS = 256;

__device__ __forceinline__ void wg_copy(gu8* dst, const gu8* src, uint32_t n) {
  const uint32_t tid = threadIdx.x;
  uint32_t full = n & ~15u;
  for (uint32_t k = tid * 16u; k < full; k += COMPACT_THREADS * 16u) st16u(dst + k, ld16u(src + k));
  for (uint32_t k = full + tid; k < n; k += COMPACT_THREADS) dst[k] = src[k];
}

__global__ __launch_bounds__(COMPACT_THREADS) void k_chunk_compact(const ChunkDesc* __restrict__ chunks,
                                                                  const BlockDesc* __restrict__ blocks,
                                                                  const StreamDesc* __restrict__ streams,
                                                                  const int32_t* __restrict__ blk_off) {
  const BlockDesc b = blocks[blockIdx.x];
  const ChunkDesc& c = chunks[b.chunk];
  if (c.mode & CH_SKIP) return;
  const uint32_t bsize = (uint32_t)b.bsize;
  if (c.mode & CH_MEMCPYED) {
    wg_copy(as_global(c.dst) + 16 + (size_t)b.blk * c.blocksize, as_global(c.src) + (size_t)b.blk * c.blocksize, bsize);
    return;
  }
  uint32_t pos = (uint32_t)blk_off[blockIdx.x];
  for (int s = 0; s < b.nstreams; s++) {
    const StreamDesc& sd = streams[b.first_stream + s];
    const bool raw = sd.result <= 0;
    const uint32_t sz = raw ? (uint32_t)sd.in_size : (uint32_t)sd.result;
    if (threadIdx.x == 0) st_i32(as_global(c.dst) + pos, (int32_t)sz);
    wg_copy(as_global(c.dst) + pos + 4, as_global(raw ? sd.in : (const uint8_t*)sd.out), sz);
    pos += 4u + sz;
  }
}

__global__ __launch_bounds__(COMPACT_THREADS) void k_copy_chunks(const ChunkDesc* __restrict__ chunks, int src_skip) {
  const ChunkDesc& c = chunks[blockIdx.y];
  if (!(c.mode & CH_MEMCPYED) || (c.mode & CH_SKIP)) return;
  const uint64_t per = (uint64_t)COMPACT_THREADS * 16u * 8u;
  for (uint64_t lo = (uint64_t)blockIdx.x * per; lo < (uint64_t)c.nbytes; lo += (uint64_t)gridDim.x * per) {
    uint64_t hi = lo + per < (uint64_t)c.nbytes ? lo + per : (uint64_t)c.nbytes;
    wg_copy(as_global(c.dst) + lo, as_global(c.src) + src_skip + lo, (uint32_t)(hi - lo));
  }
}

}
```

### c-blosc_amd/csrc/queue_order.h

```cpp
#pragma once
#include <atomic>
#include <stdint.h>
#include <stdlib.h>
#include <algorithm>
#include <vector>
#include "dev_types.h"

namespace bamd {

constexpr size_t kEncLookaheadDefault = 32;
inline size_t enc_lookahead() { return kEncLookaheadDefault; }
inline std::atomic<bool>& sched_override_off() { static std::atomic<bool> off{false}; return off; }
inline bool sched_enabled() {
  static const bool env_on = [] { const char* e = getenv("BLOSC_AMD_SCHED"); return !(e && atoi(e) == 0); }();
  return env_on && !sched_override_off().load(std::memory_order_relaxed);
}

inline void plane_order(const uint32_t* cost, bool valid, int T, std::vector<int>& order, int* nheavy) {
  order.resize((size_t)T);
  for (int j = 0; j < T; j++) order[(size_t)j] = j;
  *nheavy = T;
  if (!valid || T <= 1 || T > 256) return;
  std::stable_sort(order.begin(), order.end(), [&](int a, int b) { return cost[a] > cost[b]; });
  const uint32_t mx = cost[order[0]];
  if (mx == 0) return;
  int h = 0;
  while (h < T && cost[order[(size_t)h]] > mx / 2) h++;
  *nheavy = h;
}

inline void build_encode_queues(const std::vector<BlockDesc>& blocks, const std::vector<ChunkDesc>& chunks,
                                const uint32_t* cost, bool cost_valid, std::vector<int32_t>& out, int nq = 8, size_t* sh_at = nullptr,
                                const uint8_t* chunk_group = nullptr, int group = 0) {
  std::vector<int32_t> q[8], sh[8];
  std::vector<uint32_t> mine[8];
  for (int x = 0; x < nq; x++) mine[x].reserve(blocks.size() / (size_t)nq + 1);
  size_t nstr_all = 0;
  for (size_t g = 0; g < blocks.size(); g++) {
    if (blocks[g].nstreams <= 0 || (chunk_group && chunk_group[(size_t)blocks[g].chunk] != group)) continue;
    mine[g % (size_t)nq].push_back((uint32_t)g); nstr_all += (size_t)blocks[g].nstreams;
  }
  std::vector<int> order; int nheavy = 0, lastT = -1;
  for (int x = 0; x < 8; x++) {
    const std::vector<uint32_t>& B = mine[x];
    if (!B.empty()) { q[x].reserve(2 * (nstr_all / (size_t)nq) + B.size() + 64); sh[x].reserve(B.size()); }
    auto push_shuffle = [&](size_t i) {
      if (chunks[(size_t)blocks[B[i]].chunk].mode & CH_FUSED_SHUF) { q[x].push_back(-(int32_t)B[i] - 1); sh[x].push_back((int32_t)B[i]); }
    };
    int maxT = 1;
    const size_t kEncLookahead = enc_lookahead();
    for (size_t i = 0; i < B.size() && i < kEncLookahead; i++) push_shuffle(i);
    for (size_t i = 0; i < B.size(); i++) {
      if (i + kEncLookahead < B.size()) push_shuffle(i + kEncLookahead);
      const BlockDesc& b = blocks[B[i]];
      if (b.nstreams != lastT) { plane_order(cost, cost_valid && sched_enabled(), b.nstreams, order, &nheavy); lastT = b.nstreams; }
      if (b.nstreams > maxT) maxT = b.nstreams;
      for (int k = 0; k < nheavy; k++) q[x].push_back(b.first_stream + order[(size_t)k]);
    }
    for (int k = 1; k < maxT; k++)
      for (size_t i = 0; i < B.size(); i++) {
        const BlockDesc& b = blocks[B[i]];
        if (b.nstreams != lastT) { plane_order(cost, cost_valid && sched_enabled(), b.nstreams, order, &nheavy); lastT = b.nstreams; }
        if (k >= nheavy && k < b.nstreams) q[x].push_back(b.first_stream + order[(size_t)k]);
      }
  }
  out.clear();
  out.reserve(32 + nstr_all + 2 * blocks.size());
  out.assign(9, 0);
  for (int x = 0; x < 8; x++) { out[(size_t)x + 1] = out[(size_t)x] + (int32_t)q[x].size(); }
  for (int x = 0; x < 8; x++) out.insert(out.end(), q[x].begin(), q[x].end());
  if (out.size() == 9) out.push_back(0);
  const size_t at = out.size();
  if (sh_at) *sh_at = at;
  out.resize(at + 9, 0);
  for (int x = 0; x < 8; x++) out[at + (size_t)x + 1] = out[at + (size_t)x] + (int32_t)sh[x].size();
  for (int x = 0; x < 8; x++) out.insert(out.end(), sh[x].begin(), sh[x].end());
}

#ifndef BAMD_DEC_LEAD
#define BAMD_DEC_LEAD 16
#endif
constexpr size_t kDecLead = BAMD_DEC_LEAD;
inline void build_xcd_queues(const std::vector<BlockDesc>& blocks, size_t nstr, const uint32_t* cost, bool cost_valid,
                             std::vector<int32_t>& out, int nq = 8, uint32_t pick = 0u) {
  std::vector<int32_t> q[8];
  std::vector<uint32_t> mine[8];
  for (int x = 0; x < nq; x++) { mine[x].reserve(blocks.size() / (size_t)nq + 1); q[x].reserve(nstr / (size_t)nq + 64); }
  for (size_t g = 0; g < blocks.size(); g++) {
    const uint32_t f = (uint32_t)blocks[g].flags;
    if (blocks[g].nstreams > 0 && (pick ? (f & pick) != 0u : !(f & BLK_Z))) mine[g % (size_t)nq].push_back((uint32_t)g);
  }
  std::vector<int> order; int nheavy = 0, lastT = -1;
  auto prep = [&](const BlockDesc& b) {
    if (b.nstreams != lastT) { plane_order(cost, cost_valid && sched_enabled(), b.nstreams, order, &nheavy); lastT = b.nstreams; }
  };
  for (int x = 0; x < 8; x++) {
    const std::vector<uint32_t>& B = mine[x];
    const size_t lead = B.size() > 2 * kDecLead ? kDecLead : B.size() / 4;
    auto push_heavy = [&](size_t i) { const BlockDesc& b = blocks[B[i]]; prep(b); if (nheavy < b.nstreams) for (int k = 0; k < nheavy; k++) q[x].push_back(b.first_stream + order[(size_t)k]); };
    for (size_t i = 0; i < B.size() && i < lead; i++) push_heavy(i);
    for (size_t i = 0; i < B.size(); i++) {
      if (i + lead < B.size()) push_heavy(i + lead);
      const BlockDesc& b = blocks[B[i]];
      prep(b);
      if (nheavy < b.nstreams) { for (int k = nheavy; k < b.nstreams; k++) q[x].push_back(b.first_stream + order[(size_t)k]); }
      else for (int k = 0; k < b.nstreams; k++) q[x].push_back(b.first_stream + k);
    }
  }
  out.clear();
  out.reserve(10 + nstr);
  out.assign(9, 0);
  for (int x = 0; x < 8; x++) out[(size_t)x + 1] = out[(size_t)x] + (int32_t)q[x].size();
  for (int x = 0; x < 8; x++) out.insert(out.end(), q[x].begin(), q[x].end());
  out.resize(9 + (nstr ? nstr : 1), 0);
}

}
```

Measured before the change: 773.2 GB/s.

## Size persistent grids by LDS granules and occupancy query; halve LZ4 scratch

Persistent-grid widths now come from the granule-rounded LDS footprint and a runtime occupancy query, instead of raw byte division that could overestimate how many workgroups fit per CU. The LZ4 encoder's scratch shrinks from 512 to 256 bytes by packing two-slot entries into one word with a flag bit, so table plus scratch fills whole LDS granules and more encoder waves can be resident. The shuffle lookahead rises from 32 to 96, and per-wave profiling plus occupancy query APIs are added. The packed-scratch change risks correctness in the split-stream path, and the larger lookahead changes shuffle/encode interleaving.

```diff
diff --git a/c-blosc_amd/csrc/blosc_api.hip b/c-blosc_amd/csrc/blosc_api.hip
--- a/c-blosc_amd/csrc/blosc_api.hip
+++ b/c-blosc_amd/csrc/blosc_api.hip
@@ -525,6 +525,12 @@
   return checksum_runs(kind, nruns, jobs, digest_out, stream);
 }
 
+__attribute__((visibility("default"))) int blosc_internal_persistent_grids(int cap, const char** names, int* launched, int* occupancy) {
+  return bamd::engine_persistent_grids(cap, names, launched, occupancy);
+}
+__attribute__((visibility("default"))) int blosc_internal_enc_lz_occupancy(int dynamic_lds) { return bamd::engine_enc_lz_occupancy(dynamic_lds); }
+__attribute__((visibility("default"))) void blosc_internal_last_compress_tasks(unsigned out[3]) { bamd::engine_last_compress_tasks(out); }
+
 __attribute__((visibility("default"))) void blosc_internal_shuffle(const size_t typesize, const size_t blocksize,
                                                                    const uint8_t* src, const uint8_t* dest) {
   if (engine_filter(0, typesize, blocksize, src, (void*)dest) != 0) fprintf(stderr, "blosc_amd: shuffle failed (no GPU?)\n");
diff --git a/c-blosc_amd/csrc/enc_lz.h b/c-blosc_amd/csrc/enc_lz.h
--- a/c-blosc_amd/csrc/enc_lz.h
+++ b/c-blosc_amd/csrc/enc_lz.h
@@ -18,10 +18,16 @@
 #ifndef BAMD_ENC_LZ_MINWAVES
 #define BAMD_ENC_LZ_MINWAVES 6
 #endif
-constexpr int ENC_LDS_WAVES = (160 * 1024) / ENC_TAB_BYTES;
+constexpr int LDS_BYTES_PER_CU = 160 * 1024;
+constexpr int LDS_GRANULE_BYTES = 1280;
+constexpr int lds_occupied(int bytes) { return (bytes + LDS_GRANULE_BYTES - 1) / LDS_GRANULE_BYTES * LDS_GRANULE_BYTES; }
+constexpr int lds_workgroups_per_cu(int bytes) { return bytes > 0 ? LDS_BYTES_PER_CU / lds_occupied(bytes) : 32; }
+constexpr int ENC_LDS_WAVES = lds_workgroups_per_cu(ENC_TAB_BYTES);
 constexpr int ENC_WAVES_PER_CU = ENC_LDS_WAVES < 4 * BAMD_ENC_MINWAVES ? ENC_LDS_WAVES : 4 * BAMD_ENC_MINWAVES;
-constexpr int ENC_LZ_LDS_WAVES = (160 * 1024) / (ENC_TAB_BYTES + 512);
+constexpr int ENC_LZ_SCR_BYTES = 256;
+constexpr int ENC_LZ_LDS_WAVES = lds_workgroups_per_cu(ENC_TAB_BYTES + ENC_LZ_SCR_BYTES);
 constexpr int ENC_LZ_WAVES_PER_CU = ENC_LZ_LDS_WAVES < 4 * BAMD_ENC_LZ_MINWAVES ? ENC_LZ_LDS_WAVES : 4 * BAMD_ENC_LZ_MINWAVES;
+static_assert(lds_occupied(ENC_TAB_BYTES + ENC_LZ_SCR_BYTES) * ENC_LZ_WAVES_PER_CU <= LDS_BYTES_PER_CU, "the LZ4 kernel's workgroups of one CU fit its LDS");
 
 struct EncTable {
   __attribute__((address_space(3))) uint32_t* w;
diff --git a/c-blosc_amd/csrc/enc_lz4p.h b/c-blosc_amd/csrc/enc_lz4p.h
--- a/c-blosc_amd/csrc/enc_lz4p.h
+++ b/c-blosc_amd/csrc/enc_lz4p.h
@@ -1,8 +1,9 @@
 #ifndef BAMD_ENC_PAR
 #define BAMD_ENC_PAR 1
 #endif
-constexpr int ENC_SCR_BYTES = 512;
-static_assert(ENC_LZ_LDS_WAVES == (160 * 1024) / (ENC_TAB_BYTES + ENC_SCR_BYTES), "enc_lz.h sizes the persistent grid with this scratch in mind");
+constexpr int ENC_SCR_BYTES = 256;
+static_assert(ENC_SCR_BYTES == ENC_LZ_SCR_BYTES, "enc_lz.h sizes the persistent grid with this scratch in mind");
+static_assert((ENC_TAB_BYTES + ENC_SCR_BYTES) % LDS_GRANULE_BYTES == 0 || !BAMD_ENC_SPLIT_TAB, "table + scratch fill whole LDS granules");
 #ifndef BAMD_ENC_BACK2
 #define BAMD_ENC_BACK2 1
 #endif
@@ -285,12 +286,12 @@
         PROF_ADD(3, 1);
       }
       scr[lane] = 0u;
-      if (SS) scr[lane + 64] = 0u;
       BAMD_LDS_SYNC();
-      if (valid) scr[cq] = 0x80000000u | (excl + hdr) | (inl << 10) | (w << 17) | (L << 23);
+      if (valid) scr[cq >> SS] = 0x80000000u | (excl + hdr) | (inl << 10) | (w << 17) | (L << 23) | (SS ? (cq & 1u) << 28 : 0u);
       BAMD_LDS_SYNC();
-      const uint32_t myw = scr[lq];
-      const uint32_t myw1 = SS ? scr[lq + 1u] : 0u;
+      const uint32_t pw = scr[lane];
+      const uint32_t myw = (SS && (pw & (1u << 28))) ? 0u : pw;
+      const uint32_t myw1 = (SS && (pw & (1u << 28))) ? pw : 0u;
       const uint64_t fm = __ballot((myw >> 31) != 0u);
       uint32_t s;
       bool has;
@@ -305,7 +306,7 @@
         s = 63u - (uint32_t)__builtin_clzll(below | 1ull);
         has = below != 0ull;
       }
-      const uint32_t inf = scr[s];
+      const uint32_t inf = scr[s >> SS];
       BAMD_LDS_SYNC();
       {
         const uint32_t tpos = op + excl;
diff --git a/c-blosc_amd/csrc/engine.h b/c-blosc_amd/csrc/engine.h
--- a/c-blosc_amd/csrc/engine.h
+++ b/c-blosc_amd/csrc/engine.h
@@ -46,6 +46,10 @@
 
 int engine_filter(int kind, size_t typesize, size_t blocksize, const void* src, void* dst);
 
+int engine_persistent_grids(int cap, const char** names, int* launched, int* occupancy);
+int engine_enc_lz_occupancy(int dynamic_lds);
+void engine_last_compress_tasks(uint32_t out[3]);
+
 int engine_set_device(int dev);
 int engine_thread_device(int dev);
 int engine_device_count();
diff --git a/c-blosc_amd/csrc/engine.hip b/c-blosc_amd/csrc/engine.hip
--- a/c-blosc_amd/csrc/engine.hip
+++ b/c-blosc_amd/csrc/engine.hip
@@ -119,6 +119,37 @@
   return -1;
 }
 
+enum { GRID_DECODE = 11, GRID_ZSTD_EXEC, GRID_ZSTD_STREAMS, GRID_ZLIB_STREAMS, kGridKernels };
+struct GridKernel { const char* name; const void* fn; int threads; int bound; };
+static const GridKernel* grid_kernels() {
+#define BAMD_ENC_GRID(MODE) {"k_encode_streams_t<" #MODE ">", (const void*)k_encode_streams_t<MODE>, 64 * ENC_WAVES, enc_grid_bound(MODE)}
+  static const GridKernel k[kGridKernels] = {
+    BAMD_ENC_GRID(ENC_LZ), BAMD_ENC_GRID(ENC_ZSTD), BAMD_ENC_GRID(ENC_ZLIB), BAMD_ENC_GRID(ENC_HC), BAMD_ENC_GRID(ENC_ZSTD_T), BAMD_ENC_GRID(ENC_ZSTD_HC),
+    BAMD_ENC_GRID(ENC_ZLIB_HC), BAMD_ENC_GRID(ENC_ZSTD_TH), BAMD_ENC_GRID(ENC_ZSTD_HCH), BAMD_ENC_GRID(ENC_ZLIB_DYN), BAMD_ENC_GRID(ENC_ZLIB_DYN_HC),
+    {"k_decode_streams", (const void*)k_decode_streams, 64 * DEC_WAVES, DEC_WAVES_PER_CU},
+    {"k_zstd_exec", (const void*)k_zstd_exec, 64, ZEXEC_WAVES_PER_CU},
+    {"k_zstd_streams", (const void*)k_zstd_streams, 64, ZSTD_WAVES_PER_CU},
+    {"k_zlib_streams", (const void*)k_zlib_streams, 64, ZLIB_WAVES_PER_CU}};
+#undef BAMD_ENC_GRID
+  return k;
+}
+static_assert(ENC_LZ == 0 && ENC_ZLIB_DYN_HC == 10, "the encoder's modes index the table above");
+static_assert(lds_occupied(DEC_WAVES * (int)DR_LDS_BYTES) * DEC_WAVES_PER_CU <= LDS_BYTES_PER_CU, "k_decode_streams: the workgroups of one CU fit its LDS, granule by granule");
+static_assert(lds_occupied((int)sizeof(uint32_t) * (int)ZXB_WORDS) * ZEXEC_WAVES_PER_CU <= LDS_BYTES_PER_CU, "k_zstd_exec: the workgroups of one CU fit its LDS, granule by granule");
+static_assert(lds_occupied((int)sizeof(ZstdLds)) * ZSTD_WAVES_PER_CU <= LDS_BYTES_PER_CU, "k_zstd_streams: the workgroups of one CU fit its LDS, granule by granule");
+static_assert(lds_occupied((int)sizeof(zi::Tabs)) * ZLIB_WAVES_PER_CU <= LDS_BYTES_PER_CU, "k_zlib_streams: the workgroups of one CU fit its LDS, granule by granule");
+static void query_persistent_grids(int* wpc, int* occupancy) {
+  const GridKernel* k = grid_kernels();
+  for (int i = 0; i < kGridKernels; i++) {
+    int occ = 0;
+#ifndef BAMD_WAVE_EMU
+    if (hipOccupancyMaxActiveBlocksPerMultiprocessor(&occ, k[i].fn, k[i].threads, 0) != hipSuccess || occ < 0) { (void)hipGetLastError(); occ = 0; }
+#endif
+    occupancy[i] = occ;
+    wpc[i] = (occ > 0 && occ < k[i].bound) ? occ : k[i].bound;
+  }
+}
+
 struct EngineState {
   std::mutex mu;
   bool device_ok = false;
@@ -135,6 +166,7 @@
   bool enc_cost_valid = false, dec_cost_valid = false;
   bool single_queue = false;
   int cus = 0;
+  int grid_wpc[kGridKernels] = {0}, grid_occupancy[kGridKernels] = {0};
   struct TableKey { std::vector<BlockDesc> blocks; std::vector<uint32_t> modes; std::vector<int> order; int nq = 0; };
   struct EncGroup { int mode; size_t q_at, sh_at; int32_t ntasks; };
   struct TableCache {
@@ -301,6 +333,7 @@
     st.single_queue = true;
     if (debug_enabled()) fprintf(stderr, "blosc_amd: %s is not on the allow-list of the relaxed in-kernel hand-off; using one task queue and unfused filters\n", have_props ? pr.gcnArchName : "(unknown device)");
   }
+  query_persistent_grids(st.grid_wpc, st.grid_occupancy);
   st.enc_cost_valid = st.dec_cost_valid = false;
   st.device_ok = true;
   st.device_hint.store(st.device, std::memory_order_relaxed);
@@ -416,22 +449,25 @@
 
 #ifdef BAMD_PROFILE_DECODE
 struct StreamProfile {
-  uint32_t* d = nullptr; const char* path; size_t bytes; hipStream_t stream;
-  StreamProfile(const char* switch_name, size_t nstr, hipStream_t s) : path(getenv(switch_name)), bytes(nstr * 64), stream(s) {
-    if (path && hipMalloc((void**)&d, bytes) == hipSuccess) (void)hipMemsetAsync(d, 0, bytes, stream);
+  uint32_t* d = nullptr; std::string path; size_t bytes; hipStream_t stream;
+  StreamProfile(const char* switch_name, size_t nrec, hipStream_t s, const char* suffix = "") : path(getenv(switch_name) ? getenv(switch_name) : ""), bytes(nrec * 64), stream(s) {
+    if (!path.empty()) path += suffix;
+    if (!path.empty() && bytes && hipMalloc((void**)&d, bytes) == hipSuccess) (void)hipMemsetAsync(d, 0, bytes, stream);
   }
   ~StreamProfile() {
     if (!d) return;
     std::vector<uint32_t> h(bytes / 4);
     (void)hipStreamSynchronize(stream); (void)hipMemcpy(h.data(), d, bytes, hipMemcpyDeviceToHost); (void)hipFree(d);
-    FILE* f = fopen(path, "wb");
+    FILE* f = fopen(path.c_str(), "wb");
     if (f) { fwrite(h.data(), 4, h.size(), f); fclose(f); }
   }
 };
 #define BAMD_STREAM_PROFILE(var, switch_name, nstr) StreamProfile var(switch_name, nstr, stream)
+#define BAMD_WAVE_PROFILE(var, switch_name, nwaves) StreamProfile var(switch_name, nwaves, stream, ".waves")
 #define BAMD_PROF_ARG(var) , var.d
 #else
 #define BAMD_STREAM_PROFILE(var, switch_name, nstr)
+#define BAMD_WAVE_PROFILE(var, switch_name, nwaves)
 #define BAMD_PROF_ARG(var)
 #endif
 
@@ -441,15 +477,13 @@
   bool zstd = false, zdyn = false;
   int detect = 0;
 };
-static EncVariant encoder_variant(int codec, int clevel) {
+static EncVariant encoder_variant(const EngineState& st, int codec, int clevel) {
   EncVariant v;
   const bool zstd = codec == kZstd, zlibc = codec == kZlib;
   const bool hc = codec == kLZ4HC && lz4hc_search_enabled();
   const bool ztab = zstd && zstd_tables_enabled();
   const bool zsearch = (zstd && zstd_search_enabled(clevel)) || (zlibc && zlib_search_enabled());
   const bool zhuf = zstd && (ztab || zsearch) && zstd_huffman_enabled();
-  const int enc_wpc_lz = (zstd || zlibc) ? ENC_WAVES_PER_CU : ENC_LZ_WAVES_PER_CU;
-  v.waves_per_cu = zsearch ? (160 * 1024) / (HC_TAB_BYTES + ZS_LDS_BYTES) : (hc ? HC_WAVES_PER_CU : enc_wpc_lz);
   v.zstd = zstd;
   v.zdyn = zlibc && zlib_dynamic_enabled();
   v.detect = (!zstd && !zlibc && periodic_enabled()) ? 1 : 0;
@@ -462,6 +496,7 @@
   else if (zlibc) v.mode = ENC_ZLIB;
   else if (hc) v.mode = ENC_HC;
   else v.mode = ENC_LZ;
+  v.waves_per_cu = st.grid_wpc[v.mode];
   return v;
 }
 constexpr int kEncModes = 11;
@@ -531,6 +566,32 @@
   return true;
 }
 
+int engine_persistent_grids(int cap, const char** names, int* launched, int* occupancy) {
+  CtxGuard ctx; EngineState& st = *ctx.st;
+  int wpc[kGridKernels], occ[kGridKernels];
+  if (st.device_ok && wanted_device() == st.device) { memcpy(wpc, st.grid_wpc, sizeof wpc); memcpy(occ, st.grid_occupancy, sizeof occ); }
+  else {
+    const int dev = wanted_device();
+    if (dev < 0 || hipSetDevice(dev) != hipSuccess) return -1;
+    query_persistent_grids(wpc, occ);
+  }
+  for (int i = 0; i < kGridKernels && i < cap; i++) { names[i] = grid_kernels()[i].name; launched[i] = wpc[i]; occupancy[i] = occ[i]; }
+  return kGridKernels;
+}
+int engine_enc_lz_occupancy(int dynamic_lds) {
+#ifdef BAMD_WAVE_EMU
+  return -1;
+#else
+  const int dev = wanted_device();
+  int occ = -1;
+  if (dev < 0 || hipSetDevice(dev) != hipSuccess) return -1;
+  if (hipOccupancyMaxActiveBlocksPerMultiprocessor(&occ, (const void*)k_encode_streams_t<ENC_LZ>, 64 * ENC_WAVES, (size_t)dynamic_lds) != hipSuccess) { (void)hipGetLastError(); return -1; }
+  return occ;
+#endif
+}
+static std::atomic<uint32_t> g_last_enc_tasks[3];
+void engine_last_compress_tasks(uint32_t out[3]) { for (int i = 0; i < 3; i++) out[i] = g_last_enc_tasks[i].load(); }
+
 int engine_compress_batch(const CompressParams* params, bool per_chunk, int n, const Job* jobs, int* results, bool device_ptrs,
                           hipStream_t stream, const PackedBuffer* packed) {
   if (n <= 0) return 0;
@@ -549,7 +610,7 @@
     io.add((size_t)chunks[(size_t)i].nbytes, (size_t)chunks[(size_t)i].cbytes);
     if (chunks[(size_t)i].mode & CH_MEMCPYED) continue;
     int8_t& m = variant_of[p.codec][p.clevel];
-    if (m < 0) { const EncVariant v = encoder_variant(p.codec, p.clevel); m = (int8_t)v.mode; B.variants[v.mode] = v; }
+    if (m < 0) { const EncVariant v = encoder_variant(st, p.codec, p.clevel); m = (int8_t)v.mode; B.variants[v.mode] = v; }
     B.variant[(size_t)i] = (uint8_t)m;
     if (!B.present[m]) { B.present[m] = true; B.ngroups++; }
   }
@@ -655,7 +716,8 @@
     const int detect = v.detect;
     const dim3 grid(persistent_grid(st, (size_t)g.ntasks, v.waves_per_cu)), block(64 * ENC_WAVES);
     BAMD_STREAM_PROFILE(prof, "BLOSC_AMD_ENC_PROFILE", nstr);
-#define BAMD_ENC_LAUNCH(MODE) case MODE: hipLaunchKernelGGL(k_encode_streams_t<MODE>, grid, block, 0, stream, d_streams, d_ticket, d_qlist, d_qoff, d_shoff, d_chunks, d_blocks, d_ready, d_cost, st.single_queue ? 1 : 0, d_seqbufs, d_ctabs, detect BAMD_PROF_ARG(prof)); break
+    BAMD_WAVE_PROFILE(wprof, "BLOSC_AMD_ENC_PROFILE", grid.x);
+#define BAMD_ENC_LAUNCH(MODE) case MODE: hipLaunchKernelGGL(k_encode_streams_t<MODE>, grid, block, 0, stream, d_streams, d_ticket, d_qlist, d_qoff, d_shoff, d_chunks, d_blocks, d_ready, d_cost, st.single_queue ? 1 : 0, d_seqbufs, d_ctabs, detect BAMD_PROF_ARG(prof) BAMD_PROF_ARG(wprof)); break
     switch (g.mode) {
       BAMD_ENC_LAUNCH(ENC_ZSTD_HCH); BAMD_ENC_LAUNCH(ENC_ZSTD_HC); BAMD_ENC_LAUNCH(ENC_ZSTD_TH); BAMD_ENC_LAUNCH(ENC_ZSTD_T); BAMD_ENC_LAUNCH(ENC_ZSTD);
       BAMD_ENC_LAUNCH(ENC_ZLIB_DYN_HC); BAMD_ENC_LAUNCH(ENC_ZLIB_DYN); BAMD_ENC_LAUNCH(ENC_ZLIB_HC); BAMD_ENC_LAUNCH(ENC_ZLIB);
@@ -692,6 +754,14 @@
   for (size_t k = 0; nstr && k < tc.groups.size(); k++)
     if (check_done((const uint32_t*)(P + p_cost) + kCostWords * k, (size_t)tc.groups[k].ntasks, 0, "compress")) return -1;
   if (packed) for (int i = 0; i <= n; i++) packed->offsets[i] = (size_t)((const uint64_t*)(P + p_offsets))[i];
+  if (nstr) {
+    uint32_t taken = 0, nshuf = 0;
+    for (size_t k = 0; k < tc.groups.size(); k++) {
+      taken += ((const uint32_t*)(P + p_cost) + kCostWords * k)[256];
+      nshuf += (uint32_t)tc.queues[tc.groups[k].sh_at + 8];
+    }
+    g_last_enc_tasks[0] = taken; g_last_enc_tasks[1] = (uint32_t)nstr; g_last_enc_tasks[2] = nshuf;
+  }
   tc.commit(B.key);
   if (feedback && nstr >= 4096) { memcpy(st.enc_cost, P + p_cost, sizeof st.enc_cost); st.enc_cost_valid = true; }
   const int32_t* r = (const int32_t*)(P + p_results);
@@ -866,7 +936,7 @@
     }
     if (L.nstr_queued) {
       ProfScope ps(st, stream, "k_decode_streams");
-      const dim3 dgrid(persistent_grid(st, L.nstr_queued ? L.nstr_queued : 1, DEC_WAVES_PER_CU));
+      const dim3 dgrid(persistent_grid(st, L.nstr_queued ? L.nstr_queued : 1, st.grid_wpc[GRID_DECODE]));
       BAMD_STREAM_PROFILE(prof, "BLOSC_AMD_DEC_PROFILE", L.nstr);
       hipLaunchKernelGGL(k_decode_streams, dgrid, dim3(64 * DEC_WAVES), 0, stream, L.d_streams, L.d_status, L.d_ticket, L.d_qlist, L.d_qoff, L.d_chunks, L.d_blocks, L.d_blkdone, L.d_spans, L.d_pat, L.d_cost, st.single_queue ? 1 : 0 BAMD_PROF_ARG(prof));
     }
@@ -884,7 +954,7 @@
       }
       {
         ProfScope ps(st, stream, "k_zstd_exec");
-        hipLaunchKernelGGL(k_zstd_exec, dim3(persistent_grid(st, L.nstr, ZEXEC_WAVES_PER_CU)), dim3(64), 0, stream, L.d_streams, (int)L.nstr, L.d_status, L.d_zticket + 1,
+        hipLaunchKernelGGL(k_zstd_exec, dim3(persistent_grid(st, L.nstr, st.grid_wpc[GRID_ZSTD_EXEC])), dim3(64), 0, stream, L.d_streams, (int)L.nstr, L.d_status, L.d_zticket + 1,
                            L.d_chunks, L.d_blocks, L.d_zmeta, L.zseq_delta);
       }
       d_taken = (const uint32_t*)L.d_zmeta;
@@ -892,12 +962,12 @@
     if (L.any_zstd) {
       ProfScope ps(st, stream, "k_zstd_streams");
       BAMD_STREAM_PROFILE(zprof, "BLOSC_AMD_ZSTD_PROFILE", L.nstr);
-      hipLaunchKernelGGL(k_zstd_streams, dim3(persistent_grid(st, L.nstr, ZSTD_WAVES_PER_CU)), dim3(64), 0, stream, L.d_streams, (int)L.nstr, L.d_status,
+      hipLaunchKernelGGL(k_zstd_streams, dim3(persistent_grid(st, L.nstr, st.grid_wpc[GRID_ZSTD_STREAMS])), dim3(64), 0, stream, L.d_streams, (int)L.nstr, L.d_status,
                          L.d_zticket, L.d_chunks, L.d_blocks, L.d_cost + 257, d_taken BAMD_PROF_ARG(zprof));
     }
     if (L.any_zlib) {
       ProfScope ps(st, stream, "k_zlib_streams");
-      hipLaunchKernelGGL(k_zlib_streams, dim3(persistent_grid(st, L.nstr_zlib ? L.nstr_zlib : 1, ZLIB_WAVES_PER_CU)), dim3(64), 0, stream, L.d_streams, L.d_status,
+      hipLaunchKernelGGL(k_zlib_streams, dim3(persistent_grid(st, L.nstr_zlib ? L.nstr_zlib : 1, st.grid_wpc[GRID_ZLIB_STREAMS])), dim3(64), 0, stream, L.d_streams, L.d_status,
                          L.d_zticket + 8, L.d_zqlist, L.d_zqoff, L.d_cost + 259, L.d_chunks, L.d_blocks, L.d_blkdone, st.single_queue ? 1 : 0);
     }
     if (L.any_shuf) {
diff --git a/c-blosc_amd/csrc/k_encode.hip b/c-blosc_amd/csrc/k_encode.hip
--- a/c-blosc_amd/csrc/k_encode.hip
+++ b/c-blosc_amd/csrc/k_encode.hip
@@ -81,25 +81,44 @@
     atomicAdd(plane_cost + (j & 255u), (uint32_t)((__builtin_amdgcn_s_memtime() - cost_t0) >> 10));
   }
 #ifdef BAMD_PROFILE_DECODE
-  prof_.c[15] = (uint32_t)(prof_.t0 >> 6);
+  prof_.c[15] = (uint32_t)__builtin_amdgcn_s_memrealtime();
   if (lane == 0 && profslot) for (int i_ = 0; i_ < 16; i_++) profslot[i_] = prof_.c[i_];
 #endif
 }
 
+constexpr int enc_lds_bytes(int mode) {
+  return (enc_mode_hc(mode) ? HC_TAB_BYTES : ENC_TAB_BYTES) +
+         (enc_mode_zstd(mode) ? ZS_LDS_BYTES : (enc_mode_zlib(mode) ? DFL_LDS_BYTES : (mode == ENC_LZ ? ENC_SCR_BYTES : 0)));
+}
+constexpr int enc_min_waves(int mode) {
+  return enc_mode_hc(mode) ? 2 : ((mode == ENC_ZSTD_T || mode == ENC_ZSTD_TH) ? 5 : (mode == ENC_LZ ? BAMD_ENC_LZ_MINWAVES : BAMD_ENC_MINWAVES));
+}
+constexpr int enc_grid_bound(int mode) { return lds_workgroups_per_cu(enc_lds_bytes(mode)) < 32 ? lds_workgroups_per_cu(enc_lds_bytes(mode)) : 32; }
 template <int MODE>
-__global__ __launch_bounds__(64 * ENC_WAVES, enc_mode_hc(MODE) ? 2 : ((MODE == ENC_ZSTD_T || MODE == ENC_ZSTD_TH) ? 5 : (MODE == ENC_LZ ? BAMD_ENC_LZ_MINWAVES : BAMD_ENC_MINWAVES))) void k_encode_streams_t(
+__global__ __launch_bounds__(64 * ENC_WAVES, enc_min_waves(MODE)) void k_encode_streams_t(
     StreamDesc* __restrict__ streams, uint32_t* __restrict__ tickets , const int32_t* __restrict__ qlist,
     const int32_t* __restrict__ qoff , const int32_t* __restrict__ shoff , const ChunkDesc* __restrict__ chunks, const BlockDesc* __restrict__ blocks,
     uint32_t* __restrict__ blk_ready, uint32_t* __restrict__ plane_cost, int single_queue,
     uint64_t* __restrict__ seqbufs, const zenc::CTabs* __restrict__ ctabs, int detect_periodic
 #ifdef BAMD_PROFILE_DECODE
-    , uint32_t* __restrict__ profbuf
+    , uint32_t* __restrict__ profbuf, uint32_t* __restrict__ profwave
 #endif
     ) {
+#ifdef BAMD_PROFILE_DECODE
+  const uint64_t wt_entry = __builtin_amdgcn_s_memtime(), wr_entry = __builtin_amdgcn_s_memrealtime();
+  uint64_t wt_stream = 0, wt_shuffle = 0, wt_wait = 0, wt_wait_first = 0;
+  uint32_t wn_stream = 0, wn_shuffle = 0;
+#define WPROF_BEGIN(t) const uint64_t t = __builtin_amdgcn_s_memtime()
+#define WPROF_END(acc, t) acc += __builtin_amdgcn_s_memtime() - t
+#else
+#define WPROF_BEGIN(t)
+#define WPROF_END(acc, t)
+#endif
   constexpr bool ZSTD = enc_mode_zstd(MODE);
   constexpr int TABBYTES = enc_mode_hc(MODE) ? HC_TAB_BYTES : ENC_TAB_BYTES;
-  __shared__ __attribute__((aligned(16))) enc_entry_t tabs[ENC_WAVES][(TABBYTES + (ZSTD ? ZS_LDS_BYTES : (enc_mode_zlib(MODE) ? DFL_LDS_BYTES : (MODE == ENC_LZ ? ENC_SCR_BYTES : 0)))) / 4];
+  __shared__ __attribute__((aligned(16))) enc_entry_t tabs[ENC_WAVES][lds_occupied(enc_lds_bytes(MODE)) / 4];
   static_assert(ENC_WAVES == 1, "one stream per wave, one wave per workgroup");
+  static_assert(lds_occupied(enc_lds_bytes(MODE)) * enc_grid_bound(MODE) <= LDS_BYTES_PER_CU, "the workgroups of one CU fit its LDS, granule by granule");
   const int lane = threadIdx.x & 63;
   uint64_t* seqbuf = nullptr;
   if (ZSTD) {
@@ -115,7 +134,12 @@
   auto shuffle_one = [&]() -> bool {
     const uint32_t s = take_ticket(tickets + 8 + xcc, lane);
     if (s >= shlen) return false;
+    WPROF_BEGIN(ts_);
     shuffle_block_task(chunks, blocks, uni((uint32_t)shlist[shbase + s]), blk_ready, streams, detect_periodic, lane, (volatile uint32_t*)tabs[0]);
+    WPROF_END(wt_shuffle, ts_);
+#ifdef BAMD_PROFILE_DECODE
+    wn_shuffle++;
+#endif
     return true;
   };
   uint32_t t = take_ticket(tickets + xcc, lane);
@@ -130,13 +154,22 @@
         const uint32_t gb = uni((uint32_t)sd->aux) >> 4;
         const ChunkDesc* cd = chunks + uni((uint32_t)sd->chunk);
         bool more = !(uni(cd->mode) & CH_BITSHUFFLE) && shuffle_generic_T(uni((uint32_t)cd->typesize));
+#ifdef BAMD_PROFILE_DECODE
+        const uint64_t tw_ = __builtin_amdgcn_s_memtime(), sh0_ = wt_shuffle;
+#endif
         while (__hip_atomic_load(&blk_ready[gb], __ATOMIC_RELAXED, __HIP_MEMORY_SCOPE_AGENT) == 0u) {
           if (BAMD_ENC_HELP && more && __hip_atomic_load(tickets + 8 + xcc, __ATOMIC_RELAXED, __HIP_MEMORY_SCOPE_AGENT) < (single_queue ? gb : gb / 8u) + (uint32_t)BAMD_ENC_HELP) more = shuffle_one();
           else __builtin_amdgcn_s_sleep(16);
         }
+#ifdef BAMD_PROFILE_DECODE
+        wt_wait += (__builtin_amdgcn_s_memtime() - tw_) - (wt_shuffle - sh0_);
+        if (wn_stream == 0) wt_wait_first = wt_wait;
+#endif
       }
 #ifdef BAMD_PROFILE_DECODE
+      const uint64_t te_ = __builtin_amdgcn_s_memtime();
       encode_one_stream<MODE>(streams + task, tabs[0], chunks, blk_ready, lane, blocks, (uint32_t)task, plane_cost, seqbuf, profbuf ? profbuf + (size_t)task * 16 : nullptr);
+      wt_stream += __builtin_amdgcn_s_memtime() - te_; wn_stream++;
 #else
       encode_one_stream<MODE>(streams + task, tabs[0], chunks, blk_ready, lane, blocks, (uint32_t)task, plane_cost, seqbuf);
 #endif
@@ -145,6 +178,18 @@
     t = take_ticket(tickets + xcc, lane);
   }
   if (lane == 0 && ndone) atomicAdd(plane_cost + 256, ndone);
+#ifdef BAMD_PROFILE_DECODE
+  if (lane == 0 && profwave) {
+    uint32_t* w = profwave + (size_t)blockIdx.x * 16;
+    const uint64_t wt_exit = __builtin_amdgcn_s_memtime(), wr_exit = __builtin_amdgcn_s_memrealtime();
+    w[0] = (uint32_t)wr_entry; w[1] = (uint32_t)(wr_entry >> 32); w[2] = (uint32_t)wr_exit; w[3] = (uint32_t)(wr_exit >> 32);
+    w[4] = (uint32_t)wt_stream; w[5] = (uint32_t)wt_shuffle; w[6] = (uint32_t)wt_wait; w[7] = ndone; w[8] = wn_stream; w[9] = wn_shuffle; w[10] = xcc;
+    w[11] = 1u;
+    w[12] = (uint32_t)(wt_exit - wt_entry); w[13] = (uint32_t)wt_wait_first;
+  }
+#endif
+#undef WPROF_BEGIN
+#undef WPROF_END
 }
 
 __global__ __launch_bounds__(256) void k_encode_plan(const ChunkDesc* __restrict__ chunks, const BlockDesc* __restrict__ blocks,
diff --git a/c-blosc_amd/csrc/queue_order.h b/c-blosc_amd/csrc/queue_order.h
--- a/c-blosc_amd/csrc/queue_order.h
+++ b/c-blosc_amd/csrc/queue_order.h
@@ -8,7 +8,10 @@
 
 namespace bamd {
 
-constexpr size_t kEncLookaheadDefault = 32;
+#ifndef BAMD_ENC_LOOKAHEAD
+#define BAMD_ENC_LOOKAHEAD 96
+#endif
+constexpr size_t kEncLookaheadDefault = BAMD_ENC_LOOKAHEAD;
 inline size_t enc_lookahead() { return kEncLookaheadDefault; }
 inline std::atomic<bool>& sched_override_off() { static std::atomic<bool> off{false}; return off; }
 inline bool sched_enabled() {
```

After: 810.9 GB/s, median of 6. +4.9%, better.
